# swesterfeld/audiowmark

Measured on AMD Instinct MI355X. Metric: audio seconds watermarked+decoded per wall-second (xRT), 44.1 kHz stereo, higher is better.
Workload: dtype f32; 1 GPU; 60 min stereo 44.1 kHz white noise per GPU resident in HBM, add+get incl. payload decode, payload 0123456789abcdef0011223344556677, strength 10; parallelism=1 GPU, patterns=108, payload_matches=104, ranks_seen=1

## Files before the change

audiowmark_amd/binding.py:

```python
import ctypes as C
import os

import numpy as np

_HERE = os.path.dirname(os.path.abspath(__file__))
N_BANDS = 81
BLOCK_FRAMES = 2226
SOFT_BITS = 858


class AwmError(RuntimeError):
    pass


def library_path():
    return os.path.join(_HERE, "libawm_hip.so")




def _load_hip_runtime():
    candidates = []
    try:
        import torch
# ... 105 lines not shown
lib.awm_add_watermark_segments_rate_s16_d.argtypes = [_vp, _vp, C.c_size_t, _vp, _vp, _vp, _vp, _vp, C.c_int, C.c_int]
lib.awm_add_watermark_segments_keys_rate_s16_d.argtypes = [_vp, _vp, C.c_size_t, _vp, _vp, _vp, _vp, _vp, C.c_int, C.c_int]
lib.awm_add_watermark_segments_rates_d.argtypes = [_vp, _vp, C.c_size_t, _vp, _vp, _vp, _vp, _vp, C.c_int, _vp]
lib.awm_add_watermark_segments_keys_rates_d.argtypes = [_vp, _vp, C.c_size_t, _vp, _vp, _vp, _vp, _vp, C.c_int, _vp]
lib.awm_add_watermark_segments_rates_s16_d.argtypes = [_vp, _vp, C.c_size_t, _vp, _vp, _vp, _vp, _vp, C.c_int, _vp]
lib.awm_add_watermark_segments_keys_rates_s16_d.argtypes = [_vp, _vp, C.c_size_t, _vp, _vp, _vp, _vp, _vp, C.c_int, _vp]


class SegmentPlan(C.Structure):
    _fields_ = [(n, C.c_uint64) for n in ("mix_first", "frame_first", "frame_last", "slice_first", "slice_last", "down_first", "down_last",
                                          "in_first", "in_last", "limiter_block", "first_block", "n_blocks")] + \
               [(n, C.c_int) for n in ("down_hl", "down_np", "down_step", "up_hl", "up_np", "up_step")]


lib.awm_add_segment_plan.argtypes = [C.c_int, C.c_size_t, C.c_size_t, C.POINTER(SegmentPlan)]


class StreamRatePlan(C.Structure):
    _fields_ = [(n, C.c_uint64) for n in ("limiter_block", "down_ahead", "mix_ahead", "min_tile")] + \
               [(n, C.c_int) for n in ("down_hl", "down_np", "down_step", "up_hl", "up_np", "up_step")]


lib.awm_add_stream_rate_plan.argtypes = [C.c_int, C.POINTER(StreamRatePlan)]
lib.awm_add_stream_create_rate_at.argtypes = [_vp, _vp, C.c_char_p, C.c_int, C.c_int, C.c_size_t, C.c_size_t, C.POINTER(_vp)]
lib.awm_add_stream_create_payloads_rate_at.argtypes = [_vp, _vp, _vp, C.c_size_t, C.c_int, C.c_int, C.c_size_t, C.c_size_t, C.POINTER(_vp)]
lib.awm_add_stream_sample_rate.argtypes = [_vp]
lib.awm_add_stream_sample_rate.restype = C.c_int
lib.awm_debug_resample_span_d.argtypes = [_vp, _vp, C.c_size_t, C.c_uint64, C.c_uint64, C.c_size_t, C.c_int, C.c_int, C.c_int, _vp, C.POINTER(C.c_int)]
lib.awm_debug_add_segments_fused_in_use.argtypes = []
lib.awm_debug_add_segments_fused_in_use.restype = C.c_int
lib.awm_debug_alloc_bytes.argtypes = []
lib.awm_debug_alloc_bytes.restype = C.c_ulonglong
lib.awm_debug_payload_tables_d.argtypes = [_vp, _vp, _vp, C.c_size_t, _vp]
lib.awm_debug_key_templates_d.argtypes = [_vp, _vp, C.c_size_t, _vp]
lib.awm_debug_key_payload_tables_d.argtypes = [_vp, _vp, _vp, C.c_size_t, _vp]
lib.awm_get_watermark_batch_d.argtypes = [_vp, _vp, C.c_size_t, _vp, _vp, C.c_int, C.c_int, C.c_size_t, _vp, _vp]
lib.awm_add_watermark_batch_keys_d.argtypes = [_vp, _vp, C.c_char_p, C.c_size_t, _vp, _vp, _vp, C.c_int]
lib.awm_get_watermark_batch_keys_d.argtypes = [_vp, _vp, C.c_size_t, _vp, _vp, C.c_int, C.c_int, C.c_size_t, _vp, _vp]
lib.awm_get_watermark_rate_d.argtypes = [_vp, _vp, _vp, C.c_size_t, C.c_int, C.c_int, C.c_size_t, _vp]
lib.awm_get_watermark_batch_rate_d.argtypes = [_vp, _vp, C.c_size_t, _vp, _vp, C.c_int, C.c_int, C.c_int, C.c_size_t, _vp, _vp]
lib.awm_get_watermark_batch_keys_rate_d.argtypes = [_vp, _vp, C.c_size_t, _vp, _vp, C.c_int, C.c_int, C.c_int, C.c_size_t, _vp, _vp]
lib.awm_debug_clip_slice_values.argtypes = [C.c_int]
lib.awm_debug_clip_slice_values.restype = C.c_size_t
lib.awm_debug_clip_stage_d.argtypes = [_vp, C.c_size_t, _vp, _vp, C.c_int, C.c_int, _vp, _vp]
lib.awm_get_watermark_batch_rates_d.argtypes = [_vp, _vp, C.c_size_t, _vp, _vp, C.c_int, _vp, C.c_int, C.c_size_t, _vp, _vp]
lib.awm_get_watermark_batch_keys_rates_d.argtypes = [_vp, _vp, C.c_size_t, _vp, _vp, C.c_int, _vp, C.c_int, C.c_size_t, _vp, _vp]
lib.awm_debug_clip_stage_rates_d.argtypes = [_vp, C.c_size_t, _vp, _vp, C.c_int, _vp, _vp, _vp]
lib.awm_get_batch_rates_plan.argtypes = [C.c_size_t, _vp, _vp, _vp, _vp]
lib.awm_get_watermark_batch_rates_s16_d.argtypes = [_vp, _vp, C.c_size_t, _vp, _vp, C.c_int, _vp, C.c_int, C.c_size_t, _vp, _vp]
lib.awm_get_watermark_batch_keys_rates_s16_d.argtypes = [_vp, _vp, C.c_size_t, _vp, _vp, C.c_int, _vp, C.c_int, C.c_size_t, _vp, _vp]
lib.awm_debug_clip_stage_rates_s16_d.argtypes = [_vp, C.c_size_t, _vp, _vp, C.c_int, _vp, _vp, _vp]
lib.awm_debug_clip_form_launches.argtypes = [_vp]
lib.awm_debug_clip_form_launches.restype = None
lib.awm_debug_lane_pcm_bytes.argtypes = [_vp]
lib.awm_debug_lane_pcm_bytes.restype = C.c_size_t
lib.awm_decode_chunk_d.argtypes = [_vp, _vp, _vp, C.c_size_t, C.c_int, C.c_int, C.c_size_t, _vp]
lib.awm_tab_up_down.argtypes = [_vp, C.c_int, C.c_int, _vp, _vp]
lib.awm_tab_bit_pos.argtypes = [_vp, _vp]
lib.awm_tab_mix_entries.argtypes = [_vp, _vp]
lib.awm_tab_bit_order.argtypes = [_vp, C.c_size_t, _vp]
lib.awm_tab_frame_mod.argtypes = [_vp, C.c_char_p, _vp]
lib.awm_tab_frame_mod_template.argtypes = [_vp, _vp]
lib.awm_tab_sync_bits.argtypes = [_vp, C.c_int, _vp]
lib.awm_tab_window.argtypes = [C.c_size_t, _vp]
lib.awm_tab_synth_window.argtypes = [_vp]
lib.awm_conv_encode.argtypes = [C.c_int, _vp, C.c_size_t, _vp]
lib.awm_test_gen_noise.argtypes = [_vp, C.c_size_t, _vp]


class RawFormat(C.Structure):
    _fields_ = [("n_channels", C.c_int), ("sample_rate", C.c_int), ("bit_depth", C.c_int), ("encoding", C.c_int), ("big_endian", C.c_int)]


lib.awm_add_watermark_file.argtypes = [_vp, _vp, C.c_char_p, C.c_char_p, C.c_char_p, C.POINTER(RawFormat), C.POINTER(RawFormat)]
lib.awm_add_stream_watermark_file.argtypes = [_vp, _vp, C.c_char_p, C.c_char_p, C.c_char_p, C.POINTER(RawFormat), C.POINTER(RawFormat), C.c_size_t]
lib.awm_add_stream_create_at.argtypes = [_vp, _vp, C.c_char_p, C.c_int, C.c_size_t, C.c_size_t, C.POINTER(_vp)]
lib.awm_debug_sync_db_sliding_d.argtypes = [_vp, _vp, C.c_size_t, C.c_int, _vp, C.c_size_t, C.c_int, C.c_int, _vp]
lib.awm_debug_sync_db_sliding_rows_d.argtypes = [_vp, _vp, C.c_size_t, C.c_int, _vp, _vp, C.c_size_t, C.c_int, C.c_int, _vp, _vp, C.c_longlong, C.c_longlong,
                                                 _vp, _vp, C.c_int, C.c_int, C.c_int, _vp, _vp, C.c_longlong, _vp, C.c_longlong]
lib.awm_debug_block_plane_ld.argtypes = [_vp]
lib.awm_debug_block_db_d.argtypes = [_vp, _vp, _vp, C.c_size_t, C.c_int, _vp, C.c_size_t, C.c_uint32, _vp, C.c_size_t, C.c_size_t, _vp, C.c_size_t,
                                     _vp, _vp]
lib.awm_debug_soft_bits_planes_d.argtypes = [_vp, _vp, _vp, C.c_size_t, C.c_size_t, C.c_int, _vp, _vp, _vp, C.c_size_t, _vp]
lib.awm_get_watermark_file.argtypes = [_vp, _vp, C.c_char_p, C.POINTER(RawFormat), C.c_size_t, _vp]
lib.awm_add_get_watermark_file.argtypes = [_vp, _vp, C.c_char_p, C.c_char_p, C.c_char_p, C.POINTER(RawFormat), C.POINTER(RawFormat), C.c_size_t, _vp]
lib.awm_add_stream_create.argtypes = [_vp, _vp, C.c_char_p, C.c_int, C.c_size_t, C.POINTER(_vp)]
lib.awm_add_stream_destroy.argtypes = [_vp]
lib.awm_add_stream_destroy.restype = None
lib.awm_add_stream_input.argtypes = [_vp]
lib.awm_add_stream_input.restype = C.c_void_p
lib.awm_add_stream_push.argtypes = [_vp, C.c_size_t, C.c_int, _vp, _vp]
lib.awm_add_mix_payloads_d.argtypes = [_vp, _vp, _vp, C.c_size_t, C.c_size_t, C.c_int, _vp, C.c_double, C.c_size_t, _vp, _vp, _vp,
                                       C.c_size_t, C.c_size_t]
lib.awm_add_stream_create_payloads_at.argtypes = [_vp, _vp, _vp, C.c_size_t, C.c_int, C.c_size_t, C.c_size_t, C.POINTER(_vp)]
lib.awm_add_stream_payloads.argtypes = [_vp]
lib.awm_add_stream_payloads.restype = C.c_size_t
lib.awm_add_stream_push_payloads.argtypes = [_vp, C.c_size_t, C.c_int, _vp, _vp]
lib.awm_add_watermark_payloads_file.argtypes = [_vp, _vp, _vp, C.c_size_t, C.c_char_p, _vp, C.POINTER(RawFormat), C.POINTER(RawFormat)]
lib.awm_add_stream_watermark_payloads_file.argtypes = [_vp, _vp, _vp, C.c_size_t, C.c_char_p, _vp, C.POINTER(RawFormat), C.POINTER(RawFormat),
                                                       C.c_size_t]
lib.awm_debug_set_payloads_file_tile.argtypes = [C.c_int]
lib.awm_debug_set_payloads_file_tile.restype = None


lib.awm_decode_chunks_d.argtypes = [_vp, _vp, _vp, C.c_size_t, C.c_int, C.c_int, _vp, _vp, C.c_int, C.c_size_t, _vp, _vp]
lib.awm_pcm_decode_d.argtypes = [_vp, _vp, C.c_size_t, C.c_int, C.c_int, C.c_int, _vp]
lib.awm_pcm_encode_d.argtypes = [_vp, _vp, C.c_size_t, C.c_int, C.c_int, C.c_int, C.c_int, _vp]
lib.awm_plan_chunks.argtypes = [C.c_size_t, C.c_size_t, _vp, _vp, _vp]
lib.awm_merge_patterns.argtypes = [_vp, _vp, _vp, C.c_int, C.c_size_t, _vp]
lib.awm_prof_name.restype = C.c_char_p
lib.awm_set_speed_params.argtypes = [C.c_int, C.c_int, C.c_double, C.c_double]
lib.awm_set_speed_params.restype = None
lib.awm_resample_ratio_frames.argtypes = [C.c_size_t, C.c_int, C.c_int, C.c_double, C.c_double]
lib.awm_resample_ratio_frames.restype = C.c_size_t
lib.awm_resample_ratio_d.argtypes = [_vp, _vp, C.c_size_t, C.c_int, C.c_int, C.c_double, C.c_double, _vp, C.c_size_t]
lib.awm_detect_speed_d.argtypes = [_vp, _vp, _vp, C.c_size_t, C.c_int, C.c_int, C.c_int, _vp, _vp]
lib.awm_detect_speed_batch_d.argtypes = [_vp, _vp, C.c_int, C.c_size_t, _vp, _vp, C.c_int, C.c_int, C.c_int, _vp, _vp, _vp]
lib.awm_debug_set_speed_batch_bytes.argtypes = [C.c_size_t]
lib.awm_debug_set_speed_batch_bytes.restype = None
lib.awm_debug_speed_batch_bytes.argtypes = []
lib.awm_debug_speed_batch_bytes.restype = C.c_size_t
lib.awm_debug_set_speed_batch.argtypes = [C.c_int]
lib.awm_debug_set_speed_batch.restype = None
lib.awm_speed_batch_plan.argtypes = [C.c_size_t, _vp, C.c_int, C.c_int, C.c_int, C.c_size_t, _vp, _vp]
lib.awm_debug_speed_batch_launches.argtypes = [_vp, _vp, _vp, _vp]
lib.awm_debug_speed_batch_launches.restype = None
lib.awm_debug_speed_scan_batch_d.argtypes = [_vp, _vp, C.c_int, C.c_size_t, _vp, _vp, C.c_int, C.c_int, _vp, C.c_double, C.c_double, C.c_int, C.c_int,
                                             _vp, _vp, C.c_size_t, _vp, _vp, _vp]
lib.awm_speed_clip_location_d.argtypes = [_vp, _vp, _vp, C.c_size_t, C.c_int, C.c_int, C.c_double, C.c_int, _vp]
lib.awm_speed_mags_d.argtypes = [_vp, _vp, _vp, C.c_size_t, C.c_int, C.c_int, C.c_double, C.c_double, C.c_double, C.c_size_t, _vp]
lib.awm_var_resample_table.argtypes = [C.c_double, _vp, C.c_size_t, C.POINTER(C.c_int)]
lib.awm_speed_scan_d.argtypes = [_vp, _vp, _vp, C.c_size_t, C.c_int, C.c_int, C.c_double, C.c_double, C.c_double, C.c_int, C.c_int,
                                 _vp, C.c_int, C.c_size_t, _vp, _vp]


class Params(C.Structure):
    _fields_ = [("struct_size", C.c_size_t), ("water_delta", C.c_double), ("mix", C.c_int), ("hard", C.c_int), ("strict", C.c_int),
                ("snr", C.c_int), ("payload_size", C.c_int), ("frames_per_bit", C.c_int), ("sync_threshold2", C.c_double),
                ("get_n_best", C.c_int), ("get_chunk_size", C.c_double), ("detect_speed", C.c_int), ("detect_speed_patient", C.c_int),
                ("try_speed", C.c_double), ("test_speed", C.c_double), ("test_cut", C.c_int), ("test_no_sync", C.c_int),
                ("test_no_limiter", C.c_int), ("test_truncate", C.c_int)]

    def __init__(self, **kw):
        super().__init__()
        lib.awm_params_init(C.byref(self))
        for k, v in kw.items():
            if k not in dict(self._fields_):
                raise TypeError(f"awm_params has no field {k}")
            setattr(self, k, v)


lib.awm_params_init.argtypes = [C.POINTER(Params)]
lib.awm_params_init.restype = None
lib.awm_set_global_params.argtypes = [C.POINTER(Params)]
lib.awm_ctx_set_params.argtypes = [_vp, C.POINTER(Params)]
lib.awm_ctx_get_params.argtypes = [_vp, C.POINTER(Params)]
lib.awm_ctx_snr_begin.argtypes = [_vp]
lib.awm_ctx_snr_end.argtypes = [_vp, C.POINTER(C.c_double), C.POINTER(C.c_double)]
lib.awm_get_watermark_keys_d.argtypes = [_vp, _vp, C.c_int, _vp, C.c_size_t, C.c_int, C.c_size_t, _vp, _vp]
lib.awm_get_watermark_keys_file.argtypes = [_vp, _vp, C.c_int, C.c_char_p, C.POINTER(RawFormat), C.c_size_t, _vp, _vp]


def set_global_params(**kw):
    p = Params(**kw)
    _check(lib.awm_set_global_params(C.byref(p)), "awm_set_global_params")

# ... 938 lines not shown
    def sync_fft(self, pcm, index, frame_count, want_frames=None, first=0, last=None, out=None):
        import torch
        n, ch = _pcm_shape(pcm)
        if last is None:
            last = n * ch
        if out is None:
            db = torch.zeros((frame_count, N_BANDS), dtype=torch.float32, device=pcm.device)
            have = torch.zeros(frame_count, dtype=torch.int8, device=pcm.device)
        else:
            db = _out_tensor(out[0], (frame_count, N_BANDS), torch.float32, pcm.device, "sync_fft (db)")
            have = _out_tensor(out[1], (frame_count,), torch.int8, pcm.device, "sync_fft (have)")
        want = None
        if want_frames is not None:
            want = np.ascontiguousarray(want_frames, np.int8)
        _check(lib.awm_sync_fft_d(self._h, _dev_ptr(pcm), n, ch, index, frame_count, _np(want) if want is not None else None,
                                  first, last, _dev_ptr(db), _dev_ptr(have)), "awm_sync_fft_d")
        return db, have

    def sync_search(self, key, pcm, clip_mode=False, max_out=4096):
        n, ch = _pcm_shape(pcm)
        while True:
            idx = np.zeros(max_out, np.uint64)
            q = np.zeros(max_out, np.float64)
            bt = np.zeros(max_out, np.int32)
            cnt = _check(lib.awm_sync_search_d(self._h, key_bytes(key), _dev_ptr(pcm), n, ch, int(clip_mode), max_out, _np(idx),
                                               _np(q), _np(bt)), "awm_sync_search_d")
            if cnt <= max_out:
                return idx[:cnt], q[:cnt], bt[:cnt]
            max_out = cnt

    def search_approx(self, key, pcm, clip_mode=False):
        n, ch = _pcm_shape(pcm)
        max_out = 4 * (n // 1024 + 1)
        idx = np.zeros(max_out, np.uint64)
        raw = np.zeros(max_out, np.float64)
        mean = np.zeros(max_out, np.float64)
        cnt = _check(lib.awm_search_approx_d(self._h, key_bytes(key), _dev_ptr(pcm), n, ch, int(clip_mode), max_out, _np(idx),
                                             _np(raw), _np(mean)), "awm_search_approx_d")
        return idx[:cnt], raw[:cnt], mean[:cnt]

    def block_soft_bits(self, key, pcm, indices):
        n, ch = _pcm_shape(pcm)
        idx = np.ascontiguousarray(indices, np.uint64)
        out = np.zeros((len(idx), SOFT_BITS), np.float32)
        ok = np.zeros(len(idx), np.int32)
        _check(lib.awm_block_soft_bits_d(self._h, key_bytes(key), _dev_ptr(pcm), n, ch, _np(idx), len(idx), _np(out), _np(ok)),
               "awm_block_soft_bits_d")
        return out, ok

    def block_plane_ld(self):
        return _check(lib.awm_debug_block_plane_ld(self._h), "awm_debug_block_plane_ld")

    def debug_block_db(self, key, pcm, indices, fill=0x7FC00000, slice_range=None, slice_frames=0, planes=None):
        import torch
        n, ch = _pcm_shape(pcm)
        idx = np.ascontiguousarray(indices, np.uint64)
        if planes is None:
            planes = torch.empty((len(idx), ch, N_BANDS, self.block_plane_ld()), dtype=torch.float32, device=pcm.device)
        assert planes.dtype == torch.float32 and planes.is_cuda and planes.is_contiguous()
        assert slice_range is None or (slice_range.dtype == torch.int64 and slice_range.is_cuda and slice_range.is_contiguous() and slice_range.dim() == 2
                                       and slice_range.shape[1] == 2)
        soft = np.zeros((len(idx), SOFT_BITS), np.float32)
        slot = np.zeros(len(idx), np.int32)
        _check(lib.awm_debug_block_db_d(self._h, key_bytes(key), _dev_ptr(pcm), n, ch, _np(idx), len(idx), fill,
                                        _dev_ptr(slice_range) if slice_range is not None else None,
                                        slice_range.shape[0] if slice_range is not None else 0, slice_frames, _dev_ptr(planes), planes.numel(),
                                        _np(soft), _np(slot)), "awm_debug_block_db_d")
        return planes, soft, slot

    def debug_soft_bits_planes(self, key, planes, n_blocks=None, channels=None, block_base=None, slice_range=None, range_index=None):
        import torch
        assert planes.dtype == torch.float32 and planes.is_cuda and planes.is_contiguous()
        n_blocks = planes.shape[0] if n_blocks is None else n_blocks
        channels = planes.shape[1] if channels is None else channels
        for t, dtype in ((block_base, torch.int64), (slice_range, torch.int64), (range_index, torch.int32)):
            assert t is None or (t.dtype == dtype and t.is_cuda and t.is_contiguous())
        opt = lambda t: _dev_ptr(t) if t is not None else None
        soft = np.zeros((max(n_blocks, 1), SOFT_BITS), np.float32)
        _check(lib.awm_debug_soft_bits_planes_d(self._h, key_bytes(key), _dev_ptr(planes), planes.numel(), n_blocks, channels, opt(block_base),
                                                opt(slice_range), opt(range_index), slice_range.shape[0] if slice_range is not None else 0,
                                                _np(soft)), "awm_debug_soft_bits_planes_d")
        return soft[:n_blocks]

    def viterbi_decode(self, block_type, soft):
        soft = np.ascontiguousarray(soft, np.float32)
        if soft.ndim == 1:
            soft = soft[None, :]
        n, coded_len = soft.shape
        rate = 12 if block_type == 2 else 6
        bits = np.zeros((n, coded_len // rate - 15), np.int32)
        err = np.zeros(n, np.float32)
        _check(lib.awm_viterbi_decode(self._h, block_type, _np(soft), coded_len, n, _np(bits), _np(err)), "awm_viterbi_decode")
        return bits, err

    def _pattern_buffer(self, max_out):
        buf = getattr(self, "_pat_buf", None)
        if buf is None or len(buf) < max_out:
            buf = self._pat_buf = (Pattern * max_out)()
        return buf

    def _patterns(self, fn, what, *args, max_out=4096):
        while True:
            buf = self._pattern_buffer(max_out)
            cnt = _check(fn(*args, max_out, C.cast(buf, C.c_void_p)), what)
            if cnt <= max_out:
                return patterns_to_dicts(buf, cnt)
            max_out = cnt

    def get_watermark(self, key, pcm, sample_rate=44100):
        n, ch = _pcm_shape(pcm)
        if sample_rate != 44100:
            return self._patterns(lib.awm_get_watermark_rate_d, "awm_get_watermark_rate_d", self._h, key_bytes(key), _dev_ptr(pcm), n, ch,
                                  sample_rate)
        return self._patterns(lib.awm_get_watermark_d, "awm_get_watermark_d", self._h, key_bytes(key), _dev_ptr(pcm), n, ch)

    def clip_stage(self, clips, sample_rate, out=None):
        import torch
        rates = _rates_array(sample_rate, len(clips))
        shapes = [_pcm_shape(c) for c in clips]
        ch = shapes[0][1]
        assert all(s[1] == ch for s in shapes)
        values = lib.awm_debug_clip_slice_values(ch)
        if out is None:
            out = torch.zeros((len(clips), values), dtype=torch.float32, device=clips[0].device)
        assert out.dtype == torch.float32 and out.is_contiguous() and out.numel() == len(clips) * values
        ptrs = (C.c_void_p * len(clips))(*[_dev_ptr(c) for c in clips])
        frames = (C.c_size_t * len(clips))(*[s[0] for s in shapes])
        ranges = np.zeros((len(clips), 2), np.int64)
        if rates is not None:
            _check(lib.awm_debug_clip_stage_rates_d(self._h, len(clips), ptrs, frames, ch, rates, _dev_ptr(out), _np(ranges)),
                   "awm_debug_clip_stage_rates_d")
        else:
            _check(lib.awm_debug_clip_stage_d(self._h, len(clips), ptrs, frames, ch, sample_rate, _dev_ptr(out), _np(ranges)),
                   "awm_debug_clip_stage_d")
        return out, ranges

    def add_get_watermark(self, key, payload_hex, pcm, out, sample_rate=44100):
        n, ch = _pcm_shape(pcm)
        assert _pcm_shape(out) == (n, ch) and out.data_ptr() != pcm.data_ptr()
        return self._patterns(lib.awm_add_get_watermark_d, "awm_add_get_watermark_d", self._h, key_bytes(key), payload_hex.encode(),
                              _dev_ptr(pcm), _dev_ptr(out), n, ch, sample_rate)

    def set_params(self, params=None, **kw):
        if params is None and kw:
            params = self.get_params()
            for k, v in kw.items():
                if k not in dict(Params._fields_):
                    raise TypeError(f"awm_params has no field {k}")
                setattr(params, k, v)
        _check(lib.awm_ctx_set_params(self._h, C.byref(params) if params is not None else None), "awm_ctx_set_params")

    def get_params(self):
        p = Params()
        _check(lib.awm_ctx_get_params(self._h, C.byref(p)), "awm_ctx_get_params")
        return p

    def snr_begin(self):
        _check(lib.awm_ctx_snr_begin(self._h), "awm_ctx_snr_begin")

    def snr_end(self):
        import math
        sig, delta = C.c_double(), C.c_double()
        _check(lib.awm_ctx_snr_end(self._h, C.byref(sig), C.byref(delta)), "awm_ctx_snr_end")
        return 10 * math.log10(sig.value / delta.value) if delta.value > 0 else float("inf")

    def _patterns_keys(self, fn, what, keys, *args, max_out=4096):
# ... 131 lines not shown
```

audiowmark_amd/csrc/hip/kernels.hh:

```
#pragma once
#include <hip/hip_runtime.h>
#include <cstddef>
#include <cstdint>

#if defined(__HIP_DEVICE_COMPILE__) && !defined(__gfx950__)
#error "audiowmark_amd's HIP kernels are written for gfx950 (MI355X) only"
#endif

namespace awmk {

struct DevTables
{
  const float2 *tw512;
  const float2 *tw1024;
  const float  *window;
  const float  *synth;
  const double2 *slide;
  const double2 *tw512d;
  const float2 *slide32;
};

hipError_t launch_stft_full (hipStream_t st, const DevTables& t, const float *pcm, int n_channels,
                             long long start_index, long long hop, long long frame_count, float2 *out);

// ... 163 lines not shown
                                             bool stereo_aligned, size_t lds_bytes);
struct RateMixSegment { MixSegment s; int limiter_block; };
hipError_t launch_mix_max_segments_rates (hipStream_t st, const RateMixSegment *segs_dev, int n_segs, long long max_frames, int n_channels,
                                          int min_limiter_block);
hipError_t launch_max_segments_rates_s16 (hipStream_t st, const RateMixSegment *segs_dev, int n_segs, long long max_frames, int n_channels,
                                          int min_limiter_block);
struct RateLimiterClip { LimiterClip c; int limiter_block; };
hipError_t launch_limiter_table_batch_rates (hipStream_t st, const RateLimiterClip *clips_dev, int n_clips, float ceiling, long long max_tab);
hipError_t launch_limiter_batch_rates (hipStream_t st, const RateLimiterClip *clips_dev, int n_clips, long long max_frames, int n_channels,
                                       int min_limiter_block, float ceiling, long long max_tab);
struct RateLimitEncodeSegment { LimitEncodeSegment s; int limiter_block; };
hipError_t launch_limit_encode_segments_rates (hipStream_t st, const RateLimitEncodeSegment *segs_dev, int n_segs, long long max_frames, bool mix,
                                               int min_limiter_block);

hipError_t launch_power_sums (hipStream_t st, const float *orig, const float *mixed, long long n_values, double *acc);

struct SyncDbArgs
{
  const float *pcm;
  long long    n_frames;
  int          n_channels;
  int          per_channel;
  long long    base0, base_stride;
  const long long *stream_base;
  int          count0;
  const int   *stream_count;
  long long    n_streams;
  long long    hop;
  float       *out;
  long long    out_stream_stride;
  long long    ld;
  char        *have;
  long long    have_stream_stride;
  long long    first, last;
  int          tile_frames;
  int          xcd_interleave = 0;
  const int           *row_perm = nullptr;
  const unsigned char *band_pos = nullptr;
  int                  rows_per_plane = 0;
  float               *tail = nullptr;
  long long            tail_stream_stride = 0;
  int                  tables_per_slice = 0;
  int                  streams_per_slice = 0;
  long long            slice_stride = 0;
  const long long     *stream_range = nullptr;
  const int           *range_index = nullptr;
  int                  range_div = 1;
  int                  silent_frames_are_zero = 0;
  int                  skip_unread_silent_tiles = 0;
};
hipError_t launch_sync_db (hipStream_t st, const DevTables& t, const SyncDbArgs& a);
hipError_t launch_sync_db_sliding (hipStream_t st, const DevTables& t, const SyncDbArgs& a);
bool sliding_rows_have_tail (int n_channels);

struct SyncTableDev
{
  const int *packed;
  int        rows_per_bit;
  const unsigned *chains = nullptr;
  long long       chains_slice_stride = 0;
  int             planes_per_slice = 1;
  const int      *row_frames = nullptr;
};
void pack_scan_chains (const int *packed, int rows_per_bit, unsigned *out );
struct SyncScanArgs
{
  const float *db;
  const char  *have;
  int          have_is_run = 0;
  long long    plane_stride;
  long long    have_plane_stride;
  long long    row_stride, band_stride, have_row_stride;
  long long    n_lanes;
  const int   *lane_count;
  long long    n_planes;
  double       min_delta;
  double      *quality;
  long long    q_stride;
  SyncTableDev table;
};
hipError_t launch_sync_scan (hipStream_t st, const SyncScanArgs& a);
hipError_t launch_sync_scan_window (hipStream_t st, const SyncScanArgs& a, int total_frames);

struct GatheredScanArgs
{
  const float *db;
  const char  *have;
  long long    plane_stride, have_plane_stride;
  int          ld;
  int          have_ld = 0;
  const float *tail = nullptr;
  long long    tail_plane_stride = 0;
  int          rows_per_bit;
  int          n_lanes;
  const int   *lane_count;
  long long    n_planes;
  double       min_delta;
  double      *quality;
  long long    q_stride;
  float       *chain_mag;
  int         *chain_n;
  int          regular_waves, tail_first, tail_lanes;
};
constexpr size_t GATHERED_SCRATCH_BYTES_PER_PLANE = 18 * 128 * 4;
hipError_t launch_sync_scan_gathered (hipStream_t st, const GatheredScanArgs& a);

hipError_t launch_local_mean (hipStream_t st, const double *q, long long q_stride, long long n_start_frames,
                              double *raw_sorted, double *local_mean, int n_slices = 1);

struct PeakOut { long long p; double raw, mean; };
hipError_t launch_peak_select (hipStream_t st, const double *raw_sorted, const double *local_mean, long long n, double threshold,
                               unsigned int *count, PeakOut *out, unsigned int cap);
hipError_t launch_peak_select_slices (hipStream_t st, const double *raw_sorted, const double *local_mean, long long n, double threshold,
                                      unsigned int *count, int count_stride, PeakOut *out, unsigned int cap, int n_slices);

hipError_t launch_peak_topk (hipStream_t st, const PeakOut *in, const unsigned int *count, unsigned int cap, PeakOut *out, int k, int n_slices);
hipError_t launch_peak_topk_lists (hipStream_t st, const PeakOut *in, const unsigned int *count, int count_stride, unsigned int cap,
                                   PeakOut *out, int k, int n_slices, int n_lists);

struct SoftBitsArgs
{
  const float   *db;
  long long      block_stride, ld;
  int            n_channels;
  const int16_t *mix_frame;
  const uint8_t *mix_up, *mix_down;
  int            n_data_frames;
  int            frames_per_bit;
  int            block_frames;
  long long      n_blocks;
  float         *out;
  const int     *block_slice = nullptr;
  const long long *block_base = nullptr;
  const long long *stream_range = nullptr;
  const int       *range_index = nullptr;
};
hipError_t launch_soft_bits (hipStream_t st, const SoftBitsArgs& a);
bool soft_bits_skips_silent_items (int n_channels, int frames_per_bit);

struct SoftJobDev
{
  int       mode;
  int       n_src, src_off;
  int       len;
  int       norm0, norm1;
  long long out_off;
  int       order_off;
  int       pad;
};
struct SoftPrepArgs
{
  const float      *raw;
  int               n_bits;
  const int        *inv_order;
  const SoftJobDev *jobs;
  const int2       *src;
  long long         n_jobs;
  int               hard;
  float            *out;
};
hipError_t launch_soft_prep (hipStream_t st, const SoftPrepArgs& a);

hipError_t launch_viterbi (hipStream_t st, const float *const soft[3], const long long n_blocks[3], long long n_steps,
                           unsigned char *const decisions_ws[3], int *const bits_out[3], float *const error_out[3], unsigned int *sync_ws);
size_t viterbi_workspace_bytes (long long coded_len, int rate, long long n_blocks);
bool viterbi_steps_supported (long long n_steps);
size_t viterbi_sync_bytes (long long n_blocks);
double probe_dependent_launch_us (hipStream_t st);
const char *viterbi_form_description();

struct KeyTableArgs
{
  const unsigned char *round_keys;
  const unsigned char *sbox;
  const unsigned char *coded;
  unsigned char       *scratch;
  int                  scratch_slots;
  signed char         *tables;
  long long            n_keys;
};
size_t key_table_scratch_bytes();
size_t key_table_bytes();
hipError_t launch_frame_mod_tables (hipStream_t st, const KeyTableArgs& a);

struct KeyTemplateOut
{
  short    *tmpl;
  long long stride;
};
hipError_t launch_key_templates (hipStream_t st, const KeyTableArgs& a, const KeyTemplateOut& t);

struct PayloadTableArgs
{
  const short         *tmpl;
  const int           *tmpl_of;
  long long            tmpl_stride;
  const unsigned char *coded;
  signed char         *tables;
  long long            table_stride;
  int                  half_entries;
  int                  n_code;
  int                  n_payloads;
};
size_t     payload_table_stride (size_t block_frames);
hipError_t launch_payload_tables (hipStream_t st, const PayloadTableArgs& a);

struct ClipKeyTableOut
{
  unsigned int  *chains;
  int           *row_frames, *want, *perm;
  unsigned char *pos;
  short         *mix_frame;
  unsigned char *mix_up, *mix_down;
  int           *inv_order;
};
constexpr int CLIP_KEY_ROWS = 170, CLIP_KEY_WANT = 1020, CLIP_KEY_MIX = 51480, CLIP_KEY_CODED = 858;
hipError_t launch_clip_key_tables (hipStream_t st, const KeyTableArgs& a, const ClipKeyTableOut& out);

// ... 112 lines not shown
```

audiowmark_amd/csrc/hip/kernels.hip:

```cpp
#include "kernels.hh"
#include "awm_fft.hip.h"
#include <cstdlib>
#include <algorithm>
#include <type_traits>
#include <atomic>

namespace awmk {

constexpr int NB = 81;
constexpr int MIN_BAND = 20;
constexpr int WAVES = 4;

typedef const int __attribute__ ((address_space (4))) *const_int_ptr;

__device__ __forceinline__ void
load_shared_tables (const DevTables& t, float2 *s_tw, float *s_win, float2 *s_twb)
{
  fft512_load_twiddles (t.tw512, s_tw);
  for (int i = threadIdx.x; i < 1024; i += blockDim.x)
    s_win[i] = t.window[i];
  if (s_twb)
    for (int i = threadIdx.x; i < NB; i += blockDim.x)
      s_twb[i] = t.tw1024[MIN_BAND + i];
}
// ... 3376 lines not shown
  int chain, cand;
  if (int (blockIdx.x) < a.regular_waves)
    {
      chain = blockIdx.x % 12;
      cand = (blockIdx.x / 12) * 64 + lane;
    }
  else
    {
      chain = lane / a.tail_lanes;
      cand = a.tail_first + lane % a.tail_lanes;
    }
  const bool active = chain < 12 && cand < count;
  if (!__any (active))
    return;
  if (!active)
    chain = 0, cand = 0;
  const int bit = chain >> 1, down = chain & 1;
  const int R = a.rows_per_bit;
  const int ld = a.ld;
  const bool from_tail = a.tail && cand >= ld;
  const long long step = from_tail ? 1 : ld;
  const float *p = from_tail ? a.tail + plane * a.tail_plane_stride + ((long long) bit * R * 60 + down * 30)
                             : a.db + plane * a.plane_stride + ((long long) bit * R * 60 + down * 30) * ld + cand;
  const int hld = a.have_ld ? a.have_ld : ld;
  const char *hv = HAVE ? a.have + plane * a.have_plane_stride + (long long) bit * R * hld + cand : nullptr;

  float mag = 0.f;
  int n = 0;
  auto issue = [&] (int r, float (&v)[30], bool& present) {
    const float *q = p + (long long) r * 60 * step;
    present = HAVE ? hv[r * hld] != 0 : true;
    if (HAVE && !__any (present))
      return;
#pragma unroll
    for (int i = 0; i < 30; i++)
      v[i] = q[i * step];
  };
  auto accumulate = [&] (const float (&v)[30], bool present) {
    if (present)
      {
#pragma unroll
        for (int i = 0; i < 30; i++)
          mag = __fadd_rn (mag, v[i]);
        n++;
      }
  };
  float v[3][30];
  bool pr[3] = { false, false, false };
  const int last = R - 1;
  int r = 0;
  if (R > 0)
    {
#pragma unroll
      for (int k = 0; k < 2; k++)
        {
          issue (k < last ? k : last, v[k], pr[k]);
          __builtin_amdgcn_sched_barrier (0);
        }
      for (; r + 3 <= R; r += 3)
        {
#pragma unroll
          for (int k = 0; k < 3; k++)
            {
              const int nx = r + k + 2;
              issue (nx < last ? nx : last, v[(k + 2) % 3], pr[(k + 2) % 3]);
              __builtin_amdgcn_sched_barrier (0);
              accumulate (v[k], pr[k]);
              __builtin_amdgcn_sched_barrier (0);
            }
        }
#pragma unroll
      for (int k = 0; k < 2; k++)
        if (r + k < R)
          accumulate (v[k], pr[k]);
    }
  if (active)
    {
      a.chain_mag[(plane * 12 + chain) * 128 + cand] = mag;
      if (!down)
        a.chain_n[(plane * 6 + bit) * 128 + cand] = n;
    }
}

__global__ void __launch_bounds__ (64)
sync_quality_kernel (GatheredScanArgs a)
{
  const long long plane = blockIdx.y;
  const int cand = blockIdx.x * 64 + threadIdx.x;
  if (cand >= a.lane_count[plane])
    return;
  double q = 0;
  int total = 0;
  for (int b = 0; b < 6; b++)
    {
      const float um = a.chain_mag[(plane * 12 + 2 * b) * 128 + cand], dm = a.chain_mag[(plane * 12 + 2 * b + 1) * 128 + cand];
      const int n = a.chain_n[(plane * 6 + b) * 128 + cand];
      float raw;
      if (um == 0 || dm == 0)
        raw = 0;
      else if (um < dm)
        raw = __fsub_rn (1.f, __fdiv_rn (um, dm));
      else
        raw = __fsub_rn (__fdiv_rn (dm, um), 1.f);
      const double rb = (b & 1) ? double (raw) : -double (raw);
      q += rb * n;
      total += n;
    }
  if (total)
    q /= total;
  q = q / a.min_delta / 2.9;
  a.quality[plane * a.q_stride + cand] = q;
}

hipError_t
launch_sync_scan_gathered (hipStream_t st, const GatheredScanArgs& a0)
{
  if (a0.n_lanes <= 0 || a0.n_planes <= 0)
    return hipSuccess;
  if (!a0.lane_count || a0.n_planes > 65535 || a0.n_lanes > 128 || !a0.chain_mag || !a0.chain_n)
    return hipErrorInvalidValue;
  GatheredScanArgs a = a0;
  const int full = a.n_lanes / 64, rem = a.n_lanes % 64;
  const bool tail = rem > 0 && rem * 12 <= 64;
  a.regular_waves = 12 * (tail || rem == 0 ? full : full + 1);
  a.tail_first = 64 * full;
  a.tail_lanes = tail ? rem : 1;
  const dim3 grid (unsigned (a.regular_waves + (tail ? 1 : 0)), unsigned (a.n_planes));
  if (a.have)
    hipLaunchKernelGGL (sync_scan_gathered_kernel<true>, grid, dim3 (64), 0, st, a);
  else
    hipLaunchKernelGGL (sync_scan_gathered_kernel<false>, grid, dim3 (64), 0, st, a);
  hipLaunchKernelGGL (sync_quality_kernel, dim3 (unsigned ((a.n_lanes + 63) / 64), unsigned (a.n_planes)), dim3 (64), 0, st, a);
  return hipGetLastError();
}

__global__ void __launch_bounds__ (256)
local_mean_kernel (const double *q, long long q_stride, long long S, double *raw_sorted, double *local_mean)
{
  const long long p = (long long) blockIdx.x * blockDim.x + threadIdx.x;
  const long long n_scores = 4 * S;
  if (p >= n_scores)
    return;
  q += (long long) blockIdx.y * 4 * q_stride;
  raw_sorted += (long long) blockIdx.y * n_scores;
  local_mean += (long long) blockIdx.y * n_scores;
  double avg = 0;
  int n = 0;
  for (int j = -20; j <= 20; j++)
    {
      if (j > -4 && j < 4)
        continue;
      const long long idx = p + j;
      if (idx >= 0 && idx < n_scores)
        {
          avg += q[(idx & 3) * q_stride + (idx >> 2)];
          n++;
        }
    }
  if (n > 0)
    avg /= n;
  raw_sorted[p] = q[(p & 3) * q_stride + (p >> 2)];
  local_mean[p] = avg;
}

hipError_t
launch_local_mean (hipStream_t st, const double *q, long long q_stride, long long n_start_frames, double *raw_sorted, double *local_mean,
                   int n_slices)
{
  const long long n = 4 * n_start_frames;
  if (n <= 0 || n_slices <= 0)
    return hipSuccess;
  hipLaunchKernelGGL (local_mean_kernel, dim3 (unsigned ((n + 255) / 256), unsigned (n_slices)), dim3 (256), 0, st, q, q_stride, n_start_frames,
                      raw_sorted, local_mean);
  return hipGetLastError();
}

__global__ void __launch_bounds__ (128)
soft_bits_kernel (SoftBitsArgs a)
{
  const long long blk = blockIdx.y;
  const int bit = blockIdx.x * blockDim.x + threadIdx.x;
  const int n_bits = a.n_data_frames / a.frames_per_bit;
  if (bit >= n_bits)
    return;
  const float *db = a.db + blk * a.block_stride;
  const int C = a.n_channels;
  const long long mix0 = a.block_slice ? (long long) a.block_slice[blk] * a.n_data_frames * 30 : 0;
  const int16_t *mix_frame = a.mix_frame + mix0;
  const uint8_t *mix_up = a.mix_up + mix0, *mix_down = a.mix_down + mix0;
  double umag = 0, dmag = 0;
  for (int f = bit * a.frames_per_bit; f < (bit + 1) * a.frames_per_bit; f++)
    for (int ch = 0; ch < C; ch++)
      {
        const float *plane = db + (long long) ch * NB * a.ld;
        for (int j = 0; j < 30; j++)
          {
            const int b = f * 30 + j;
            const int frame = mix_frame[b];
            const int next = frame + 1 < a.block_frames ? frame + 1 : frame - 1;
            const int prev = frame - 1 >= 0 ? frame - 1 : frame + 1;
            const float *pu = plane + (long long) (mix_up[b] - MIN_BAND) * a.ld;
            const float *pd = plane + (long long) (mix_down[b] - MIN_BAND) * a.ld;
            umag += pu[frame];
            umag -= double (__fadd_rn (pu[prev], pu[next])) * 0.5;
            dmag += pd[frame];
            dmag -= double (__fadd_rn (pd[prev], pd[next])) * 0.5;
          }
      }
  a.out[blk * n_bits + bit] = float (umag - dmag);
}

constexpr int SB_WAVES = 4;
constexpr int SB_BPW = 4;
constexpr int SB_MAX_ITEMS = 256;

__global__ void __launch_bounds__ (64 * SB_WAVES)
soft_bits_wave_kernel (SoftBitsArgs a, int groups_per_block)
{
  extern __shared__ __attribute__ ((aligned (16))) float4 s_item_dyn[];
  const int lane = threadIdx.x & 63, wave = threadIdx.x >> 6;
  const long long slot = blockIdx.x >> 3;
  const long long blk = (slot / groups_per_block) * 8 + (blockIdx.x & 7);
  const int group = int (slot % groups_per_block);
  if (blk >= a.n_blocks)
    return;
  const int n_bits = a.n_data_frames / a.frames_per_bit;
  const int bit0 = (group * SB_WAVES + wave) * SB_BPW;
  if (bit0 >= n_bits)
    return;
  const float *db = a.db + blk * a.block_stride;
  const int C = a.n_channels;
  const long long mix0 = a.block_slice ? (long long) a.block_slice[blk] * a.n_data_frames * 30 : 0;
  const int16_t *mix_frame = a.mix_frame + mix0;
  const uint8_t *mix_up = a.mix_up + mix0, *mix_down = a.mix_down + mix0;
  const int n_items = a.frames_per_bit * C * 30;
  float4 *items = s_item_dyn + (size_t) wave * SB_BPW * n_items;
  const int n_here = min (SB_BPW, n_bits - bit0);
  int live_lo = 0, live_hi = 0x7fffffff;
  if (a.stream_range)
    {
      const long long sl = a.range_index[blk];
      const long long first = a.stream_range[2 * sl], last = a.stream_range[2 * sl + 1];
      live_lo = a.block_frames;
      live_hi = -1;
      if (first >= 0)
        {
          const long long base = a.block_base[blk];
          const long long lo_num = (first + C - 1) / C - 1024 - base, hi_num = last / C - base;
          const long long lo = lo_num <= 0 ? 0 : (lo_num + 1023) / 1024, hi = hi_num < 0 ? -1 : hi_num / 1024;
          live_lo = int (lo < a.block_frames ? lo : a.block_frames);
          live_hi = int (hi < a.block_frames ? hi : a.block_frames - 1);
        }
    }
  const float zero_db = db_from_complex (make_float2 (0.f, 0.f));
  for (int i = lane; i < n_items; i += 64)
#pragma unroll
  for (int q = 0; q < SB_BPW; q++)
    {
      const int e = q * n_items + i;
      const int bit = bit0 + min (q, n_here - 1);
      const int fi = i / (C * 30), ch = (i / 30) % C, j = i % 30;
      const int b = (bit * a.frames_per_bit + fi) * 30 + j;
      const int frame = mix_frame[b];
      const int next = frame + 1 < a.block_frames ? frame + 1 : frame - 1;
      const int prev = frame - 1 >= 0 ? frame - 1 : frame + 1;
      if (max (frame, max (prev, next)) < live_lo || min (frame, min (prev, next)) > live_hi)
        {
          items[e] = make_float4 (zero_db, __fadd_rn (zero_db, zero_db), zero_db, __fadd_rn (zero_db, zero_db));
          continue;
        }
      const float *plane = db + (long long) ch * NB * a.ld;
      const float *pu = plane + (long long) (mix_up[b] - MIN_BAND) * a.ld;
      const float *pd = plane + (long long) (mix_down[b] - MIN_BAND) * a.ld;
      items[e] = make_float4 (pu[frame], __fadd_rn (pu[prev], pu[next]), pd[frame], __fadd_rn (pd[prev], pd[next]));
    }
  wave_sync();
  if (lane < n_here)
    {
      const float4 *mine = items + lane * n_items;
      double umag = 0, dmag = 0;
      for (int i = 0; i < n_items; i++)
        {
          const float4 t = mine[i];
          umag = __dadd_rn (umag, double (t.x));
          umag = __dsub_rn (umag, __dmul_rn (double (t.y), 0.5));
          dmag = __dadd_rn (dmag, double (t.z));
          dmag = __dsub_rn (dmag, __dmul_rn (double (t.w), 0.5));
        }
      a.out[blk * n_bits + bit0 + lane] = float (__dsub_rn (umag, dmag));
    }
}

int g_soft_bits_generic = 0;
extern "C" void awm_debug_set_soft_bits_generic (int on) { g_soft_bits_generic = on; }

bool
soft_bits_skips_silent_items (int n_channels, int frames_per_bit)
{
  return !g_soft_bits_generic && frames_per_bit * n_channels * 30 <= SB_MAX_ITEMS;
}

hipError_t
launch_soft_bits (hipStream_t st, const SoftBitsArgs& a)
{
  if (a.n_blocks <= 0)
    return hipSuccess;
  const int n_bits = a.n_data_frames / a.frames_per_bit;
// ... 990 lines not shown
```

audiowmark_amd/csrc/host/capi_kernels.cc:

```cpp
#include "context.hh"
#include "syncfinder.hh"
#include "wmget.hh"
#include "wmdecode.hh"
#include "wmspeed.hh"
#include "utils.hh"
#include "wmfile.hh"
#include "keytab_stage.hh"
#include <sys/stat.h>
#include <atomic>
#include <future>
#include <thread>
#include <tuple>
#include <algorithm>
#include <array>
#include <cmath>
#include <cstdlib>
#include <cstring>
#include <memory>

using namespace awm;
namespace awm { Key capi_key (const uint8_t key[16]); }
namespace awm { extern int g_key_tables_on_device; int clip_key_tables_check (awm_ctx *ctx, const uint8_t *keys, size_t n_keys, long long mismatch_out[9]); }

namespace {
// ... 1660 lines not shown
    bad = "slice_range_d, n_slices and slice_frames go together";
  else if (slice_range_d && (slice_frames > n_frames || n_slices > n_frames / slice_frames))
    bad = "the slices do not fit into the samples";
  if (!bad && slice_range_d)
    for (size_t i = 0; i < n_blocks && !bad; i++)
      if (index[i] <= n_frames && n_frames - index[i] >= block_len && index[i] / slice_frames >= n_slices)
        bad = "a block starts behind the last slice";
  if (!bad && slice_range_d)
    if (int rc = debug_check_ranges (ctx, slice_range_d, n_slices, (long long) (n_frames * n_channels), bad))
      return rc;
  if (bad)
    {
      set_error (std::string ("awm_debug_block_db_d: ") + bad);
      return AWM_ERR_ARG;
    }
  KeyTables *kt = ctx->get_key_tables (capi_key (key));
  if (!kt)
    return AWM_ERR_HIP;
  const size_t n_bits = mark_data_frame_count() / params().frames_per_bit;
  const std::vector<size_t> idx (index, index + n_blocks);
  std::vector<int> slot_of;
  std::vector<char> ok;
  const BlockDbView view { fill, planes_out_d };
  if (int rc = block_soft_bits_dev (ctx, ctx, kt, make_wav (pcm_d, n_frames, n_channels), idx, slot_of, ok, slice_range_d, slice_frames, &view))
    return rc;
  size_t n_slots = 0;
  for (size_t i = 0; i < n_blocks; i++)
    {
      slot_out[i] = slot_of[i];
      n_slots = std::max (n_slots, size_t (slot_of[i] + 1));
    }
  if (n_slots)
    AWM_HIP_CHECK (hipMemcpyAsync (soft_out, ctx->ws_soft.ptr, n_slots * n_bits * sizeof (float), hipMemcpyDeviceToHost, ctx->stream));
  AWM_HIP_CHECK (stream_wait (ctx->stream));
  return 0;
}

int
awm_debug_soft_bits_planes_d (awm_ctx *ctx, const uint8_t key[16], const float *planes_d, size_t planes_values, size_t n_blocks, int n_channels,
                              const long long *block_base_d, const long long *slice_range_d, const int *range_index_d, size_t n_slices,
                              float *soft_out)
{
  AWM_ENTER (ctx);
  const size_t block_values = size_t (std::max (n_channels, 0)) * Params::n_bands * size_t (block_plane_ld());
  const bool ranges = slice_range_d != nullptr;
  const char *bad = nullptr;
  if (!planes_d || !soft_out)
    bad = "null pointer";
  else if (n_channels < 1 || n_channels > 3)
    bad = "1, 2 or 3 channels";
  else if (n_blocks < 1 || n_blocks > DEBUG_BLOCKS_MAX)
    bad = "1 .. 64 blocks";
  else if (planes_values / block_values < n_blocks)
    bad = "planes_d holds fewer than n_blocks blocks";
  else if ((block_base_d != nullptr) != ranges || (range_index_d != nullptr) != ranges || (n_slices != 0) != ranges)
    bad = "block_base_d, slice_range_d, range_index_d and n_slices go together";
  if (!bad && ranges)
    {
      std::vector<long long> base (n_blocks);
      std::vector<int> slice (n_blocks);
      AWM_HIP_CHECK (hipMemcpyAsync (base.data(), block_base_d, n_blocks * sizeof (long long), hipMemcpyDeviceToHost, ctx->stream));
      AWM_HIP_CHECK (hipMemcpyAsync (slice.data(), range_index_d, n_blocks * sizeof (int), hipMemcpyDeviceToHost, ctx->stream));
      if (int rc = debug_check_ranges (ctx, slice_range_d, n_slices, DEBUG_RANGE_MAX * n_channels, bad))
        return rc;
      for (size_t i = 0; i < n_blocks && !bad; i++)
        if (base[i] < 0 || base[i] > DEBUG_RANGE_MAX || slice[i] < 0 || size_t (slice[i]) >= n_slices)
          bad = "a block's base or slice is out of range";
    }
  if (bad)
    {
      set_error (std::string ("awm_debug_soft_bits_planes_d: ") + bad);
      return AWM_ERR_ARG;
    }
  KeyTables *kt = ctx->get_key_tables (capi_key (key));
  if (!kt)
    return AWM_ERR_HIP;
  const size_t n_bits = mark_data_frame_count() / params().frames_per_bit;
  if (int rc = ctx->ws_soft.reserve (n_blocks * n_bits * sizeof (float))) return rc;
  const awmk::SoftBitsArgs sb = block_soft_args (kt, n_channels, planes_d, n_blocks, ctx->ws_soft.as<float>(), block_base_d, range_index_d,
                                                 slice_range_d, ranges);
  AWM_HIP_CHECK (awmk::launch_soft_bits (ctx->stream, sb));
  AWM_HIP_CHECK (hipMemcpyAsync (soft_out, ctx->ws_soft.ptr, n_blocks * n_bits * sizeof (float), hipMemcpyDeviceToHost, ctx->stream));
  AWM_HIP_CHECK (stream_wait (ctx->stream));
  return 0;
}

int
awm_viterbi_decode (awm_ctx *ctx, int block_type, const float *soft, size_t coded_len, size_t n, int *bits_out, float *error_out)
{
  AWM_ENTER (ctx);
  if (block_type < 0 || block_type > 2)
    return AWM_ERR_ARG;
  std::vector<std::vector<float>> in (n);
  for (size_t i = 0; i < n; i++)
    in[i].assign (soft + i * coded_len, soft + (i + 1) * coded_len);
  std::vector<std::vector<int>> bits;
  std::vector<float> errors;
  if (int rc = viterbi_decode (ctx, ConvBlockType (block_type), in, bits, errors))
    return rc;
  for (size_t i = 0; i < n; i++)
    {
      std::copy (bits[i].begin(), bits[i].end(), bits_out + i * bits[i].size());
      error_out[i] = errors[i];
    }
  return 0;
}

int
awm_add_watermark_d (awm_ctx *ctx, const uint8_t key[16], const char *payload_hex, const float *pcm_in_d, float *out_d,
                     size_t n_frames, int n_channels, int sample_rate)
{
  AWM_ENTER (ctx);
  if (n_channels >= 1 && add_buffers_overlap (pcm_in_d, out_d, n_frames * size_t (n_channels)))
    {
      set_error ("awm_add_watermark_d: the output overlaps the input");
      return AWM_ERR_ARG;
    }
  FrameModTable *fm = ctx->get_frame_mod (capi_key (key), payload_hex ? payload_hex : "");
  if (!fm)
    return AWM_ERR_ARG;
  if (sample_rate != Params::mark_sample_rate)
    return add_full_rate (ctx, pcm_in_d, out_d, n_frames, n_channels, fm->dev.as<int8_t>(), params().water_delta, !params().test_no_limiter, sample_rate);
  return add_full (ctx, pcm_in_d, out_d, n_frames, n_channels, fm->dev.as<int8_t>(), params().water_delta, !params().test_no_limiter);
}

extern "C" void awm_debug_set_add_payloads_fused (int on) { g_add_payloads_fused = on; }
extern "C" int  awm_debug_add_payloads_fused_in_use (void) { return g_add_payloads_fused_in_use; }
extern "C" int  awm_debug_add_payloads_tile (void) { return awmk::ADD_MULTI_TILE; }
static int g_add_payloads_rate_fused = 2, g_add_payloads_rate_fused_in_use = 0;
extern "C" void awm_debug_set_add_payloads_rate_fused (int mode) { g_add_payloads_rate_fused = mode < 0 ? 0 : mode > 2 ? 2 : mode; }
extern "C" int  awm_debug_add_payloads_rate_fused_in_use (void) { return g_add_payloads_rate_fused_in_use; }

static int
add_payloads_rate (awm_ctx *ctx, const Key& k, const char *const *payload_hex, size_t n_payloads, const float *pcm_in_d, float *const *out_d,
                   size_t n_frames, int C, double water_delta, int use_limiter, int rate, const RateConverter& down, const RateConverter& up,
                   bool *taken)
{
  hipStream_t st = ctx->stream;
  const size_t last44 = up.window_start (n_frames - 1) + size_t (up.hl()) + 1;
  const size_t F = last44 / Params::frame_size + 1;
  const size_t n44 = (F + 1) * Params::frame_size;
  const size_t n_ws = std::min<size_t> (n_payloads, size_t (awmk::ADD_MULTI_TILE)), ws_values = n44 * size_t (C);
  const int lim_block = int (size_t (rate) * size_t (Params::limiter_block_size_ms) / 1000);
  const size_t n_blocks = n_frames / lim_block + 2;
  const ResampleTable& ut = *up.fixed;
  awmk::ResampleMixArgs ma {};
  ma.orig = pcm_in_d;
  ma.n_in = (long long) (F * Params::frame_size);
  ma.n_channels = C;
  ma.ctab = ut.ctab.as<float>();
  ma.hl = ut.hl;
  ma.np = ut.np;
  ma.step = ut.step;
  ma.n_out = (long long) n_frames;
  ma.n_blocks = (long long) n_blocks;
  ma.limiter_block = lim_block;
  ma.n = 1;
  bool mixed = g_add_payloads_rate_fused == 2;
  for (size_t p = 0; mixed && p < n_payloads; p++)
    {
      ma.o[0].wm44 = pcm_in_d;
      ma.o[0].out = out_d[p];
      mixed = awmk::resample_mix_multi_takes (ma);
    }
  *taken = false;
  if (ctx->ws_rate_a.reserve (ws_values * sizeof (float)) || ctx->ws_rate_b.reserve (n_ws * ws_values * sizeof (float))
// ... 3056 lines not shown
```

audiowmark_amd/csrc/host/context.cc:

```cpp
#include "context.hh"
#include <algorithm>
#include <atomic>
#include <chrono>
#include <cstdlib>
#include "utils.hh"
#include <cmath>
#include <cstring>

namespace awm {

static thread_local std::string g_last_error;
void set_error (const std::string& msg) { g_last_error = msg; }
const std::string& last_error() { return g_last_error; }
std::string hip_error_string (hipError_t e) { return std::string (hipGetErrorName (e)) + " (" + hipGetErrorString (e) + ")"; }

static std::atomic<long>   g_dev_allocs { 0 }, g_pin_allocs { 0 };
static std::atomic<double> g_dev_alloc_ms { 0.0 }, g_pin_alloc_ms { 0.0 };
static std::atomic<unsigned long long> g_dev_alloc_bytes { 0 };
static void
note_alloc (std::atomic<long>& count, std::atomic<double>& ms, std::chrono::steady_clock::time_point t0)
{
  const double dt = std::chrono::duration<double, std::milli> (std::chrono::steady_clock::now() - t0).count();
  count.fetch_add (1, std::memory_order_relaxed);
  double cur = ms.load (std::memory_order_relaxed);
// ... 75 lines not shown
extern "C" void
awm_debug_alloc_stats (long *dev_allocs, double *dev_ms, long *pinned_allocs, double *pinned_ms)
{
  if (dev_allocs) *dev_allocs = awm::g_dev_allocs.load();
  if (dev_ms) *dev_ms = awm::g_dev_alloc_ms.load();
  if (pinned_allocs) *pinned_allocs = awm::g_pin_allocs.load();
  if (pinned_ms) *pinned_ms = awm::g_pin_alloc_ms.load();
}

extern "C" unsigned long long awm_debug_alloc_bytes (void) { return awm::g_dev_alloc_bytes.load(); }

hipEvent_t
awm::ReadyMarks::next_event()
{
  if (used == pool.size())
    {
      hipEvent_t e = nullptr;
      if (hipEventCreateWithFlags (&e, hipEventDisableTiming) != hipSuccess)
        return nullptr;
      pool.push_back (e);
    }
  return pool[used++];
}

void
awm::ReadyMarks::release()
{
  disarm();
  for (hipEvent_t e : pool)
    (void) hipEventDestroy (e);
  pool.clear();
}

bool
awm::FileStaging::ensure_events()
{
  if (have_events)
    return true;
  for (int i = 0; i < RING; i++)
    for (hipEvent_t *e : { &in_copied[i], &in_used[i], &out_encoded[i], &out_copied[i] })
      if (!*e && hipEventCreateWithFlags (e, hipEventDisableTiming) != hipSuccess)
        return false;
  have_events = true;
  return true;
}

void
awm::FileStaging::release()
{
  for (int i = 0; i < RING; i++)
    {
      for (hipEvent_t *e : { &in_copied[i], &in_used[i], &out_encoded[i], &out_copied[i] })
        if (*e)
          {
            (void) hipEventDestroy (*e);
            *e = nullptr;
          }
      in_host[i].release();
      out_host[i].release();
      in_dev[i].release();
      out_dev[i].release();
    }
  pcm.release();
  have_events = false;
}

void
awm::WorkLane::release_lane()
{
  for (DevBuffer *b : { &ws_db, &ws_block_db, &ws_have, &ws_q, &ws_raw, &ws_mean, &ws_misc, &ws_refine, &ws_refine_have, &ws_soft, &ws_viterbi,
                        &ws_viterbi_in, &ws_viterbi_bits, &ws_viterbi_err, &ws_viterbi_sync, &ws_block_max, &ws_clip, &ws_idx, &ws_limit_tab, &ws_jobs, &ws_group, &ws_keytab, &ws_keytab_aux, &ws_keytab_scratch, &ws_rate, &ws_pcm, &ws_shard_edge, &ws_shard_tail, &ws_shard_q })
    b->release();
  for (PinnedBuffer *b : { &pin_refine_in[0], &pin_refine_in[1], &pin_refine_q[0], &pin_refine_q[1], &pin_peaks, &pin_blocks, &pin_jobs, &pin_bits, &pin_small, &pin_group, &pin_shard, &pin_shard_up, &pin_keytab })
    b->release();
  for (hipEvent_t& ev : ev_refine)
    if (ev)
      {
        (void) hipEventDestroy (ev);
        ev = nullptr;
      }
  if (ev_sync)
    (void) hipEventDestroy (ev_sync);
  ev_sync = nullptr;
  awm::speed_scratch_free (this);
}

unsigned int *
awm::WorkLane::viterbi_sync (size_t n_decodes)
{
  const size_t before = ws_viterbi_sync.bytes;
  if (ws_viterbi_sync.reserve (awmk::viterbi_sync_bytes ((long long) n_decodes)))
    return nullptr;
  if (ws_viterbi_sync.bytes != before && hipMemsetAsync (ws_viterbi_sync.ptr, 0, ws_viterbi_sync.bytes, stream) != hipSuccess)
    {
      ws_viterbi_sync.release();
      return nullptr;
    }
  return ws_viterbi_sync.as<unsigned int>();
}

awm::WorkLane *
awm_ctx::lane (int i)
{
  if (i <= 0)
    return this;
  if (i >= awm::MAX_LANES)
    return nullptr;
  auto& l = extra_lanes[i - 1];
  if (!l)
    {
      auto nl = std::make_unique<awm::WorkLane>();
      if (hipStreamCreateWithFlags (&nl->stream, hipStreamNonBlocking) != hipSuccess)
        return nullptr;
      nl->own_stream = true;
      l = std::move (nl);
    }
  return l.get();
}

using namespace awm;

int
awm::upload_sync (DevBuffer& buf, const void *src, size_t bytes, hipStream_t st)
{
  if (int rc = buf.reserve (bytes ? bytes : 1))
    return rc;
  static std::mutex staging_mutex;
  static PinnedBuffer staging;
  std::lock_guard<std::mutex> lock (staging_mutex);
  if (int rc = staging.reserve (bytes ? bytes : 1))
    return rc;
  std::memcpy (staging.ptr, src, bytes);
  AWM_HIP_CHECK (hipMemcpyAsync (buf.ptr, staging.ptr, bytes, hipMemcpyHostToDevice, st));
  AWM_HIP_CHECK (hipStreamSynchronize (st));
  return 0;
}

std::vector<float>
awm::zita_table (double frel, unsigned h, unsigned n)
{
  auto sinc = [] (double x) { x = std::fabs (x); if (x < 1e-6) return 1.0; x *= M_PI; return std::sin (x) / x; };
  auto wind = [] (double x) { x = std::fabs (x); if (x >= 1.0) return 0.0; x *= M_PI; return 0.384 + 0.500 * std::cos (x) + 0.116 * std::cos (2 * x); };
  std::vector<float> ctab (size_t (h) * (n + 1));
  float *p = ctab.data();
  for (unsigned j = 0; j <= n; j++)
    {
      double t = double (j) / double (n);
      for (unsigned i = 0; i < h; i++)
        {
          p[h - i - 1] = float (frel * sinc (t * frel) * wind (t / h));
          t += 1;
        }
      p += h;
    }
  return ctab;
}

static int
upload (DevBuffer& buf, const void *src, size_t bytes, hipStream_t st)
{
  return upload_sync (buf, src, bytes, st);
}

static std::vector<int>
pack_sync_table (const SyncTable& t, const std::vector<int>& want_pos )
{
  const int R = t.rows_per_bit;
  std::vector<int> packed (size_t (6) * R * 64, 0);
  for (int bit = 0; bit < 6; bit++)
    for (int r = 0; r < R; r++)
      {
        int *row = &packed[(size_t (bit) * R + r) * 64];
        const size_t src = size_t (bit) * R + r;
        for (int i = 0; i < 30; i++)
          {
            row[i] = t.up[src * 30 + i];
            row[30 + i] = t.down[src * 30 + i];
          }
        row[60] = want_pos.empty() ? t.frame[src] : want_pos[t.frame[src]];
        row[61] = r + 1 < R ? (want_pos.empty() ? t.frame[src + 1] : want_pos[t.frame[src + 1]]) : 0x7fffffff;
      }
  return packed;
}

namespace awm {
ClipKeyHost
build_clip_key_host (const Key& key)
{
  ClipKeyHost h;
  const SyncTable st = build_sync_table (key, true);
  const int total = mark_block_frame_count() * 2, R = st.rows_per_bit;
  std::vector<int> want_pos (total, -1);
  std::vector<char> want (total, 0);
  for (int f : st.frame)
    want[f] = 1;
  for (int f = 0; f < total; f++)
    if (want[f])
// ... 388 lines not shown

  std::vector<float> blob;
  auto push_c = [&] (double re, double im) { blob.push_back (float (re)); blob.push_back (float (im)); };
  const size_t off_tw512 = blob.size();
  for (int k = 0; k < 512; k++)
    push_c (std::cos (-2 * M_PI * k / 512), std::sin (-2 * M_PI * k / 512));
  const size_t off_tw1024 = blob.size();
  for (int k = 0; k <= 512; k++)
    push_c (std::cos (-2 * M_PI * k / 1024), std::sin (-2 * M_PI * k / 1024));
  while (blob.size() % 4) blob.push_back (0);
  const size_t off_win = blob.size();
  auto win = gen_normalized_window (Params::frame_size);
  blob.insert (blob.end(), win.begin(), win.end());
  const size_t off_synth = blob.size();
  auto synth = gen_synth_window();
  blob.insert (blob.end(), synth.begin(), synth.end());
  std::vector<double> slide;
  for (int k = 19; k <= 102; k++)
    {
      for (int j = 0; j < 8; j++)
        {
          slide.push_back (std::cos (-2 * M_PI * k * j / 1024));
          slide.push_back (std::sin (-2 * M_PI * k * j / 1024));
        }
      slide.push_back (std::cos (2 * M_PI * k * 8 / 1024));
      slide.push_back (std::sin (2 * M_PI * k * 8 / 1024));
    }
  const size_t off_tw512d = slide.size();
  for (int k = 0; k < 512; k++)
    {
      slide.push_back (std::cos (-2 * M_PI * k / 512));
      slide.push_back (std::sin (-2 * M_PI * k / 512));
    }
  const size_t off_slide32 = slide.size();
  {
    std::vector<float> f;
    for (int k = 19; k <= 102; k++)
      for (int j = 0; j < 8; j++)
        {
          f.push_back (float (std::cos (2 * M_PI * k * (8 - j) / 1024)));
          f.push_back (float (std::sin (2 * M_PI * k * (8 - j) / 1024)));
        }
    slide.resize (off_slide32 + f.size() / 2);
    std::memcpy (slide.data() + off_slide32, f.data(), f.size() * sizeof (float));
  }
  if (int rc = upload (ctx->tab_slide, slide.data(), slide.size() * sizeof (double), ctx->stream))
    return rc;
  ctx->tabs.slide = ctx->tab_slide.as<double2>();
  ctx->tabs.tw512d = reinterpret_cast<const double2 *> (ctx->tab_slide.as<double>() + off_tw512d);
  ctx->tabs.slide32 = reinterpret_cast<const float2 *> (ctx->tab_slide.as<double>() + off_slide32);
  if (int rc = upload (ctx->tab_mem, blob.data(), blob.size() * sizeof (float), ctx->stream))
    return rc;
  const float *base = ctx->tab_mem.as<float>();
  ctx->tabs.tw512 = reinterpret_cast<const float2 *> (base + off_tw512);
  ctx->tabs.tw1024 = reinterpret_cast<const float2 *> (base + off_tw1024);
  ctx->tabs.window = base + off_win;
  ctx->tabs.synth = base + off_synth;
  if (awmk::probe_dependent_launch_us (ctx->stream) < 0 && hipStreamSynchronize (ctx->stream) != hipSuccess)
    {
      set_error ("awm_ctx_create: the device does not complete work on the context's stream");
      return AWM_ERR_HIP;
    }
  *ctx_out = ctx.release();
  return 0;
}

int
awm_ctx_set_chunk_lanes (awm_ctx *ctx, int n_lanes)
{
  if (!ctx || n_lanes < 1)
    return AWM_ERR_ARG;
  ctx->chunk_lanes = std::min (n_lanes, awm::CHUNK_LANES);
  return 0;
}

int
awm_ctx_warm_up (awm_ctx *ctx, int detect_speed, int file_level)
{
  if (!ctx)
    return AWM_ERR_ARG;
  AWM_HIP_CHECK (hipSetDevice (ctx->device));
  const int lanes = std::max (1, std::min (ctx->chunk_lanes, awm::CHUNK_LANES)) * (detect_speed ? 2 : 1);
  for (int i = 0; i < lanes && i < awm::MAX_LANES; i++)
    if (!ctx->lane (i))
      {
        awm::set_error ("cannot create a work lane (stream)");
        return AWM_ERR_HIP;
      }
  if (file_level && !ctx->get_copy_stream())
    {
      awm::set_error ("cannot create the copy stream");
      return AWM_ERR_HIP;
    }
  return 0;
}

int
awm_ctx_trim (awm_ctx *ctx)
{
  if (!ctx)
    return AWM_ERR_ARG;
  AWM_HIP_CHECK (hipSetDevice (ctx->device));
  AWM_HIP_CHECK (hipStreamSynchronize (ctx->stream));
  for (auto& l : ctx->extra_lanes)
    if (l)
      {
        if (l->stream)
          AWM_HIP_CHECK (hipStreamSynchronize (l->stream));
        l->release_lane();
      }
  if (ctx->copy_stream)
    AWM_HIP_CHECK (hipStreamSynchronize (ctx->copy_stream));
  ctx->release_lane();
  ctx->file_staging.release();
  awm::speed_workspace_free (ctx);
  ctx->ws_add_batch.release();
  ctx->pin_add_batch.release();
  ctx->ws_seg_in.release();
  ctx->ws_key_tmpl.release();
  ctx->ws_seg_out.release();
  ctx->ws_merge_soft.release();
  ctx->ws_rate_a.release();
  ctx->ws_rate_b.release();
  ctx->ws_rate_c.release();
  for (awm_ctx *h : ctx->helpers)
    if (h && h != ctx)
      if (int rc = awm_ctx_trim (h)) return rc;
  return 0;
}

size_t
awm_debug_lane_pcm_bytes (awm_ctx *ctx)
{
  if (!ctx)
    return 0;
  size_t bytes = ctx->ws_pcm.bytes;
  for (auto& l : ctx->extra_lanes)
    if (l)
      bytes += l->ws_pcm.bytes;
  return bytes;
}

void
awm_ctx_destroy (awm_ctx *ctx)
{
  if (!ctx)
    return;
  (void) hipSetDevice (ctx->device);
  (void) hipStreamSynchronize (ctx->stream);
  for (auto& kt : ctx->key_tables)
    release_key_tables (*kt);
  for (auto& t : ctx->frame_mod_tables)
    t->dev.release();
  for (auto& t : ctx->frame_mod_templates)
    t->dev.release();
  for (auto& t : ctx->resample_tables)
    t->ctab.release();
  awm::speed_workspace_free (ctx);
  ctx->ws_snr.release();
  ctx->ws_seg_in.release();
  ctx->ws_key_tmpl.release();
  ctx->ws_seg_out.release();
  ctx->ws_add_batch.release();
  ctx->pin_add_batch.release();
  if (ctx->ev_add_batch)
    (void) hipEventDestroy (ctx->ev_add_batch);
  ctx->ev_add_batch = nullptr;
  ctx->ws_merge_soft.release();
  for (hipEvent_t e : ctx->merge_events)
    if (e)
      (void) hipEventDestroy (e);
  ctx->merge_events.clear();
  ctx->ws_rate_a.release();
  ctx->ws_rate_b.release();
  ctx->ws_rate_c.release();
  ctx->tab_mem.release();
  ctx->tab_slide.release();
  for (auto& l : ctx->extra_lanes)
    if (l)
      {
        if (l->stream)
          (void) hipStreamSynchronize (l->stream);
        l->release_lane();
        if (l->own_stream && l->stream)
          (void) hipStreamDestroy (l->stream);
      }
  ctx->release_lane();
  if (ctx->copy_stream)
    (void) hipStreamSynchronize (ctx->copy_stream);
  ctx->file_staging.release();
  ctx->ready.release();
  if (ctx->copy_stream)
    (void) hipStreamDestroy (ctx->copy_stream);
  if (ctx->own_stream && ctx->stream)
    (void) hipStreamDestroy (ctx->stream);
  delete ctx;
}

int awm_ctx_device (const awm_ctx *ctx) { return ctx ? ctx->device : -1; }

int
awm_ctx_synchronize (awm_ctx *ctx)
{
  if (!ctx)
    return AWM_ERR_ARG;
  AWM_HIP_CHECK (hipStreamSynchronize (ctx->stream));
  return 0;
}

void *awm_ctx_stream (awm_ctx *ctx) { return ctx ? (void *) ctx->stream : nullptr; }

int
awm_ctx_set_stream (awm_ctx *ctx, void *hip_stream)
{
  if (!ctx)
    return AWM_ERR_ARG;
  AWM_HIP_CHECK (hipStreamSynchronize (ctx->stream));
  if (ctx->own_stream && ctx->stream)
    (void) hipStreamDestroy (ctx->stream);
  ctx->stream = (hipStream_t) hip_stream;
  ctx->own_stream = false;
  return 0;
}

}
```

audiowmark_amd/csrc/host/context.hh:

```
#pragma once
#include <condition_variable>
#include <mutex>
#include <hip/hip_runtime.h>
#include <map>
#include <mutex>
#include <memory>
#include <string>
#include <vector>
#include "../hip/kernels.hh"
#include "wmcommon.hh"

namespace awm { void set_error (const std::string& msg); const std::string& last_error(); std::string hip_error_string (hipError_t e); }

#define AWM_HIP_CHECK(expr) \
  do { hipError_t e__ = (expr); if (e__ != hipSuccess) { awm::set_error (std::string (#expr) + ": " + awm::hip_error_string (e__)); return AWM_ERR_HIP; } } while (0)

namespace awm {

inline void
cpu_relax()
{
  for (int k = 0; k < 48; k++)
    __builtin_ia32_pause();
}
// ... 107 lines not shown

struct SpeedWorkspace;
struct SpeedScratch;
struct WorkLane;
void speed_scratch_free (WorkLane *lane);
} struct awm_ctx; namespace awm {
void speed_workspace_free (awm_ctx *ctx);

struct FileStaging
{
  static constexpr int RING = 4;
  PinnedBuffer in_host[RING], out_host[RING];
  DevBuffer    in_dev[RING], out_dev[RING];
  DevBuffer    pcm;
  bool         keep = false;
  size_t       kept_values = 0;
  int          kept_channels = 0, kept_rate = 0;
  hipEvent_t   in_copied[RING] = {}, in_used[RING] = {}, out_encoded[RING] = {}, out_copied[RING] = {};
  bool         have_events = false;
  bool         ensure_events();
  void         release();
};

struct ReadyMarks
{
  const float *base = nullptr;
  size_t       n_frames = 0;
  bool         armed = false;
  std::vector<std::pair<size_t, hipEvent_t>> marks;
  std::vector<hipEvent_t> pool;
  size_t       used = 0;
  hipEvent_t   next_event();
  bool         live = false, live_done = false;
  std::mutex   mu;
  std::condition_variable cv;
  void         disarm() { armed = false; live = live_done = false; marks.clear(); used = 0; base = nullptr; n_frames = 0; }
  void         release();
};

struct FrameModTable
{
  std::vector<unsigned char> key;
  std::string payload;
  bool        mix = true;
  int         frames_per_bit = 2;
  unsigned long last_use = 0;
  DevBuffer   dev;
};

struct FrameModTemplate
{
  std::vector<unsigned char> key;
  bool        mix = true;
  int         frames_per_bit = 2;
  unsigned long last_use = 0;
  DevBuffer   dev;
};

}

namespace awm {
enum ProfId { PROF_ADD_MIX, PROF_LIMITER, PROF_SYNC_DB, PROF_SYNC_SCAN, PROF_LOCAL_MEAN, PROF_REFINE_DB, PROF_REFINE_SCAN,
              PROF_BLOCK_DB, PROF_SOFT_BITS, PROF_VITERBI, PROF_STFT,
              PROF_RESAMPLE, PROF_RESAMPLE_VAR, PROF_SPEED_MAGS, PROF_SPEED_COMPARE, PROF_KEYTAB, PROF_ADD_MIX_MULTI, PROF_PAYLOAD_TAB,
              PROF_RESAMPLE_MIX, PROF_CLIP_RESAMPLE, PROF_KEY_TEMPLATE, PROF_CLIP_STAGE_MIXED,
              PROF_CLIP_PAD_S16, PROF_CLIP_RESAMPLE_S16, PROF_CLIP_STAGE_MIXED_S16,
              PROF_PCM_DECODE, PROF_PCM_ENCODE, PROF_SEGMENT_GATHER_S16, PROF_LIMIT_ENCODE_S16, PROF_COUNT };
struct ProfPending { int id; hipEvent_t start, stop; };
}

namespace awm {
struct WorkLane
{
  hipStream_t    stream = nullptr;
  bool           own_stream = false;
  DevBuffer ws_db, ws_block_db, ws_have, ws_q, ws_raw, ws_mean, ws_misc, ws_refine, ws_refine_have, ws_soft,
            ws_viterbi, ws_viterbi_in, ws_viterbi_bits, ws_viterbi_err, ws_viterbi_sync, ws_block_max, ws_clip, ws_idx, ws_limit_tab, ws_jobs, ws_group, ws_keytab, ws_keytab_aux, ws_keytab_scratch;
  DevBuffer ws_rate;
  DevBuffer ws_pcm;
  DevBuffer ws_shard_edge, ws_shard_tail, ws_shard_q;
  PinnedBuffer pin_refine_in[2], pin_refine_q[2], pin_peaks, pin_blocks, pin_jobs, pin_bits, pin_small, pin_group, pin_shard, pin_shard_up, pin_keytab;
  hipEvent_t   ev_refine[2] = { nullptr, nullptr };
  hipEvent_t   ev_sync = nullptr;
  SpeedScratch *speed_scratch = nullptr;
  double       prof_live_fraction = 1.0;
  unsigned int *viterbi_sync (size_t n_decodes);
  void release_lane();
};
constexpr int MAX_LANES = 16;
constexpr int CHUNK_LANES = 4;
}

struct awm_ctx : awm::WorkLane
{
  int            device = -1;
  awmk::DevTables tabs {};
  awm::DevBuffer tab_mem, tab_slide;

  std::vector<std::unique_ptr<awm::KeyTables>>     key_tables;
  std::vector<std::unique_ptr<awm::FrameModTable>> frame_mod_tables;
  std::vector<std::unique_ptr<awm::FrameModTemplate>> frame_mod_templates;
  std::vector<std::unique_ptr<awm::ResampleTable>> resample_tables;
  awm::ResampleTable *get_resample_table (int rate_in, int rate_out);
  awm::DevBuffer ws_rate_a, ws_rate_b, ws_rate_c;
  std::unique_ptr<awm::WorkLane> extra_lanes[awm::MAX_LANES - 1];
  awm::WorkLane *lane (int i);
  awm::FileStaging file_staging;
  awm::ReadyMarks ready;
  hipStream_t    copy_stream = nullptr;
  hipStream_t    get_copy_stream();
  std::vector<awm_ctx *> helpers;
  std::unique_ptr<awm::ParamValues> own_params;
  awm::DevBuffer ws_merge_soft;
  std::vector<hipEvent_t> merge_events;
  awm::DevBuffer    ws_add_batch;
  awm::PinnedBuffer pin_add_batch;
  hipEvent_t        ev_add_batch = nullptr;
  awm::DevBuffer ws_seg_in, ws_seg_out;
  awm::DevBuffer ws_key_tmpl;
  awm::DevBuffer ws_snr;
  bool           snr_on = false;
  int            chunk_lanes = awm::CHUNK_LANES;

  awm::SpeedWorkspace *speed = nullptr;
  std::mutex     speed_mutex;

  std::mutex     table_mutex;
  unsigned long  table_clock = 0;
  static constexpr size_t MAX_CACHED_TABLES = 64;
  std::mutex     prof_mutex;
  bool   prof_enabled = false;
  std::vector<awm::ProfPending> prof_pending;
  double prof_ms[awm::PROF_COUNT] = { 0 };
  long   prof_launches[awm::PROF_COUNT] = { 0 };
  double prof_bytes[awm::PROF_COUNT] = { 0 };
  void   prof_collect();

  awm::KeyTables     *get_key_tables (const awm::Key& key);
  awm::FrameModTable *get_frame_mod (const awm::Key& key, const std::string& payload_hex);
  awm::FrameModTemplate *get_frame_mod_template (const awm::Key& key);
};

#include "../../../include/awm_hip.h"

namespace awm {
struct ProfScope
{
  awm_ctx *ctx;
  int      id;
  hipEvent_t start = nullptr;
  hipStream_t st;
  ProfScope (awm_ctx *c, int i, double algorithmic_bytes, hipStream_t stream = nullptr) : ctx (c), id (i), st (stream ? stream : c->stream)
  {
    if (!ctx->prof_enabled)
      return;
    {
      std::lock_guard<std::mutex> lock (ctx->prof_mutex);
      ctx->prof_bytes[id] += algorithmic_bytes;
      ctx->prof_launches[id]++;
    }
    if (hipEventCreate (&start) != hipSuccess) { start = nullptr; return; }
    (void) hipEventRecord (start, st);
  }
  ~ProfScope()
  {
    if (!start)
// ... 10 lines not shown
```

audiowmark_amd/csrc/host/syncfinder.cc:

```cpp
#include "syncfinder.hh"
#include "utils.hh"
#include <algorithm>
#include <cmath>
#include <cstdlib>

namespace awm {

static inline int
total_frames (SyncFinder::Mode mode)
{
  return int (mark_block_frame_count()) * (mode == SyncFinder::Mode::CLIP ? 2 : 1);
}

int
SyncFinder::scan_silence (const DeviceWav& wav)
{
  if (int rc = prepare_launch (wav, Mode::CLIP))
    return rc;
  return prepare_finish();
}

int
SyncFinder::prepare_launch (const DeviceWav& wav, Mode mode, size_t scan_lo, size_t scan_hi)
{
  m_prepare_pending = false;
  if (mode != Mode::CLIP)
    {
      m_first = 0;
      m_last = wav.n_values();
      return 0;
    }
  if (int rc = m_lane->ws_misc.reserve (64)) return rc;
  if (int rc = m_lane->pin_small.reserve (64)) return rc;
  auto *res = m_lane->ws_misc.as<unsigned long long>();
  scan_hi = std::min (scan_hi, wav.n_values());
  scan_lo = std::min (scan_lo, scan_hi);
  AWM_HIP_CHECK (awmk::launch_nonzero_range (m_lane->stream, wav.data + scan_lo, (long long) (scan_hi - scan_lo), res));
  AWM_HIP_CHECK (hipMemcpyAsync (m_lane->pin_small.ptr, res, 2 * sizeof (unsigned long long), hipMemcpyDeviceToHost, m_lane->stream));
  m_prepare_values = wav.n_values();
  m_prepare_lo = scan_lo;
  m_prepare_pending = true;
  return 0;
}

int
SyncFinder::prepare_finish()
{
  if (!m_prepare_pending)
    return 0;
  m_prepare_pending = false;
  AWM_HIP_CHECK (stream_wait (m_lane->stream));
  const auto *h = m_lane->pin_small.as<unsigned long long>();
  const bool none = h[0] == ~0ULL;
  m_first = none ? m_prepare_values : m_prepare_lo + h[0];
  m_last = none ? m_prepare_values : m_prepare_lo + h[1];
  return 0;
}

int
SyncFinder::search_approx (KeyTables *kt, const DeviceWav& wav, Mode mode, std::vector<SearchScore>& out)
{
  out.clear();
  long long n_scores = 0;
  if (int rc = approx_device (kt, wav, mode, n_scores))
    return rc;
  return fetch_scores (n_scores, out);
}

int
SyncFinder::fetch_scores (long long n_scores, std::vector<SearchScore>& out)
{
  out.clear();
  if (n_scores <= 0)
    return 0;
  hipStream_t st = m_lane->stream;
  std::vector<double> raw (n_scores), mean (n_scores);
  AWM_HIP_CHECK (hipMemcpyAsync (raw.data(), m_lane->ws_raw.ptr, raw.size() * sizeof (double), hipMemcpyDeviceToHost, st));
  AWM_HIP_CHECK (hipMemcpyAsync (mean.data(), m_lane->ws_mean.ptr, mean.size() * sizeof (double), hipMemcpyDeviceToHost, st));
  AWM_HIP_CHECK (stream_wait (st));
  out.resize (raw.size());
  for (size_t p = 0; p < raw.size(); p++)
    {
      out[p].index = (p >> 2) * Params::frame_size + (p & 3) * Params::sync_search_step;
      out[p].raw_quality = raw[p];
      out[p].local_mean = mean[p];
// ... 262 lines not shown
      if (q >= q_last && q >= q_next)
        {
          selected.push_back (scores[i]);
          i++;
        }
    }
  scores.swap (selected);
}

void
SyncFinder::mask_avg_false_positives (std::vector<SearchScore>& scores)
{
  constexpr int    mask_distance = local_mean_distance + 3;
  constexpr double mask_factor = 3;
  auto sign = [] (const SearchScore& s) { return s.raw_quality - s.local_mean < 0 ? -1 : 1; };
  std::vector<SearchScore> kept;
  const int n = int (scores.size());
  for (int i = 0; i < n; i++)
    {
      bool mask = false;
      for (int d = -mask_distance; d <= mask_distance; d++)
        {
          const int j = i + d;
          if (j == i || j < 0 || j >= n)
            continue;
          const int distance = std::abs (int (scores[i].index) - int (scores[j].index)) / Params::sync_search_step;
          if (distance <= mask_distance
              && scores[j].abs_quality() > scores[i].abs_quality() * mask_factor
              && sign (scores[j]) != sign (scores[i]))
            mask = true;
        }
      if (!mask)
        kept.push_back (scores[i]);
    }
  scores.swap (kept);
}

void
SyncFinder::select_threshold_and_n_best (std::vector<SearchScore>& scores, double threshold)
{
  std::sort (scores.begin(), scores.end(), [] (const SearchScore& a, const SearchScore& b) { return a.abs_quality() > b.abs_quality(); });
  int i = 0;
  while (i < int (scores.size()) && scores[i].abs_quality() > threshold)
    i++;
  if (i >= params().get_n_best)
    scores.resize (i);
  else if (int (scores.size()) > params().get_n_best)
    scores.resize (params().get_n_best);
}

void
SyncFinder::select_truncate_n (std::vector<SearchScore>& scores, size_t n)
{
  std::sort (scores.begin(), scores.end(), [] (const SearchScore& a, const SearchScore& b) { return a.abs_quality() > b.abs_quality(); });
  if (scores.size() > n)
    scores.resize (n);
}

int
SyncFinder::search_refine (KeyTables *kt, const DeviceWav& wav, Mode mode, std::vector<SearchScore>& scores)
{
  SearchJob job;
  job.candidates = scores;
  if (int rc = refine_launch (kt, wav, mode, job))
    return rc;
  return refine_finish (job, scores);
}

namespace {
constexpr int REFINE_TP = 72;
constexpr int REFINE_TP_LINES = 64;
constexpr int REFINE_QS = 128;
}

int
SyncFinder::refine_launch (KeyTables *kt, const DeviceWav& wav, Mode mode, SearchJob& job)
{
  const int clip = mode == Mode::CLIP;
  const auto& sync = kt->sync[clip];
  const int NW = kt->slices ? kt->want_rows_of_slices() : int (sync.want_list.size());
  const size_t n_cand = job.candidates.size();
  job.refined.clear();
  job.batch_pending = false;
  if (!n_cand)
    return 0;
  const bool gathered = wav.n_channels <= 2;
  const int row_values = gathered ? 2 * int (Params::bands_per_frame) : Params::n_bands;
  const bool tail_layout = gathered && awmk::sliding_rows_have_tail (wav.n_channels);
  const size_t per_cand = size_t (NW) * row_values * (tail_layout ? REFINE_TP_LINES : REFINE_TP);
  const size_t tail_per_cand = tail_layout ? size_t (NW) * row_values : 0;
  size_t batch = std::max<size_t> (1, (size_t (job.slice_frames ? 12 : 3) << 30) / (per_cand * sizeof (float)));
  batch = std::min (batch, n_cand);
  if (int rc = m_lane->ws_refine.reserve (batch * (per_cand + tail_per_cand) * sizeof (float))) return rc;
  if (int rc = m_lane->ws_refine_have.reserve (batch * NW * REFINE_TP)) return rc;
  if (int rc = m_lane->ws_q.reserve (batch * (REFINE_QS * sizeof (double) + awmk::GATHERED_SCRATCH_BYTES_PER_PLANE))) return rc;
  if (int rc = m_lane->ws_idx.reserve (batch * NW * (sizeof (long long) + sizeof (int)) + 2 * batch * sizeof (int))) return rc;
  for (size_t c0 = 0; c0 < n_cand; c0 += batch)
    {
      if (job.batch_pending)
        if (int rc = refine_batch_finish (job))
          return rc;
      if (int rc = refine_batch_launch (kt, wav, mode, job, c0, std::min (batch, n_cand - c0), batch))
        return rc;
    }
  return 0;
}

int
SyncFinder::refine_batch_launch (KeyTables *kt, const DeviceWav& wav, Mode mode, SearchJob& job, size_t c0, size_t nb, size_t batch)
{
  const int clip = mode == Mode::CLIP;
  const auto& sync = kt->sync[clip];
  const int NW = kt->slices ? kt->want_rows_of_slices() : int (sync.want_list.size());
  const long long total = total_frames (mode);
  const int QS = REFINE_QS;
  hipStream_t st = m_lane->stream;
  const bool gathered = wav.n_channels <= 2;
  const int row_values = gathered ? 2 * int (Params::bands_per_frame) : Params::n_bands;
  const bool tail_layout = gathered && awmk::sliding_rows_have_tail (wav.n_channels);
  const int TP = tail_layout ? REFINE_TP_LINES : REFINE_TP;
  const int HP = REFINE_TP;
  const size_t per_cand = size_t (NW) * row_values * TP;
  const size_t tail_per_cand = tail_layout ? size_t (NW) * row_values : 0;
  float *const d_tail = tail_layout ? m_lane->ws_refine.as<float>() + batch * per_cand : nullptr;

  const size_t in_bytes = nb * NW * (sizeof (long long) + sizeof (int)) + 2 * nb * sizeof (int);
  const bool slices = job.slice_frames > 0;
  const long long span_frames = slices ? (long long) job.slice_frames : (long long) wav.n_frames;
  PinnedBuffer& pin_in = m_lane->pin_refine_in[job.slot];
  PinnedBuffer& pin_q = m_lane->pin_refine_q[job.slot];
  if (int rc = pin_in.reserve (in_bytes)) return rc;
  if (int rc = pin_q.reserve (nb * QS * sizeof (double))) return rc;
  auto *stream_base = pin_in.as<long long>();
  int *stream_count = reinterpret_cast<int *> (stream_base + nb * NW);
  int *lanes = stream_count + nb * NW;
  int *slice_of = lanes + nb;
  job.lane_count.assign (nb, 0);
  job.starts.assign (nb, 0);
  job.c0 = c0;
  job.nb = nb;
  int max_count = 0;
  long long n_items = 0;
  double db_bytes = 0;
  for (size_t c = 0; c < nb; c++)
    {
      const SearchScore& s = job.candidates[c0 + c];
      const int start = std::max (int (s.index) - Params::sync_search_step, 0);
      const int end = int (s.index) + Params::sync_search_step;
      const long long limit = span_frames - total * Params::frame_size;
      const long long slice0 = slices ? (long long) job.cand_slice[c0 + c] * span_frames : 0;
      slice_of[c] = slices ? job.cand_slice[c0 + c] : 0;
      int count = 0;
      for (int fine = start; fine <= end; fine += Params::sync_search_fine)
        if (fine <= limit)
          count++;
      job.starts[c] = start;
      job.lane_count[c] = lanes[c] = count;
      max_count = std::max (max_count, count);
      n_items += (long long) count * NW;
      if (count)
        db_bytes += double (NW) * ((1024.0 + 8.0 * (count - 1)) * 4 * wav.n_channels + 4.0 * row_values * count);
      const int *want_list = kt->slices ? kt->want_of_slice (job.cand_slice[c0 + c]) : sync.want_list.data();
      for (int w = 0; w < NW; w++)
        {
          stream_base[c * NW + w] = slice0 + start + (long long) want_list[w] * Params::frame_size;
          stream_count[c * NW + w] = count;
        }
    }
  auto *d_base = m_lane->ws_idx.as<long long>();
  int *d_count = reinterpret_cast<int *> (d_base + nb * NW);
  int *d_lanes = d_count + nb * NW;
  int *d_slice_of = d_lanes + nb;
  AWM_HIP_CHECK (hipMemcpyAsync (d_base, stream_base, in_bytes, hipMemcpyHostToDevice, st));

  double *q = pin_q.as<double>();
  std::fill (q, q + nb * QS, 0.0);
  if (max_count > 0)
    {
      awmk::SyncDbArgs da {};
      da.pcm = wav.data;
      da.n_frames = wav.n_frames;
      da.n_channels = wav.n_channels;
      da.per_channel = 0;
      da.stream_base = d_base;
      da.stream_count = d_count;
      da.count0 = max_count;
      da.n_streams = (long long) nb * NW;
      da.hop = Params::sync_search_fine;
      da.out = m_lane->ws_refine.as<float>();
      da.out_stream_stride = (long long) row_values * TP;
      if (gathered)
        {
          da.row_perm = sync.refine_perm.as<int>();
          da.band_pos = sync.refine_pos.as<unsigned char>();
          da.rows_per_plane = NW;
        }
      da.ld = TP;
      da.tail = d_tail;
      da.tail_stream_stride = row_values;
      da.have = m_lane->ws_refine_have.as<char>();
      da.have_stream_stride = HP;
      da.first = (long long) m_first;
      da.last = (long long) m_last;
      if (slices)
        {
          da.stream_range = job.slice_range;
          da.range_index = d_slice_of;
          da.range_div = NW;
          da.tables_per_slice = kt->slices ? 1 : 0;
        }
      da.tile_frames = TP;
      {
        ProfScope ps (m_ctx, PROF_REFINE_DB, (slices ? m_lane->prof_live_fraction : 1.0) * db_bytes, st);
        if (gathered)
          AWM_HIP_CHECK (awmk::launch_sync_db_sliding (st, m_ctx->tabs, da));
        else
          AWM_HIP_CHECK (awmk::launch_sync_db (st, m_ctx->tabs, da));
      }
      if (gathered)
        {
          awmk::GatheredScanArgs ga {};
          ga.db = m_lane->ws_refine.as<float>();
          ga.have = clip ? m_lane->ws_refine_have.as<char>() : nullptr;
          ga.plane_stride = (long long) per_cand;
          ga.have_plane_stride = (long long) NW * HP;
          ga.ld = TP;
          ga.have_ld = HP;
          ga.tail = d_tail;
          ga.tail_plane_stride = (long long) tail_per_cand;
          ga.rows_per_bit = sync.host.rows_per_bit;
          ga.n_lanes = max_count;
          ga.lane_count = d_lanes;
          ga.n_planes = (long long) nb;
          ga.min_delta = std::min (params().water_delta, 0.080);
          ga.quality = m_lane->ws_q.as<double>();
          ga.q_stride = QS;
          ga.chain_mag = reinterpret_cast<float *> (ga.quality + batch * QS);
          ga.chain_n = reinterpret_cast<int *> (ga.chain_mag + batch * 12 * 128);
          ProfScope ps (m_ctx, PROF_REFINE_SCAN, (slices ? m_lane->prof_live_fraction : 1.0) * double (n_items) * 4.0 * row_values, st);
          AWM_HIP_CHECK (awmk::launch_sync_scan_gathered (st, ga));
        }
      else
        {
          awmk::SyncScanArgs sa {};
          sa.db = m_lane->ws_refine.as<float>();
          sa.have = clip ? m_lane->ws_refine_have.as<char>() : nullptr;
          sa.plane_stride = (long long) per_cand;
          sa.have_plane_stride = (long long) NW * HP;
          sa.row_stride = (long long) Params::n_bands * TP;
          sa.band_stride = TP;
          sa.have_row_stride = HP;
          sa.n_lanes = max_count;
          sa.lane_count = d_lanes;
          sa.n_planes = (long long) nb;
          sa.min_delta = std::min (params().water_delta, 0.080);
          sa.quality = m_lane->ws_q.as<double>();
          sa.q_stride = QS;
          sa.table.packed = sync.packed_refine.as<int>();
          sa.table.rows_per_bit = sync.host.rows_per_bit;
          ProfScope ps (m_ctx, PROF_REFINE_SCAN, double (n_items) * 324.0, st);
          AWM_HIP_CHECK (awmk::launch_sync_scan (st, sa));
        }
      AWM_HIP_CHECK (hipMemcpyAsync (q, m_lane->ws_q.ptr, nb * QS * sizeof (double), hipMemcpyDeviceToHost, st));
    }
  hipEvent_t& ev = m_lane->ev_refine[job.slot];
  if (!ev)
    AWM_HIP_CHECK (hipEventCreateWithFlags (&ev, hipEventDisableTiming));
  AWM_HIP_CHECK (hipEventRecord (ev, st));
  job.batch_pending = true;
  return 0;
}

int
SyncFinder::refine_batch_finish (SearchJob& job)
{
  if (!job.batch_pending)
    return 0;
  AWM_HIP_CHECK (event_wait (m_lane->ev_refine[job.slot]));
  job.batch_pending = false;
  const double *q = m_lane->pin_refine_q[job.slot].as<double>();
  for (size_t c = 0; c < job.nb; c++)
    {
      const SearchScore& s = job.candidates[job.c0 + c];
      double best_quality = s.raw_quality;
      size_t best_index = s.index;
      for (int t = 0; t < job.lane_count[c]; t++)
        {
          const double qt = q[c * REFINE_QS + t];
          if (std::fabs (qt - s.local_mean) > std::fabs (best_quality - s.local_mean))
            {
              best_quality = qt;
              best_index = job.starts[c] + t * Params::sync_search_fine;
            }
        }
      job.refined.push_back ({ best_index, best_quality, s.local_mean });
    }
  return 0;
}

int
SyncFinder::refine_finish (SearchJob& job, std::vector<SearchScore>& scores)
{
  if (int rc = refine_batch_finish (job))
    return rc;
  std::stable_sort (job.refined.begin(), job.refined.end(), [] (const SearchScore& a, const SearchScore& b) { return a.index < b.index; });
  scores.swap (job.refined);
  job.refined.clear();
  return 0;
}

int
SyncFinder::prepare (const DeviceWav& wav, Mode mode)
{
  if (int rc = prepare_launch (wav, mode))
    return rc;
  return prepare_finish();
}

int
SyncFinder::search (const Key& key, const DeviceWav& wav, Mode mode, std::vector<Score>& out, bool db_ready)
{
  SearchJob job;
  if (int rc = search_launch (key, wav, mode, job, db_ready))
    return rc;
  return search_finish (job, out);
}

int
SyncFinder::search_launch (const Key& key, const DeviceWav& wav, Mode mode, SearchJob& job, bool db_ready)
{
  if (int rc = approx_launch (key, wav, mode, job,  db_ready, db_ready))
    return rc;
  return select_refine (job);
}

int
SyncFinder::approx_launch (const Key& key, const DeviceWav& wav, Mode mode, SearchJob& job, bool prepared, bool db_ready)
{
  job.out.clear();
  job.done = true;
  job.batch_pending = false;
  job.select_pending = false;
  KeyTables *kt = m_ctx->get_key_tables (key);
  if (!kt)
    return AWM_ERR_HIP;
  if (params().test_no_sync)
    {
      if (mode == Mode::BLOCK)
        {
          const size_t expect0 = Params::frames_pad_start * Params::frame_size;
          const size_t step = mark_block_frame_count() * Params::frame_size;
          const size_t end = (wav.n_frames / Params::frame_size) * Params::frame_size;
          int ab = 0;
          for (size_t idx = expect0; idx + step < end; idx += step)
            job.out.push_back ({ idx, 1.0, (ab++ & 1) ? ConvBlockType::b : ConvBlockType::a });
        }
      return 0;
    }
  if (!prepared)
    if (int rc = prepare (wav, mode))
      return rc;
  job.kt = kt;
  job.wav = wav;
  job.mode = mode;
  job.n_scores = 0;
  if (int rc = approx_device (kt, wav, mode, job.n_scores, db_ready))
    return rc;
  job.speculate_n_best = mode == Mode::CLIP;
  if (int rc = select_launch (job.n_scores, params().sync_threshold2 * 0.75, job.speculate_n_best))
    return rc;
  job.done = false;
  job.select_pending = true;
  return 0;
}

int
SyncFinder::select_refine (SearchJob& job)
{
  if (job.done || !job.select_pending)
    return 0;
  job.select_pending = false;
  if (int rc = select_finish (job.n_scores, params().sync_threshold2 * 0.75, job.candidates, job.speculate_n_best))
    return rc;
  if (job.mode == Mode::CLIP)
    select_truncate_n (job.candidates, std::max (params().get_n_best, 5));
  return refine_launch (job.kt, job.wav, job.mode, job);
}

int
SyncFinder::search_finish (SearchJob& job, std::vector<Score>& out)
{
  out.clear();
  if (job.done)
    {
      out = job.out;
      return 0;
    }
  std::vector<SearchScore> scores;
  if (int rc = refine_finish (job, scores))
    return rc;
  job.done = true;
  select_threshold_and_n_best (scores, params().sync_threshold2);
  std::sort (scores.begin(), scores.end(), [] (const SearchScore& a, const SearchScore& b) { return a.index < b.index; });
  for (const auto& s : scores)
    {
      const double q = s.raw_quality - s.local_mean;
      out.push_back ({ s.index, std::fabs (q), q > 0 ? ConvBlockType::a : ConvBlockType::b });
    }
  return 0;
}

void
SyncFinder::finish_scores (std::vector<SearchScore> scores, std::vector<Score>& out)
{
  out.clear();
  std::stable_sort (scores.begin(), scores.end(), [] (const SearchScore& a, const SearchScore& b) { return a.index < b.index; });
  select_threshold_and_n_best (scores, params().sync_threshold2);
  std::sort (scores.begin(), scores.end(), [] (const SearchScore& a, const SearchScore& b) { return a.index < b.index; });
  for (const auto& s : scores)
    {
      const double q = s.raw_quality - s.local_mean;
      out.push_back ({ s.index, std::fabs (q), q > 0 ? ConvBlockType::a : ConvBlockType::b });
    }
}


namespace {
constexpr unsigned int GROUP_HEAD = 32;
constexpr int GROUP_TOPK_SLICES = 4;
size_t align256 (size_t n) { return (n + 255) & ~size_t (255); }
struct GroupLayout
{
  size_t off_th, off_top, bytes;
  GroupLayout (int n_slices, int k)
  {
    off_th = align256 (size_t (n_slices) * 2 * sizeof (unsigned int));
    off_top = off_th + size_t (n_slices) * GROUP_HEAD * sizeof (awmk::PeakOut);
    bytes = off_top + size_t (n_slices) * GROUP_TOPK_SLICES * k * sizeof (awmk::PeakOut);
  }
};
}

int
SyncFinder::group_approx_launch (KeyTables *kt, const DeviceWav& group, int n_slices, const long long *d_range, GroupJob& gj, bool db_ready)
{
  gj.n_slices = n_slices;
  gj.kt = kt;
  gj.group = group;
  gj.slice_frames = n_slices > 0 ? group.n_frames / n_slices : 0;
  gj.n_scores = 0;
  gj.fallback.assign (std::max (n_slices, 0), 0);
  gj.refine = SearchJob();
  gj.refine.slice_frames = gj.slice_frames;
  gj.refine.slice_range = d_range;
  const Mode mode = Mode::CLIP;
  const long long frame_count = gj.slice_frames / Params::frame_size;
  const long long n_db = frame_count - 1;
  const long long S = n_db - total_frames (mode);
  const int k = params().get_n_best + 1;
  if (n_slices <= 0 || n_db <= 0 || S <= 0 || params().test_no_sync)
    return 0;
  if (gj.slice_frames % Params::frame_size || k > TOPK_MAX)
    {
      gj.fallback.assign (n_slices, 1);
      return 0;
    }
  hipStream_t st = m_lane->stream;
  const int n_shifts = Params::frame_size / Params::sync_search_step;
  const long long ld = (n_db + 63) & ~63LL;
  const long long plane = ld * Params::n_bands;
  const long long q_stride = (S + 63) & ~63LL;
  const long long n_planes = (long long) n_slices * n_shifts;
  const long long n_scores = (long long) n_shifts * S;
  if (int rc = m_lane->ws_db.reserve (size_t (n_planes) * plane * sizeof (float))) return rc;
  if (int rc = m_lane->ws_have.reserve (size_t (n_planes) * ld)) return rc;
  if (int rc = m_lane->ws_q.reserve (size_t (n_planes) * q_stride * sizeof (double))) return rc;
  if (int rc = m_lane->ws_raw.reserve (size_t (n_slices) * n_scores * sizeof (double))) return rc;
  if (int rc = m_lane->ws_mean.reserve (size_t (n_slices) * n_scores * sizeof (double))) return rc;

  awmk::SyncDbArgs da {};
  da.pcm = group.data;
  da.n_frames = group.n_frames;
  da.n_channels = group.n_channels;
  da.base0 = 0;
  da.base_stride = Params::sync_search_step;
  da.streams_per_slice = n_shifts;
  da.slice_stride = (long long) gj.slice_frames;
  da.stream_range = d_range;
  da.range_div = n_shifts;
  da.count0 = int (n_db);
// ... 137 lines not shown
```

audiowmark_amd/csrc/host/syncfinder.hh:

```
#pragma once
#include "context.hh"

namespace awm {

struct DeviceWav
{
  const float *data = nullptr;
  size_t       n_frames = 0;
  int          n_channels = 0;
  int          sample_rate = 44100;
  const int16_t *pcm16 = nullptr;
  size_t n_values() const { return n_frames * n_channels; }
};

class SyncFinder
{
public:
  enum class Mode { BLOCK, CLIP };
  struct Score
  {
    size_t        index;
    double        quality;
    ConvBlockType block_type;
  };
  struct SearchScore
  {
    size_t index;
    double raw_quality;
    double local_mean;
    double abs_quality() const { return std::fabs (raw_quality - local_mean); }
  };
  static constexpr int local_mean_distance = 20;

  explicit SyncFinder (awm_ctx *ctx, WorkLane *lane = nullptr) : m_ctx (ctx), m_lane (lane ? lane : ctx) {}
  hipEvent_t after_db_event = nullptr;
  hipEvent_t after_scan_event = nullptr;

  int search (const Key& key, const DeviceWav& wav, Mode mode, std::vector<Score>& out, bool db_ready = false);
  int prepare (const DeviceWav& wav, Mode mode);
  int prepare_launch (const DeviceWav& wav, Mode mode, size_t scan_lo = 0, size_t scan_hi = size_t (-1));
  int prepare_finish();
  int search_approx (KeyTables *kt, const DeviceWav& wav, Mode mode, std::vector<SearchScore>& out);
  int approx_device (KeyTables *kt, const DeviceWav& wav, Mode mode, long long& n_scores, bool db_ready = false, bool scores_only = false);
  int scores_loaded (long long n_start_frames);
  int select_candidates (long long n_scores, double threshold, std::vector<SearchScore>& out);
  int select_launch (long long n_scores, double threshold, bool speculate_n_best = false);
  int select_finish (long long n_scores, double threshold, std::vector<SearchScore>& out, bool speculated = false);
  int search_refine (KeyTables *kt, const DeviceWav& wav, Mode mode, std::vector<SearchScore>& scores);

  struct SearchJob
  {
    int    slot = 0;
    bool   done = true;
    std::vector<Score> out;
    std::vector<SearchScore> candidates, refined;
    std::vector<int> lane_count, starts;
    size_t c0 = 0, nb = 0;
    bool   batch_pending = false;
    KeyTables *kt = nullptr;
    DeviceWav  wav;
    Mode       mode = Mode::BLOCK;
    long long  n_scores = 0;
    bool       select_pending = false;
    bool       speculate_n_best = false;
    std::vector<int> cand_slice;
    size_t           slice_frames = 0;
    const long long *slice_range = nullptr;
  };
  int search_launch (const Key& key, const DeviceWav& wav, Mode mode, SearchJob& job, bool db_ready = false);
  int search_finish (SearchJob& job, std::vector<Score>& out);
  int approx_launch (const Key& key, const DeviceWav& wav, Mode mode, SearchJob& job, bool prepared = false, bool db_ready = false);
  int select_refine (SearchJob& job);


  struct GroupJob
  {
    int        n_slices = 0;
    size_t     slice_frames = 0;
    long long  n_scores = 0;
    KeyTables *kt = nullptr;
    DeviceWav  group;
    SearchJob  refine;
    std::vector<char> fallback;
  };
  int group_approx_launch (KeyTables *kt, const DeviceWav& group, int n_slices, const long long *d_range, GroupJob& gj, bool db_ready = false);
  int group_select_refine (GroupJob& gj);
  int group_finish (GroupJob& gj, std::vector<std::vector<Score>>& out);

  int refine_launch (KeyTables *kt, const DeviceWav& wav, Mode mode, SearchJob& job);
  int refine_collect (SearchJob& job) { return refine_batch_finish (job); }
  static void finish_scores (std::vector<SearchScore> refined, std::vector<Score>& out);

  static void select_local_maxima (std::vector<SearchScore>& scores);
  static void mask_avg_false_positives (std::vector<SearchScore>& scores);
  static void select_threshold_and_n_best (std::vector<SearchScore>& scores, double threshold);
  static void select_truncate_n (std::vector<SearchScore>& scores, size_t n);
private:
  awm_ctx  *m_ctx;
  WorkLane *m_lane;
  size_t   m_first = 0, m_last = 0;
  size_t   m_prepare_values = 0, m_prepare_lo = 0;
  bool     m_prepare_pending = false;
  int scan_silence (const DeviceWav& wav);
  int fetch_scores (long long n_scores, std::vector<SearchScore>& out);
  int refine_batch_launch (KeyTables *kt, const DeviceWav& wav, Mode mode, SearchJob& job, size_t c0, size_t nb, size_t batch);
  int refine_batch_finish (SearchJob& job);
  int refine_finish (SearchJob& job, std::vector<SearchScore>& scores);
};

}
```

audiowmark_amd/csrc/host/wmdecode.hh:

```
#pragma once
#include "wmget.hh"

namespace awm {

struct PatternRawBits
{
  size_t        index;
  double        quality;
  int           slot;
  ConvBlockType block_type;
};

struct PendingDecode
{
  ConvBlockType      code_type;
  int                mode;
  std::vector<std::pair<int, int>> src;
  int                norm0, norm1;
  double             time;
  SyncFinder::Score  score;
  ResultSet::Type    type;
  size_t             chunk = 0;
  int                order_off = 0;
};

struct DecodeJob
{
  std::vector<PendingDecode> pending;
  std::vector<size_t> which[3];
  size_t nb[3] = { 0, 0, 0 }, bits_off[3] = { 0, 0, 0 }, err_off[3] = { 0, 0, 0 };
  size_t bits_total = 0, err_total = 0, n_out = 0;
  bool   launched = false;
};

struct BlockDbView { unsigned int fill; float *planes_out; };
int block_soft_bits_dev (awm_ctx *ctx, WorkLane *lane, KeyTables *kt, const DeviceWav& wav, const std::vector<size_t>& index,
                         std::vector<int>& slot_of, std::vector<char>& ok, const long long *slice_range = nullptr, size_t slice_frames = 0,
                         const BlockDbView *view = nullptr);
long long block_plane_ld();
awmk::SyncDbArgs block_db_args (const DeviceWav& wav, const long long *d_bases, const int *d_slice_of, size_t nb, float *planes,
                                const long long *slice_range, size_t slice_frames);
awmk::SoftBitsArgs block_soft_args (KeyTables *kt, int n_channels, const float *planes, size_t nb, float *out, const long long *d_bases,
                                    const int *d_slice_of, const long long *slice_range, bool slices);
int decode_launch (awm_ctx *ctx, WorkLane *lane, KeyTables *kt, DecodeJob& job, const float *raw = nullptr);
struct DecodedPattern { size_t pending_index; std::vector<int> bits; float error; };
int decode_finish (WorkLane *lane, const Key& key, DecodeJob& job, const std::vector<ResultSet *>& result_sets, double speed,
                   std::vector<DecodedPattern> *patterns_out = nullptr);
void combine_blocks (const std::vector<PatternRawBits>& pattern_raw_vec, const DeviceWav& wav, size_t chunk, std::vector<PendingDecode>& pending);

int decode_chunks_blocks_only (awm_ctx *ctx, const std::vector<Key>& key_list, const DeviceWav& wav, const std::vector<ChunkRange>& chunks,
                               std::vector<ResultSet>& chunk_sets, std::string *debug_sync_first, int lane_base = 0);

int decode_speed_chunk (awm_ctx *ctx, WorkLane *lane, ResultSet& result_set, const std::vector<Key>& key_list, const DeviceWav& chunk_wav,
                        bool first_chunk, std::string *report);

}
```

audiowmark_amd/csrc/host/wmget.cc:

```cpp
#include "wmget.hh"
#include "wmdecode.hh"
#include "wmspeed.hh"
#include "keytab_stage.hh"
#include <atomic>
#include <functional>
#include <future>
#include <chrono>
#include <memory>
#include <thread>
#include "utils.hh"
#include <algorithm>
#include <cmath>
#include <map>
#include <optional>

namespace awm {
int g_key_tables_on_device = 1;


std::vector<float>
normalize_soft_bits (const std::vector<float>& soft_bits)
{
  std::vector<float> norm;
  norm.reserve (soft_bits.size());
// ... 59 lines not shown
  sb.db = planes;
  sb.block_stride = (long long) n_channels * Params::n_bands * ld;
  sb.ld = ld;
  sb.n_channels = n_channels;
  sb.mix_frame = kt->mix_frame.as<int16_t>();
  sb.mix_up = kt->mix_up.as<uint8_t>();
  sb.mix_down = kt->mix_down.as<uint8_t>();
  sb.n_data_frames = mark_data_frame_count();
  sb.frames_per_bit = params().frames_per_bit;
  sb.block_frames = int (mark_block_frame_count());
  sb.n_blocks = (long long) nb;
  sb.out = out;
  if (kt->slices && slices)
    sb.block_slice = d_slice_of;
  if (slice_range && slices)
    {
      sb.block_base = d_bases;
      sb.stream_range = slice_range;
      sb.range_index = d_slice_of;
    }
  return sb;
}

int
block_soft_bits_dev (awm_ctx *ctx, WorkLane *lane, KeyTables *kt, const DeviceWav& wav, const std::vector<size_t>& index,
                     std::vector<int>& slot_of, std::vector<char>& ok, const long long *slice_range, size_t slice_frames,
                     const BlockDbView *view)
{
  const size_t count = mark_block_frame_count();
  const int n_bits = mark_data_frame_count() / params().frames_per_bit;
  const int C = wav.n_channels;
  slot_of.assign (index.size(), -1);
  ok.assign (index.size(), 0);
  std::vector<long long> bases;
  for (size_t i = 0; i < index.size(); i++)
    if (wav.n_values() >= (index[i] + count * Params::frame_size) * C)
      {
        ok[i] = 1;
        slot_of[i] = int (bases.size());
        bases.push_back ((long long) index[i]);
      }
  if (bases.empty())
    return 0;
  hipStream_t st = lane->stream;
  const long long block_stride = (long long) C * Params::n_bands * block_plane_ld();
  const size_t max_batch = std::max<size_t> (1, (size_t (2) << 30) / (block_stride * sizeof (float)));
  if (int rc = lane->ws_soft.reserve (bases.size() * n_bits * sizeof (float))) return rc;
  const size_t idx_bytes = bases.size() * (sizeof (long long) + sizeof (int));
  if (int rc = lane->ws_idx.reserve (idx_bytes)) return rc;
  if (int rc = lane->pin_blocks.reserve (idx_bytes)) return rc;
  std::copy (bases.begin(), bases.end(), lane->pin_blocks.as<long long>());
  int *slice_of = reinterpret_cast<int *> (lane->pin_blocks.as<long long>() + bases.size());
  for (size_t i = 0; i < bases.size(); i++)
    slice_of[i] = slice_frames ? int (size_t (bases[i]) / slice_frames) : 0;
  AWM_HIP_CHECK (hipMemcpyAsync (lane->ws_idx.ptr, lane->pin_blocks.ptr, idx_bytes, hipMemcpyHostToDevice, st));
  const long long *d_bases = lane->ws_idx.as<long long>();
  const int *d_slice_of = reinterpret_cast<const int *> (d_bases + bases.size());
  const bool padded = slice_range && slice_frames;
  for (size_t b0 = 0; b0 < bases.size(); b0 += max_batch)
    {
      const size_t nb = std::min (max_batch, bases.size() - b0);
      if (int rc = lane->ws_block_db.reserve (nb * block_stride * sizeof (float))) return rc;
      float *planes = lane->ws_block_db.as<float>();
      if (view)
        AWM_HIP_CHECK (awmk::launch_fill_u32 (st, reinterpret_cast<unsigned int *> (planes), view->fill, nb * block_stride));
      const awmk::SyncDbArgs da = block_db_args (wav, d_bases + b0, d_slice_of + b0, nb, planes, slice_range, slice_frames);
      {
        ProfScope ps (ctx, PROF_BLOCK_DB, (padded ? lane->prof_live_fraction : 1.0) * double (nb) * count * C * (4096.0 + 324.0), st);
        AWM_HIP_CHECK (awmk::launch_sync_db (st, ctx->tabs, da));
      }
      const awmk::SoftBitsArgs sb = block_soft_args (kt, C, planes, nb, lane->ws_soft.as<float>() + b0 * n_bits, d_bases + b0, d_slice_of + b0,
                                                     slice_range, slice_frames != 0);
      {
        ProfScope ps (ctx, PROF_SOFT_BITS, (padded ? lane->prof_live_fraction : 1.0) * double (nb) * count * C * 324.0, st);
        AWM_HIP_CHECK (awmk::launch_soft_bits (st, sb));
      }
      if (view)
        AWM_HIP_CHECK (hipMemcpyAsync (view->planes_out + b0 * block_stride, planes, nb * block_stride * sizeof (float), hipMemcpyDeviceToDevice, st));
    }
  return 0;
}

int
block_soft_bits (awm_ctx *ctx, KeyTables *kt, const DeviceWav& wav, const std::vector<size_t>& index,
                 std::vector<std::vector<float>>& raw_bits, std::vector<char>& ok)
{
  const int n_bits = mark_data_frame_count() / params().frames_per_bit;
  std::vector<int> slot_of;
  raw_bits.assign (index.size(), {});
  if (int rc = block_soft_bits_dev (ctx, ctx, kt, wav, index, slot_of, ok))
    return rc;
  size_t n_slots = 0;
  for (int sl : slot_of)
    n_slots = std::max (n_slots, size_t (sl + 1));
  if (!n_slots)
    return 0;
  std::vector<float> host (n_slots * n_bits);
  AWM_HIP_CHECK (hipMemcpyAsync (host.data(), ctx->ws_soft.ptr, host.size() * sizeof (float), hipMemcpyDeviceToHost, ctx->stream));
  AWM_HIP_CHECK (stream_wait (ctx->stream));
  for (size_t i = 0; i < index.size(); i++)
    if (slot_of[i] >= 0)
      raw_bits[i].assign (host.begin() + size_t (slot_of[i]) * n_bits, host.begin() + size_t (slot_of[i] + 1) * n_bits);
  return 0;
}

int
viterbi_check_errors (WorkLane *lane, const float *errors, size_t n)
{
  for (size_t i = 0; i < n; i++)
    if (errors[i] <= -1.5f)
      {
        if (lane->ws_viterbi_sync.ptr)
          (void) hipMemsetAsync (lane->ws_viterbi_sync.ptr, 0, lane->ws_viterbi_sync.bytes, lane->stream);
        set_error (std::string ("viterbi: a device-side wait between the workgroups of a decode timed out; ") + awmk::viterbi_form_description()
                   + " -- awm_debug_set_viterbi_persistent (0) selects the launch chain");
        return AWM_ERR_HIP;
      }
  return 0;
}

int
viterbi_decode_all (awm_ctx *ctx, const std::vector<std::vector<float>> soft[3], std::vector<std::vector<int>> bits[3],
                    std::vector<float> errors[3])
{
  size_t n_steps = 0;
  bool have_steps = false;
  for (int t = 0; t < 3; t++)
    {
      bits[t].assign (soft[t].size(), {});
      errors[t].assign (soft[t].size(), 0.f);
      const size_t rate = t == 2 ? 12 : 6;
      for (const auto& v : soft[t])
        {
          if (v.size() % rate || (have_steps && v.size() / rate != n_steps))
            {
              set_error ("viterbi_decode: ragged batch (a coded length that is no multiple of the rate, or blocks of different lengths)");
              return AWM_ERR_ARG;
            }
          n_steps = v.size() / rate;
          have_steps = true;
        }
    }
  if (soft[0].empty() && soft[1].empty() && soft[2].empty())
    return 0;
  if (!awmk::viterbi_steps_supported ((long long) std::min<size_t> (n_steps, 1u << 20)))
    {
      set_error ("viterbi_decode: " + std::to_string (n_steps) + " trellis steps per block; the decoder takes 15 (the termination alone) up to 256 (64 rounds of 4)");
      return AWM_ERR_ARG;
    }
  hipStream_t st = ctx->stream;
  const size_t n_out = n_steps - conv_order;
  const size_t max_batch = 512;
  size_t done[3] = { 0, 0, 0 };
  while (done[0] < soft[0].size() || done[1] < soft[1].size() || done[2] < soft[2].size())
    {
      size_t nb[3], in_off[3], ws_off[3], bits_off[3], err_off[3];
      size_t in_total = 0, ws_total = 0, bits_total = 0, err_total = 0;
      for (int t = 0; t < 3; t++)
        {
          const size_t rate = t == 2 ? 12 : 6;
          nb[t] = std::min (max_batch, soft[t].size() - done[t]);
          in_off[t] = in_total;    in_total += nb[t] * n_steps * rate;
          ws_off[t] = ws_total;    ws_total += awmk::viterbi_workspace_bytes (n_steps * rate, rate, nb[t]);
          bits_off[t] = bits_total; bits_total += nb[t] * n_out;
          err_off[t] = err_total;  err_total += nb[t];
        }
// ... 242 lines not shown

  static ConvBlockType other (ConvBlockType t) { return t == ConvBlockType::a ? ConvBlockType::b : ConvBlockType::a; }

  std::vector<size_t>
  chain_from (size_t start) const
  {
    const long long half_frame = Params::frame_size / 2;
    const long long last_gap = lrint (blocks.back().index / double (block_len) + 0.5);
    std::vector<size_t> chain { start };
    for (long long gap = 1; gap <= last_gap; )
      {
        const PatternRawBits& tail = blocks[chain.back()];
        const ConvBlockType type = (gap & 1) ? other (tail.block_type) : tail.block_type;
        const size_t next = nearest (chain.back(), blocks.size(), type, (long long) tail.index + gap * block_len, gap * half_frame);
        if (next == NO_BLOCK)
          gap++;
        else
          {
            chain.push_back (next);
            gap = 1;
          }
      }
    return chain;
  }

  float
  quality_sum (const std::vector<size_t>& chain) const
  {
    float sum = 0;
    for (size_t pos : chain)
      sum += blocks[pos].quality;
    return sum;
  }
};

}

void
combine_blocks (const std::vector<PatternRawBits>& raw_blocks, const DeviceWav& wav, size_t chunk, std::vector<PendingDecode>& pending)
{
  const BlockList list { raw_blocks, (long long) (mark_block_frame_count() * Params::frame_size) };
  for (size_t pos = 0; pos < raw_blocks.size(); pos++)
    {
      const PatternRawBits& b = raw_blocks[pos];
      if (b.block_type != ConvBlockType::b)
        continue;
      const size_t partner = list.nearest (0, pos, ConvBlockType::a, (long long) b.index - list.block_len, Params::frame_size / 2);
      if (partner == NO_BLOCK)
        continue;
      const PatternRawBits& a = raw_blocks[partner];
      const SyncFinder::Score score { b.index, (a.quality + b.quality) / 2, ConvBlockType::ab };
      pending.push_back ({ ConvBlockType::ab, 1, { { a.slot, 0 }, { b.slot, 1 } }, 0, 0, double (b.index) / wav.sample_rate, score,
                           ResultSet::Type::BLOCK, chunk });
    }
  std::vector<size_t> best;
  float best_sum = 0;
  for (size_t start = 0; start < raw_blocks.size(); start++)
    {
      std::vector<size_t> chain = list.chain_from (start);
      const float sum = list.quality_sum (chain);
      if (sum > best_sum)
        {
          best = std::move (chain);
          best_sum = sum;
        }
    }
  if (best.size() < 2)
    return;
  PendingDecode all { ConvBlockType::ab, 2, {}, 0, 0, 0.0, { 0, 0, ConvBlockType::a }, ResultSet::Type::ALL, chunk };
  for (size_t pos : best)
    {
      const PatternRawBits& blk = raw_blocks[pos];
      const int ab = blk.block_type == ConvBlockType::b;
      all.src.push_back ({ blk.slot, ab });
      (ab ? all.norm1 : all.norm0)++;
      all.score.quality += blk.quality;
    }
  all.score.quality /= all.norm0 + all.norm1;
  pending.push_back (std::move (all));
}

int g_merge_decodes = 0;
extern "C" void awm_debug_set_merge_decodes (int on) { g_merge_decodes = on; }
int g_chunk_stagger = -1;
extern "C" void awm_debug_set_chunk_stagger (int on) { g_chunk_stagger = on; }
int g_speed_overlap = 1;
extern "C" void awm_debug_set_speed_overlap (int on) { g_speed_overlap = on; }
namespace {

int
block_decoder_run (awm_ctx *ctx, WorkLane *home, bool spread, const std::vector<Key>& key_list, const DeviceWav& stream,
                   const std::vector<ChunkRange>& chunks, const std::vector<ResultSet *>& result_sets, double speed,
                   std::string *debug_sync_first_chunk, int lane_base = 0)
{
  const size_t count = mark_block_frame_count();
  std::vector<SyncFinder::Score> first_scores;
  const int n_lanes = !spread ? 1 : int (std::min<size_t> (chunks.size(), size_t (std::max (1, std::min (ctx->chunk_lanes, CHUNK_LANES)))));
  std::vector<WorkLane *> lanes;
  if (!spread)
    lanes.push_back (home);
  else
    for (int i = 0; i < std::max (n_lanes, 1); i++)
      {
        WorkLane *l = ctx->lane (lane_base + i);
        if (!l)
          {
            set_error ("cannot create a work lane (stream)");
            return AWM_ERR_HIP;
          }
        lanes.push_back (l);
      }
  ReadyMarks *marks = (spread && lane_base == 0 && lanes.size() > 1 && ctx->ready.armed && ctx->ready.base == stream.data
                       && ctx->ready.n_frames == stream.n_frames && (ctx->ready.live || !ctx->ready.marks.empty())) ? &ctx->ready : nullptr;
  if (marks && !marks->live)
    std::rotate (lanes.begin(), lanes.begin() + 1, lanes.end());
  else if (lanes.size() > 1 && lane_base == 0)
    {
      if (!ctx->ev_sync)
        AWM_HIP_CHECK (hipEventCreateWithFlags (&ctx->ev_sync, hipEventDisableTiming));
      AWM_HIP_CHECK (hipEventRecord (ctx->ev_sync, ctx->stream));
      for (size_t i = 1; i < lanes.size(); i++)
        AWM_HIP_CHECK (hipStreamWaitEvent (lanes[i]->stream, ctx->ev_sync, 0));
    }
  auto wait_for_mark = [&] (WorkLane *lane, size_t last_sample_plus_one) -> int {
    if (!marks)
      return 0;
    if (marks->live)
      {
        std::unique_lock<std::mutex> lock (marks->mu);
        marks->cv.wait (lock, [&] { return marks->live_done || (!marks->marks.empty() && marks->marks.back().first >= last_sample_plus_one); });
        hipEvent_t ev = nullptr;
        for (const auto& m : marks->marks)
          if (m.first >= last_sample_plus_one)
            {
              ev = m.second;
              break;
            }
        if (!ev && !marks->marks.empty())
          ev = marks->marks.back().second;
        lock.unlock();
        if (ev)
          AWM_HIP_CHECK (hipStreamWaitEvent (lane->stream, ev, 0));
        return 0;
      }
    if (lane->stream == ctx->stream)
      return 0;
    for (const auto& m : marks->marks)
      if (m.first >= last_sample_plus_one)
        {
          AWM_HIP_CHECK (hipStreamWaitEvent (lane->stream, m.second, 0));
          return 0;
        }
    AWM_HIP_CHECK (hipStreamWaitEvent (lane->stream, marks->marks.back().second, 0));
    return 0;
  };
  struct LaneDrain
  {
    const std::vector<WorkLane *>& lanes;
    bool ok = false;
    ~LaneDrain()
    {
      if (!ok)
        for (WorkLane *l : lanes)
          (void) hipStreamSynchronize (l->stream);
    }
  } drain { lanes };
  auto chunk_wav = [&] (size_t c) {
    DeviceWav cw = stream;
    cw.data = stream.data + chunks[c].first_frame * stream.n_channels;
    cw.n_frames = chunks[c].n_frames;
    return cw;
  };
  struct ChunkState
  {
    size_t c;
    WorkLane *lane;
    size_t ki = 0;
    int stage = 0;
    std::unique_ptr<SyncFinder> finder;
    SyncFinder::SearchJob job;
    DecodeJob decode;
  };
  std::vector<ChunkState> active;
  std::vector<char> lane_busy (lanes.size(), 0);
  size_t next_chunk = 0;
  const int n_soft_bits = mark_data_frame_count() / params().frames_per_bit;
  struct Deferred
  {
    DecodeJob job;
    std::vector<hipEvent_t> rows_ready;
  };
  std::vector<Deferred> deferred (key_list.size());
  size_t merge_rows = 0, merge_capacity = 0;
  if (g_merge_decodes && chunks.size() > 1 && chunks.size() <= size_t (CHUNK_LANES))
    {
      for (const auto& c : chunks)
        merge_capacity += 2 * (c.n_frames / (count * Params::frame_size) + 4);
      merge_capacity *= key_list.size();
      if (ctx->ws_merge_soft.reserve (merge_capacity * n_soft_bits * sizeof (float)))
        merge_capacity = 0;
    }
  size_t merge_events_used = 0;
  std::vector<hipEvent_t> stagger_events (chunks.size(), nullptr);
  struct EventsFree { std::vector<hipEvent_t>& ev; ~EventsFree() { for (hipEvent_t e : ev) if (e) (void) hipEventDestroy (e); } } stagger_free { stagger_events };
  auto advance = [&] (ChunkState& cs) -> int {
    const Key& key = key_list[cs.ki];
    KeyTables *kt = ctx->get_key_tables (key);
    if (!kt)
      return AWM_ERR_HIP;
    if (!cs.finder)
      cs.finder = std::make_unique<SyncFinder> (ctx, cs.lane);
    SyncFinder& finder = *cs.finder;
    const size_t c = cs.c;
    switch (cs.stage)
      {
      case 0:
        {
          if (cs.ki == 0)
            if (int rc = wait_for_mark (cs.lane, chunks[c].first_frame + chunks[c].n_frames))
              return rc;
          const int stagger = g_chunk_stagger >= 0 ? g_chunk_stagger : (chunks.size() > lanes.size() ? 2 : 1);
          if (stagger && cs.ki == 0 && spread)
            {
              if (c > 0 && stagger_events[c - 1])
                AWM_HIP_CHECK (hipStreamWaitEvent (cs.lane->stream, stagger_events[c - 1], 0));
              if (c + 1 < chunks.size())
                {
                  AWM_HIP_CHECK (hipEventCreateWithFlags (&stagger_events[c], hipEventDisableTiming));
                  (stagger == 2 ? finder.after_scan_event : finder.after_db_event) = stagger_events[c];
                }
            }
          if (int rc = finder.approx_launch (key, chunk_wav (c), SyncFinder::Mode::BLOCK, cs.job,  false,  cs.ki > 0))
            return rc;
          finder.after_db_event = finder.after_scan_event = nullptr;
          cs.stage = 1;
          return 0;
        }
      case 1:
        if (int rc = finder.select_refine (cs.job))
          return rc;
        cs.stage = 2;
        return 0;
      case 2:
        {
          std::vector<SyncFinder::Score> scores;
          if (int rc = finder.search_finish (cs.job, scores))
            return rc;
          if (cs.ki == 0 && c == 0)
            first_scores = scores;
          std::vector<size_t> wanted;
          std::vector<const SyncFinder::Score *> wanted_score;
          for (const auto& sc : scores)
            if (chunks[c].n_frames >= sc.index + count * Params::frame_size)
              {
                wanted.push_back (chunks[c].first_frame + sc.index);
                wanted_score.push_back (&sc);
              }
          std::vector<int> slot_of;
          std::vector<char> ok;
          if (int rc = block_soft_bits_dev (ctx, cs.lane, kt, stream, wanted, slot_of, ok))
            return rc;
          std::vector<PatternRawBits> pattern_raw_vec;
          cs.decode = DecodeJob();
          auto& pending = cs.decode.pending;
          for (size_t w = 0; w < wanted.size(); w++)
            {
              if (!ok[w])
                continue;
              const SyncFinder::Score& sc = *wanted_score[w];
              PatternRawBits rb;
              rb.index = sc.index;
              rb.quality = sc.quality;
              rb.slot = slot_of[w];
              rb.block_type = sc.block_type;
              pending.push_back ({ rb.block_type, 0, { { rb.slot, 0 } }, 0, 0, double (rb.index) / stream.sample_rate,
                                   sc, ResultSet::Type::BLOCK, c });
              pattern_raw_vec.push_back (rb);
            }
          combine_blocks (pattern_raw_vec, stream, c, pending);
          size_t n_rows = 0;
          for (size_t w = 0; w < wanted.size(); w++)
            if (ok[w])
              n_rows = std::max (n_rows, size_t (slot_of[w]) + 1);
          if (merge_rows + n_rows <= merge_capacity && !pending.empty())
            {
              hipStream_t st = cs.lane->stream;
              AWM_HIP_CHECK (hipMemcpyAsync (ctx->ws_merge_soft.as<float>() + merge_rows * n_soft_bits, cs.lane->ws_soft.ptr,
                                             n_rows * n_soft_bits * sizeof (float), hipMemcpyDeviceToDevice, st));
              if (merge_events_used == ctx->merge_events.size())
                {
                  hipEvent_t e = nullptr;
                  AWM_HIP_CHECK (hipEventCreateWithFlags (&e, hipEventDisableTiming));
                  ctx->merge_events.push_back (e);
                }
              hipEvent_t ev = ctx->merge_events[merge_events_used++];
              AWM_HIP_CHECK (hipEventRecord (ev, st));
              Deferred& d = deferred[cs.ki];
              d.rows_ready.push_back (ev);
              for (auto& p : pending)
                {
                  for (auto& sp : p.src)
                    sp.first += int (merge_rows);
                  d.job.pending.push_back (std::move (p));
                }
              merge_rows += n_rows;
              cs.decode = DecodeJob();
              cs.ki++;
              cs.stage = cs.ki < key_list.size() ? 0 : 4;
              return 0;
            }
          if (int rc = decode_launch (ctx, cs.lane, kt, cs.decode))
            return rc;
          cs.stage = 3;
          return 0;
        }
      default:
        if (int rc = decode_finish (cs.lane, key, cs.decode, result_sets, speed))
          return rc;
        cs.ki++;
        cs.stage = cs.ki < key_list.size() ? 0 : 4;
        return 0;
      }
  };
  while (next_chunk < chunks.size() || !active.empty())
    {
      bool progressed = false;
      auto chunk_is_loaded = [&] (size_t c) {
        if (!marks || !marks->live)
          return true;
        std::lock_guard<std::mutex> lock (marks->mu);
        return marks->live_done || (!marks->marks.empty() && marks->marks.back().first >= chunks[c].first_frame + chunks[c].n_frames);
      };
      while (next_chunk < chunks.size() && !lane_busy[next_chunk % lanes.size()] && !key_list.empty() && chunk_is_loaded (next_chunk))
        {
          ChunkState cs;
          cs.c = next_chunk;
          cs.lane = lanes[next_chunk % lanes.size()];
          lane_busy[next_chunk % lanes.size()] = 1;
          active.push_back (std::move (cs));
          if (int rc = advance (active.back()))
            return rc;
          next_chunk++;
          progressed = true;
        }
      if (key_list.empty())
        break;
      for (auto& cs : active)
        {
          if (cs.stage >= 1 && cs.stage <= 3 && (active.size() == 1 || hipStreamQuery (cs.lane->stream) != hipErrorNotReady))
            {
              if (int rc = advance (cs))
                return rc;
              if (cs.stage == 0)
                if (int rc = advance (cs))
                  return rc;
              progressed = true;
            }
        }
      for (size_t i = 0; i < active.size(); )
        if (active[i].stage == 4)
          {
            lane_busy[active[i].c % lanes.size()] = 0;
            active.erase (active.begin() + i);
            progressed = true;
          }
        else
          i++;
      if (!progressed)
        {
          if (marks && marks->live && active.empty() && next_chunk < chunks.size())
            {
              std::unique_lock<std::mutex> lock (marks->mu);
              const size_t need = chunks[next_chunk].first_frame + chunks[next_chunk].n_frames;
              marks->cv.wait_for (lock, std::chrono::milliseconds (2),
                                  [&] { return marks->live_done || (!marks->marks.empty() && marks->marks.back().first >= need); });
            }
          else
            std::this_thread::yield();
        }
    }
  for (size_t ki = 0; ki < key_list.size(); ki++)
    {
      Deferred& d = deferred[ki];
      if (d.job.pending.empty())
        continue;
      KeyTables *kt = ctx->get_key_tables (key_list[ki]);
      if (!kt)
        return AWM_ERR_HIP;
      WorkLane *lane = lanes[0];
      for (hipEvent_t ev : d.rows_ready)
        AWM_HIP_CHECK (hipStreamWaitEvent (lane->stream, ev, 0));
      if (int rc = decode_launch (ctx, lane, kt, d.job, ctx->ws_merge_soft.as<float>()))
        return rc;
      if (int rc = decode_finish (lane, key_list[ki], d.job, result_sets, speed))
        return rc;
    }
  drain.ok = true;
  if (debug_sync_first_chunk)
    {
      debug_sync_first_chunk->clear();
      if (key_list.size() == 1 && !chunks.empty())
        {
          const int expect0 = Params::frames_pad_start * Params::frame_size;
          const int expect_step = count * Params::frame_size;
          const int expect_end = int (chunks[0].n_frames / Params::frame_size) * Params::frame_size;
          int sync_match = 0;
          for (int expect_index = expect0; expect_index + expect_step < expect_end; expect_index += expect_step)
            for (const auto& s : first_scores)
              if (std::abs (int (s.index + params().test_cut) - expect_index) < int (Params::frame_size / 2))
                {
                  sync_match++;
                  break;
                }
          *debug_sync_first_chunk = string_printf ("sync_match %d %zd\n", sync_match, first_scores.size());
        }
    }
  return 0;
}


int
clip_run_padded (awm_ctx *ctx, WorkLane *lane, const std::vector<Key>& key_list, const DeviceWav& wav, ResultSet& result_set,
                 double time_offset_sec, double speed)
{
  SyncFinder sync_finder (ctx, lane);
  const size_t count = mark_block_frame_count();
  for (size_t ki = 0; ki < key_list.size(); ki++)
    {
      const Key& key = key_list[ki];
      KeyTables *kt = ctx->get_key_tables (key);
      if (!kt)
        return AWM_ERR_HIP;
// ... 1303 lines not shown
```

include/awm_hip.h:

```cpp
#ifndef AWM_HIP_H
#define AWM_HIP_H

#include <stddef.h>
#include <stdint.h>

#ifdef __cplusplus
extern "C" {
#endif

#define AWM_ERR_GENERIC    (-1)
#define AWM_ERR_NO_DEVICE  (-2)
#define AWM_ERR_ARG        (-3)
#define AWM_ERR_HIP        (-4)
#define AWM_ERR_IO         (-5)

#define AWM_FRAME_SIZE      1024
#define AWM_N_BANDS         81
#define AWM_BLOCK_FRAMES    2226
#define AWM_SOFT_BITS       858

typedef struct awm_ctx awm_ctx;

const char *awm_last_error (void);
const char *awm_version (void);
// ... 245 lines not shown
int awm_multi_get_d (awm_ctx *const *ctxs, int n_ctx, const uint8_t key[16], const float *const *pcm_d, int n_channels,
                     const uint64_t *span_frames, size_t max_out, awm_pattern *out);

int awm_multi_add_watermark_batch_d (awm_ctx *const *ctxs, int n_ctx, const int *ctx_of_clip, const uint8_t *keys, const uint8_t *one_key,
                                     const char *payload_hex, size_t n_clips, const float *const *pcm_in_d, float *const *out_d,
                                     const size_t *n_frames, int n_channels);
int awm_multi_get_watermark_batch_d (awm_ctx *const *ctxs, int n_ctx, const int *ctx_of_clip, const uint8_t *keys, const uint8_t *one_key,
                                     size_t n_clips, const float *const *pcm_d, const size_t *n_frames, int n_channels,
                                     size_t max_out_per_clip, awm_pattern *out, int *n_out);

int awm_ctx_set_helpers (awm_ctx *ctx, awm_ctx *const *helpers, int n_helpers);

void awm_set_speed_params (int detect_speed, int detect_speed_patient, double try_speed, double test_speed);
size_t awm_resample_ratio_frames (size_t n_frames, int n_channels, int rate, double ratio, double max_in_seconds);
int awm_resample_ratio_d (awm_ctx *ctx, const float *pcm_in_d, size_t n_frames, int n_channels, int rate, double ratio,
                          double max_in_seconds, float *out_d, size_t n_out_frames);
int awm_detect_speed_d (awm_ctx *ctx, const uint8_t key[16], const float *pcm_d, size_t n_frames, int n_channels, int rate,
                        int patient, double *speed_out, double *quality_out);
int awm_speed_clip_location_d (awm_ctx *ctx, const uint8_t key[16], const float *pcm_d, size_t n_frames, int n_channels, int rate,
                               double seconds, int candidates, double *location);
int awm_speed_mags_d (awm_ctx *ctx, const uint8_t key[16], const float *pcm_d, size_t n_frames, int n_channels, int rate,
                      double clip_location, double center, double seconds, size_t max_rows, float *out);
int awm_speed_scan_d (awm_ctx *ctx, const uint8_t key[16], const float *pcm_d, size_t n_frames, int n_channels, int rate,
                      double clip_location, double seconds, double step, int n_steps, int n_center_steps,
                      const double *speeds, int n_speeds, size_t max_out, double *out_speed, double *out_quality);

int  awm_detect_speed_batch_d (awm_ctx *ctx, const uint8_t *keys, int key_per_clip, size_t n_clips, const float *const *pcm_d,
                               const size_t *n_frames, int n_channels, int rate, int patient, double *speed_out, double *quality_out,
                               int *use_out);
void awm_debug_set_speed_batch_bytes (size_t bytes);
size_t awm_debug_speed_batch_bytes (void);
int  awm_speed_batch_plan (size_t n_clips, const size_t *n_frames, int n_channels, int rate, int patient, size_t budget_bytes,
                           int *group_of_clip, size_t *bytes_of_group);
void awm_debug_speed_batch_launches (int *k12, int *k13, int *k14, int *k15);
void awm_debug_set_speed_batch (int mode);
int  awm_debug_speed_scan_batch_d (awm_ctx *ctx, const uint8_t *keys, int key_per_clip, size_t n_clips, const float *const *pcm_d,
                                   const size_t *n_frames, int n_channels, int rate, const double *clip_locations, double seconds,
                                   double step, int n_steps, int n_center_steps, const double *speeds, const int *n_speeds,
                                   size_t max_out_per_clip, double *out_speed, double *out_quality, int *n_out);

int    awm_speed_select_n_best (double *speed, double *quality, int count, int n);
double awm_speed_smooth_best (const double *speed, const double *quality, int count, double step, double distance);
size_t awm_speed_clip_positions (const uint8_t key[16], size_t n_values, size_t max_out, uint64_t *positions);
int    awm_speed_clip_candidates (const uint8_t key[16], const float *hashed_values, size_t n, int candidates, double *locations);
int    awm_var_resample_table (double ratio, float *out, size_t max_floats, int *hl);

void awm_debug_set_viterbi_super (int on);
void awm_debug_set_viterbi_persistent (int on);
double awm_debug_dependent_launch_us (void);
int  awm_debug_viterbi_one_launch_in_use (void);
void awm_debug_set_sliding3 (int on);
void awm_debug_set_refine_form (int form);
int  awm_debug_refine_form (void);
void awm_debug_set_k4s_ablate (int flags);
int  awm_debug_sync_db_sliding_d (awm_ctx *ctx, const float *pcm_d, size_t n_frames, int n_channels, const long long *base_d, size_t n_streams,
                                  int count, int ld, float *out_d);
int  awm_debug_sync_db_sliding_rows_d (awm_ctx *ctx, const float *pcm_d, size_t n_frames, int n_channels, const long long *base_d, const int *count_d,
                                       size_t n_streams, int count0, int rows_per_plane, const int *row_perm_d, const unsigned char *band_pos_d,
                                       long long first, long long last, const long long *stream_range_d, const int *range_index_d, int range_div,
                                       int tables_per_slice, int ld, float *out_d, float *tail_d, long long tail_stream_stride, char *have_d,
                                       long long have_stream_stride);
void awm_debug_set_soft_bits_generic (int on);
int  awm_debug_block_plane_ld (awm_ctx *ctx);
int  awm_debug_block_db_d (awm_ctx *ctx, const uint8_t key[16], const float *pcm_d, size_t n_frames, int n_channels, const uint64_t *index,
                           size_t n_blocks, uint32_t fill, const long long *slice_range_d, size_t n_slices, size_t slice_frames,
                           float *planes_out_d, size_t planes_values, float *soft_out, int *slot_out);
int  awm_debug_soft_bits_planes_d (awm_ctx *ctx, const uint8_t key[16], const float *planes_d, size_t planes_values, size_t n_blocks, int n_channels,
                                   const long long *block_base_d, const long long *slice_range_d, const int *range_index_d, size_t n_slices,
                                   float *soft_out);
void awm_debug_set_scan_generic (int on);
int  awm_debug_scan_generic_launches (void);
void awm_debug_set_chunk_stagger (int mode);
void awm_debug_set_resample_phase (int on);
int  awm_debug_resample_span_d (awm_ctx *ctx, const float *in_d, size_t n_in, uint64_t in0, uint64_t out0, size_t n_out, int n_channels,
                                int rate_in, int rate_out, float *out_d, int *phase_form_used);
void awm_debug_set_get_overlap (int on);
void awm_debug_set_speed_compare_wide (int on);
void awm_debug_set_speed_compare_fold (int on);
void awm_debug_set_resample_var_mode (int mode);
void awm_debug_set_speed_overlap (int on);
int  awm_debug_frame_mod_tables_d (awm_ctx *ctx, const uint8_t *keys, size_t n_keys, const char *payload_hex, int8_t *tables_out);
int  awm_debug_clip_key_tables_check_d (awm_ctx *ctx, const uint8_t *keys, size_t n_keys, long long mismatch_out[9]);
void awm_debug_set_key_tables_on_device (int on);
void awm_debug_set_merge_decodes (int on);
void awm_debug_set_add_batched (int on);
void awm_debug_set_add_slab_mb (int mb);
void awm_debug_set_add_payloads_fused (int on);
int  awm_debug_add_payloads_fused_in_use (void);
void awm_debug_set_add_payloads_rate_fused (int mode);
int  awm_debug_add_payloads_rate_fused_in_use (void);
int  awm_debug_add_segments_fused_in_use (void);
int  awm_debug_payload_tables_d (awm_ctx *ctx, const uint8_t key[16], const char *const *payload_hex, size_t n_payloads, int8_t *tables_out);
int  awm_debug_key_templates_d (awm_ctx *ctx, const uint8_t *keys, size_t n_keys, int16_t *out);
int  awm_debug_key_payload_tables_d (awm_ctx *ctx, const uint8_t *keys, const char *const *payload_hex, size_t n, int8_t *tables_out);
void awm_debug_set_payloads_file_tile (int frames1024);
int  awm_debug_add_payloads_tile (void);
void awm_debug_set_fft_pair (int on);
void awm_debug_set_clip_poison (int on);
size_t awm_debug_clip_slice_values (int n_channels);
int  awm_debug_clip_stage_d (awm_ctx *ctx, size_t n_clips, const float *const *pcm_d, const size_t *n_frames, int n_channels, int sample_rate,
                             float *slices_d, long long *range_out);
int  awm_debug_clip_stage_rates_d (awm_ctx *ctx, size_t n_clips, const float *const *pcm_d, const size_t *n_frames, int n_channels,
                                   const int *sample_rates, float *slices_d, long long *range_out);
int  awm_debug_clip_stage_rates_s16_d (awm_ctx *ctx, size_t n_clips, const int16_t *const *pcm_d, const size_t *n_frames, int n_channels,
                                       const int *sample_rates, float *slices_d, long long *range_out);
void awm_debug_clip_form_launches (long out[3]);
size_t awm_debug_lane_pcm_bytes (awm_ctx *ctx);
void awm_debug_set_clip_pad_margin (int frames);
void awm_debug_set_staged_threads (int n);
void awm_debug_clip_key_timing (double us_out[3]);
double awm_debug_time_group_key_tables (int n_keys, int threads);
void awm_debug_set_group_fallback (int on);
void awm_debug_alloc_stats (long *dev_allocs, double *dev_ms, long *pinned_allocs, double *pinned_ms);
unsigned long long awm_debug_alloc_bytes (void);
void awm_debug_file_timing (double ms_out[8]);
void awm_debug_set_io_flags (int flags);

void awm_set_io_threads (int n);

void awm_set_quiet (int quiet);

void awm_set_params (double water_delta, int mix, int frames_per_bit, int test_no_limiter,
                     double sync_threshold2, int n_best, double chunk_size_min);
typedef struct
{
  size_t struct_size;
  double water_delta;
  int    mix;
  int    hard;
  int    strict;
  int    snr;
  int    payload_size;
  int    frames_per_bit;
  double sync_threshold2;
  int    get_n_best;
  double get_chunk_size;
  int    detect_speed, detect_speed_patient;
  double try_speed, test_speed;
  int    test_cut, test_no_sync, test_no_limiter, test_truncate;
} awm_params;
void awm_params_init (awm_params *p);
int  awm_set_global_params (const awm_params *p);
int  awm_ctx_set_params (awm_ctx *ctx, const awm_params *p);
int  awm_ctx_get_params (const awm_ctx *ctx, awm_params *out);

int  awm_ctx_snr_begin (awm_ctx *ctx);
int  awm_ctx_snr_end (awm_ctx *ctx, double *signal_power, double *delta_power);

#ifdef __cplusplus
}
#endif
#endif
```

Baseline: 726,500 xRT.

## Queue block decode behind sync refine using on-device best-offset selection

Adds a device-side selection step in the sync quality kernel that picks each candidate's best refined offset and writes the block base and a live count. Soft-bit extraction for candidate blocks can then be queued right behind the refine batch, on a second stream and gated by events, instead of waiting for a host round trip to choose offsets. Dead blocks are skipped in the soft-bits kernels. This adds extra streams, events and a fallback path for when host and device selections disagree, and it may do speculative work on candidates that are later rejected.

```diff
diff --git a/audiowmark_amd/binding.py b/audiowmark_amd/binding.py
--- a/audiowmark_amd/binding.py
+++ b/audiowmark_amd/binding.py
@@ -211,6 +211,14 @@
 lib.awm_debug_block_db_d.argtypes = [_vp, _vp, _vp, C.c_size_t, C.c_int, _vp, C.c_size_t, C.c_uint32, _vp, C.c_size_t, C.c_size_t, _vp, C.c_size_t,
                                      _vp, _vp]
 lib.awm_debug_soft_bits_planes_d.argtypes = [_vp, _vp, _vp, C.c_size_t, C.c_size_t, C.c_int, _vp, _vp, _vp, C.c_size_t, _vp]
+lib.awm_debug_decode_behind_d.argtypes = [_vp, _vp, _vp, C.c_size_t, C.c_int, C.c_size_t, _vp, _vp, _vp, _vp, _vp, _vp, C.c_longlong, C.c_longlong,
+                                          C.c_longlong, C.c_uint32, _vp, C.c_size_t, _vp, _vp, _vp]
+lib.awm_debug_set_decode_behind_refine.argtypes = [C.c_int]
+lib.awm_debug_set_decode_behind_refine.restype = None
+lib.awm_debug_set_decode_behind_split.argtypes = [C.c_int]
+lib.awm_debug_set_decode_behind_split.restype = None
+lib.awm_debug_decode_behind_counts.argtypes = [_vp, C.c_int]
+lib.awm_debug_decode_behind_counts.restype = None
 lib.awm_get_watermark_file.argtypes = [_vp, _vp, C.c_char_p, C.POINTER(RawFormat), C.c_size_t, _vp]
 lib.awm_add_get_watermark_file.argtypes = [_vp, _vp, C.c_char_p, C.c_char_p, C.c_char_p, C.POINTER(RawFormat), C.POINTER(RawFormat), C.c_size_t, _vp]
 lib.awm_add_stream_create.argtypes = [_vp, _vp, C.c_char_p, C.c_int, C.c_size_t, C.POINTER(_vp)]
@@ -1315,6 +1323,36 @@
                                                 _np(soft)), "awm_debug_soft_bits_planes_d")
         return soft[:n_blocks]
 
+    def debug_decode_behind(self, quality, n_offsets, raw_quality, local_mean, index, start, chunk_first, chunk_frames, stream_frames,
+                            key=None, pcm=None, fill=0x7FC00000):
+        import torch
+        quality = np.ascontiguousarray(quality, np.float64)
+        n = quality.shape[0]
+        assert quality.shape == (n, 128)
+        n_offsets = np.ascontiguousarray(n_offsets, np.int32)
+        raw_quality, local_mean = np.ascontiguousarray(raw_quality, np.float64), np.ascontiguousarray(local_mean, np.float64)
+        index, start = np.ascontiguousarray(index, np.int64), np.ascontiguousarray(start, np.int64)
+        assert all(len(a) == n for a in (n_offsets, raw_quality, local_mean, index, start))
+        base, count = np.zeros(n, np.int64), np.zeros(n, np.int32)
+        planes = soft = None
+        n_frames = ch = 0
+        if pcm is not None:
+            n_frames, ch = _pcm_shape(pcm)
+            planes = torch.empty((n, ch, N_BANDS, self.block_plane_ld()), dtype=torch.float32, device=pcm.device)
+            soft = np.zeros(2 * n * SOFT_BITS, np.float32)
+        _check(lib.awm_debug_decode_behind_d(self._h, key_bytes(key), _dev_ptr(pcm) if pcm is not None else None, n_frames, ch, n, _np(quality),
+                                             _np(n_offsets), _np(raw_quality), _np(local_mean), _np(index), _np(start), chunk_first, chunk_frames,
+                                             stream_frames, fill, _dev_ptr(planes) if planes is not None else None,
+                                             planes.numel() if planes is not None else 0, _np(soft) if soft is not None else None,
+                                             _np(base), _np(count)), "awm_debug_decode_behind_d")
+        return (base, count) if pcm is None else (base, count, planes, soft[:n * SOFT_BITS].reshape(n, SOFT_BITS))
+
+    @staticmethod
+    def decode_behind_counts(reset=False):
+        out = (C.c_longlong * 4)()
+        lib.awm_debug_decode_behind_counts(out, 1 if reset else 0)
+        return tuple(out)
+
     def viterbi_decode(self, block_type, soft):
         soft = np.ascontiguousarray(soft, np.float32)
         if soft.ndim == 1:
diff --git a/audiowmark_amd/csrc/hip/kernels.hh b/audiowmark_amd/csrc/hip/kernels.hh
--- a/audiowmark_amd/csrc/hip/kernels.hh
+++ b/audiowmark_amd/csrc/hip/kernels.hh
@@ -269,6 +269,12 @@
 hipError_t launch_sync_scan (hipStream_t st, const SyncScanArgs& a);
 hipError_t launch_sync_scan_window (hipStream_t st, const SyncScanArgs& a, int total_frames);
 
+struct RefineSelectIn
+{
+  double    raw_quality, local_mean;
+  long long index;
+  long long start;
+};
 struct GatheredScanArgs
 {
   const float *db;
@@ -288,9 +294,19 @@
   float       *chain_mag;
   int         *chain_n;
   int          regular_waves, tail_first, tail_lanes;
+  const RefineSelectIn *select = nullptr;
+  long long    select_chunk_first = 0;
+  long long    select_chunk_frames = 0;
+  long long    select_stream_frames = 0;
+  long long    select_block_samples = 0;
+  int          select_block_frames = 0;
+  int          select_fine = 8;
+  long long   *select_base = nullptr;
+  int         *select_count = nullptr;
 };
 constexpr size_t GATHERED_SCRATCH_BYTES_PER_PLANE = 18 * 128 * 4;
 hipError_t launch_sync_scan_gathered (hipStream_t st, const GatheredScanArgs& a);
+hipError_t launch_refine_select_only (hipStream_t st, const GatheredScanArgs& a);
 
 hipError_t launch_local_mean (hipStream_t st, const double *q, long long q_stride, long long n_start_frames,
                               double *raw_sorted, double *local_mean, int n_slices = 1);
@@ -321,6 +337,7 @@
   const long long *block_base = nullptr;
   const long long *stream_range = nullptr;
   const int       *range_index = nullptr;
+  const int       *block_live = nullptr;
 };
 hipError_t launch_soft_bits (hipStream_t st, const SoftBitsArgs& a);
 bool soft_bits_skips_silent_items (int n_channels, int frames_per_bit);
diff --git a/audiowmark_amd/csrc/hip/kernels.hip b/audiowmark_amd/csrc/hip/kernels.hip
--- a/audiowmark_amd/csrc/hip/kernels.hip
+++ b/audiowmark_amd/csrc/hip/kernels.hip
@@ -3482,34 +3482,65 @@
     }
 }
 
-__global__ void __launch_bounds__ (64)
+template<bool COMPUTE> __global__ void __launch_bounds__ (128)
 sync_quality_kernel (GatheredScanArgs a)
 {
+  __shared__ double s_q[128];
   const long long plane = blockIdx.y;
-  const int cand = blockIdx.x * 64 + threadIdx.x;
-  if (cand >= a.lane_count[plane])
+  const int cand = threadIdx.x;
+  const int count = min (a.lane_count[plane], 128);
+  if (cand < count)
+    {
+      double q = 0;
+      if (COMPUTE)
+        {
+          int total = 0;
+          for (int b = 0; b < 6; b++)
+            {
+              const float um = a.chain_mag[(plane * 12 + 2 * b) * 128 + cand], dm = a.chain_mag[(plane * 12 + 2 * b + 1) * 128 + cand];
+              const int n = a.chain_n[(plane * 6 + b) * 128 + cand];
+              float raw;
+              if (um == 0 || dm == 0)
+                raw = 0;
+              else if (um < dm)
+                raw = __fsub_rn (1.f, __fdiv_rn (um, dm));
+              else
+                raw = __fsub_rn (__fdiv_rn (dm, um), 1.f);
+              const double rb = (b & 1) ? double (raw) : -double (raw);
+              q += rb * n;
+              total += n;
+            }
+          if (total)
+            q /= total;
+          q = q / a.min_delta / 2.9;
+          a.quality[plane * a.q_stride + cand] = q;
+        }
+      else
+        q = a.quality[plane * a.q_stride + cand];
+      s_q[cand] = q;
+    }
+  if (!a.select)
     return;
-  double q = 0;
-  int total = 0;
-  for (int b = 0; b < 6; b++)
-    {
-      const float um = a.chain_mag[(plane * 12 + 2 * b) * 128 + cand], dm = a.chain_mag[(plane * 12 + 2 * b + 1) * 128 + cand];
-      const int n = a.chain_n[(plane * 6 + b) * 128 + cand];
-      float raw;
-      if (um == 0 || dm == 0)
-        raw = 0;
-      else if (um < dm)
-        raw = __fsub_rn (1.f, __fdiv_rn (um, dm));
-      else
-        raw = __fsub_rn (__fdiv_rn (dm, um), 1.f);
-      const double rb = (b & 1) ? double (raw) : -double (raw);
-      q += rb * n;
-      total += n;
-    }
-  if (total)
-    q /= total;
-  q = q / a.min_delta / 2.9;
-  a.quality[plane * a.q_stride + cand] = q;
+  __syncthreads();
+  if (threadIdx.x == 0)
+    {
+      const RefineSelectIn s = a.select[plane];
+      double best_quality = s.raw_quality;
+      long long best_index = s.index;
+      for (int t = 0; t < count; t++)
+        {
+          const double qt = s_q[t];
+          if (fabs (qt - s.local_mean) > fabs (best_quality - s.local_mean))
+            {
+              best_quality = qt;
+              best_index = s.start + (long long) t * a.select_fine;
+            }
+        }
+      const bool live = a.select_chunk_frames >= best_index + a.select_block_samples
+                        && a.select_stream_frames >= a.select_chunk_first + best_index + a.select_block_samples;
+      a.select_base[plane] = a.select_chunk_first + best_index;
+      a.select_count[plane] = live ? a.select_block_frames : 0;
+    }
 }
 
 hipError_t
@@ -3517,7 +3548,7 @@
 {
   if (a0.n_lanes <= 0 || a0.n_planes <= 0)
     return hipSuccess;
-  if (!a0.lane_count || a0.n_planes > 65535 || a0.n_lanes > 128 || !a0.chain_mag || !a0.chain_n)
+  if (!a0.lane_count || a0.n_planes > 65535 || a0.n_lanes > 128 || !a0.chain_mag || !a0.chain_n || (a0.select && (!a0.select_base || !a0.select_count)))
     return hipErrorInvalidValue;
   GatheredScanArgs a = a0;
   const int full = a.n_lanes / 64, rem = a.n_lanes % 64;
@@ -3530,7 +3561,18 @@
     hipLaunchKernelGGL (sync_scan_gathered_kernel<true>, grid, dim3 (64), 0, st, a);
   else
     hipLaunchKernelGGL (sync_scan_gathered_kernel<false>, grid, dim3 (64), 0, st, a);
-  hipLaunchKernelGGL (sync_quality_kernel, dim3 (unsigned ((a.n_lanes + 63) / 64), unsigned (a.n_planes)), dim3 (64), 0, st, a);
+  hipLaunchKernelGGL (sync_quality_kernel<true>, dim3 (1, unsigned (a.n_planes)), dim3 (128), 0, st, a);
+  return hipGetLastError();
+}
+
+hipError_t
+launch_refine_select_only (hipStream_t st, const GatheredScanArgs& a)
+{
+  if (a.n_planes <= 0)
+    return hipSuccess;
+  if (!a.lane_count || a.n_planes > 65535 || a.n_lanes < 0 || a.n_lanes > 128 || !a.quality || !a.select || !a.select_base || !a.select_count)
+    return hipErrorInvalidValue;
+  hipLaunchKernelGGL (sync_quality_kernel<false>, dim3 (1, unsigned (a.n_planes)), dim3 (128), 0, st, a);
   return hipGetLastError();
 }
 
@@ -3581,7 +3623,7 @@
   const long long blk = blockIdx.y;
   const int bit = blockIdx.x * blockDim.x + threadIdx.x;
   const int n_bits = a.n_data_frames / a.frames_per_bit;
-  if (bit >= n_bits)
+  if (bit >= n_bits || (a.block_live && !a.block_live[blk]))
     return;
   const float *db = a.db + blk * a.block_stride;
   const int C = a.n_channels;
@@ -3622,7 +3664,7 @@
   const long long slot = blockIdx.x >> 3;
   const long long blk = (slot / groups_per_block) * 8 + (blockIdx.x & 7);
   const int group = int (slot % groups_per_block);
-  if (blk >= a.n_blocks)
+  if (blk >= a.n_blocks || (a.block_live && !a.block_live[blk]))
     return;
   const int n_bits = a.n_data_frames / a.frames_per_bit;
   const int bit0 = (group * SB_WAVES + wave) * SB_BPW;
diff --git a/audiowmark_amd/csrc/host/capi_kernels.cc b/audiowmark_amd/csrc/host/capi_kernels.cc
--- a/audiowmark_amd/csrc/host/capi_kernels.cc
+++ b/audiowmark_amd/csrc/host/capi_kernels.cc
@@ -1766,6 +1766,94 @@
   AWM_HIP_CHECK (awmk::launch_soft_bits (ctx->stream, sb));
   AWM_HIP_CHECK (hipMemcpyAsync (soft_out, ctx->ws_soft.ptr, n_blocks * n_bits * sizeof (float), hipMemcpyDeviceToHost, ctx->stream));
   AWM_HIP_CHECK (stream_wait (ctx->stream));
+  return 0;
+}
+
+int
+awm_debug_decode_behind_d (awm_ctx *ctx, const uint8_t key[16], const float *pcm_d, size_t n_frames, int n_channels, size_t n_cand,
+                           const double *quality, const int *n_offsets, const double *raw_quality, const double *local_mean,
+                           const long long *index, const long long *start, long long chunk_first, long long chunk_frames,
+                           long long stream_frames, uint32_t fill, float *planes_out_d, size_t planes_values, float *soft_out,
+                           long long *base_out, int *count_out)
+{
+  AWM_ENTER (ctx);
+  constexpr int QS = 128;
+  const size_t block_values = size_t (std::max (n_channels, 0)) * Params::n_bands * size_t (block_plane_ld());
+  const char *bad = nullptr;
+  if (!quality || !n_offsets || !raw_quality || !local_mean || !index || !start || !base_out || !count_out)
+    bad = "null pointer";
+  else if (n_cand < 1 || n_cand > DEBUG_BLOCKS_MAX)
+    bad = "1 .. 64 candidates";
+  else if (chunk_first < 0 || chunk_frames < 0 || stream_frames < 0 || chunk_first > DEBUG_RANGE_MAX || chunk_frames > DEBUG_RANGE_MAX
+           || stream_frames > DEBUG_RANGE_MAX)
+    bad = "chunk or stream out of range";
+  else if (pcm_d && (n_channels < 1 || n_channels > 2 || !planes_out_d || !soft_out || planes_values / block_values < n_cand))
+    bad = "with samples: 1 or 2 channels, planes_out_d for n_cand blocks and soft_out";
+  else if (pcm_d && size_t (stream_frames) > n_frames)
+    bad = "the stream is longer than the samples";
+  for (size_t i = 0; i < n_cand && !bad; i++)
+    if (n_offsets[i] < 0 || n_offsets[i] > QS || index[i] < 0 || start[i] < 0 || index[i] > DEBUG_RANGE_MAX || start[i] > DEBUG_RANGE_MAX)
+      bad = "a candidate's offsets, index or start is out of range";
+  if (bad)
+    {
+      set_error (std::string ("awm_debug_decode_behind_d: ") + bad);
+      return AWM_ERR_ARG;
+    }
+  hipStream_t st = ctx->stream;
+  const size_t q_bytes = n_cand * QS * sizeof (double), sel_bytes = n_cand * sizeof (awmk::RefineSelectIn);
+  const size_t in_bytes = q_bytes + sel_bytes + n_cand * sizeof (int), out_bytes = n_cand * (sizeof (long long) + sizeof (int));
+  if (int rc = ctx->ws_q.reserve (in_bytes)) return rc;
+  if (int rc = ctx->ws_block_base.reserve (out_bytes)) return rc;
+  if (int rc = ctx->pin_small.reserve (in_bytes + out_bytes)) return rc;
+  char *pin = ctx->pin_small.as<char>();
+  std::memcpy (pin, quality, q_bytes);
+  auto *sel = reinterpret_cast<awmk::RefineSelectIn *> (pin + q_bytes);
+  int max_offsets = 0;
+  for (size_t i = 0; i < n_cand; i++)
+    {
+      sel[i] = { raw_quality[i], local_mean[i], index[i], start[i] };
+      max_offsets = std::max (max_offsets, n_offsets[i]);
+    }
+  std::memcpy (pin + q_bytes + sel_bytes, n_offsets, n_cand * sizeof (int));
+  AWM_HIP_CHECK (hipMemcpyAsync (ctx->ws_q.ptr, pin, in_bytes, hipMemcpyHostToDevice, st));
+  awmk::GatheredScanArgs ga {};
+  ga.quality = ctx->ws_q.as<double>();
+  ga.q_stride = QS;
+  ga.n_lanes = max_offsets;
+  ga.n_planes = (long long) n_cand;
+  ga.select = reinterpret_cast<const awmk::RefineSelectIn *> (ctx->ws_q.as<char>() + q_bytes);
+  ga.lane_count = reinterpret_cast<const int *> (ctx->ws_q.as<char>() + q_bytes + sel_bytes);
+  ga.select_chunk_first = chunk_first;
+  ga.select_chunk_frames = chunk_frames;
+  ga.select_stream_frames = stream_frames;
+  ga.select_block_samples = (long long) (mark_block_frame_count() * Params::frame_size);
+  ga.select_block_frames = int (mark_block_frame_count());
+  ga.select_fine = Params::sync_search_fine;
+  ga.select_base = ctx->ws_block_base.as<long long>();
+  ga.select_count = reinterpret_cast<int *> (ga.select_base + n_cand);
+  AWM_HIP_CHECK (awmk::launch_refine_select_only (st, ga));
+  AWM_HIP_CHECK (hipMemcpyAsync (pin + in_bytes, ctx->ws_block_base.ptr, out_bytes, hipMemcpyDeviceToHost, st));
+  const size_t n_bits = mark_data_frame_count() / params().frames_per_bit;
+  if (pcm_d)
+    {
+      KeyTables *kt = ctx->get_key_tables (capi_key (key));
+      if (!kt)
+        return AWM_ERR_HIP;
+      bool fits = false;
+      if (int rc = block_soft_bits_reserve (ctx, n_channels, n_cand, fits)) return rc;
+      if (!fits)
+        return AWM_ERR_ARG;
+      AWM_HIP_CHECK (awmk::launch_fill_u32 (st, ctx->ws_block_db.as<unsigned int>(), fill, n_cand * block_values));
+      AWM_HIP_CHECK (awmk::launch_fill_u32 (st, ctx->ws_soft.as<unsigned int>(), fill, n_cand * n_bits));
+      if (int rc = block_soft_bits_queued (ctx, ctx, kt, make_wav (pcm_d, size_t (stream_frames), n_channels), ga.select_base, ga.select_count, 0,
+                                           n_cand, st))
+        return rc;
+      AWM_HIP_CHECK (hipMemcpyAsync (planes_out_d, ctx->ws_block_db.ptr, n_cand * block_values * sizeof (float), hipMemcpyDeviceToDevice, st));
+      AWM_HIP_CHECK (hipMemcpyAsync (soft_out, ctx->ws_soft.ptr, n_cand * n_bits * sizeof (float), hipMemcpyDeviceToHost, st));
+    }
+  AWM_HIP_CHECK (stream_wait (st));
+  std::memcpy (base_out, pin + in_bytes, n_cand * sizeof (long long));
+  std::memcpy (count_out, pin + in_bytes + n_cand * sizeof (long long), n_cand * sizeof (int));
   return 0;
 }
 
diff --git a/audiowmark_amd/csrc/host/context.cc b/audiowmark_amd/csrc/host/context.cc
--- a/audiowmark_amd/csrc/host/context.cc
+++ b/audiowmark_amd/csrc/host/context.cc
@@ -181,7 +181,22 @@
   if (ev_sync)
     (void) hipEventDestroy (ev_sync);
   ev_sync = nullptr;
+  ws_block_base.release();
+  for (hipEvent_t& ev : ev_behind)
+    if (ev)
+      {
+        (void) hipEventDestroy (ev);
+        ev = nullptr;
+      }
   awm::speed_scratch_free (this);
+}
+
+hipStream_t
+awm::WorkLane::second_stream()
+{
+  if (!stream2 && hipStreamCreateWithFlags (&stream2, hipStreamNonBlocking) != hipSuccess)
+    stream2 = nullptr;
+  return stream2;
 }
 
 unsigned int *
@@ -212,6 +227,11 @@
       if (hipStreamCreateWithFlags (&nl->stream, hipStreamNonBlocking) != hipSuccess)
         return nullptr;
       nl->own_stream = true;
+      if (!nl->second_stream())
+        {
+          (void) hipStreamDestroy (nl->stream);
+          return nullptr;
+        }
       l = std::move (nl);
     }
   return l.get();
@@ -766,7 +786,7 @@
   AWM_HIP_CHECK (hipSetDevice (ctx->device));
   const int lanes = std::max (1, std::min (ctx->chunk_lanes, awm::CHUNK_LANES)) * (detect_speed ? 2 : 1);
   for (int i = 0; i < lanes && i < awm::MAX_LANES; i++)
-    if (!ctx->lane (i))
+    if (!ctx->lane (i) || !ctx->lane (i)->second_stream())
       {
         awm::set_error ("cannot create a work lane (stream)");
         return AWM_ERR_HIP;
@@ -791,10 +811,14 @@
       {
         if (l->stream)
           AWM_HIP_CHECK (hipStreamSynchronize (l->stream));
+        if (l->stream2)
+          AWM_HIP_CHECK (hipStreamSynchronize (l->stream2));
         l->release_lane();
       }
   if (ctx->copy_stream)
     AWM_HIP_CHECK (hipStreamSynchronize (ctx->copy_stream));
+  if (ctx->stream2)
+    AWM_HIP_CHECK (hipStreamSynchronize (ctx->stream2));
   ctx->release_lane();
   ctx->file_staging.release();
   awm::speed_workspace_free (ctx);
@@ -865,10 +889,21 @@
       {
         if (l->stream)
           (void) hipStreamSynchronize (l->stream);
+        if (l->stream2)
+          {
+            (void) hipStreamSynchronize (l->stream2);
+            (void) hipStreamDestroy (l->stream2);
+          }
         l->release_lane();
         if (l->own_stream && l->stream)
           (void) hipStreamDestroy (l->stream);
       }
+  if (ctx->stream2)
+    {
+      (void) hipStreamSynchronize (ctx->stream2);
+      (void) hipStreamDestroy (ctx->stream2);
+      ctx->stream2 = nullptr;
+    }
   ctx->release_lane();
   if (ctx->copy_stream)
     (void) hipStreamSynchronize (ctx->copy_stream);
diff --git a/audiowmark_amd/csrc/host/context.hh b/audiowmark_amd/csrc/host/context.hh
--- a/audiowmark_amd/csrc/host/context.hh
+++ b/audiowmark_amd/csrc/host/context.hh
@@ -213,6 +213,10 @@
   PinnedBuffer pin_refine_in[2], pin_refine_q[2], pin_peaks, pin_blocks, pin_jobs, pin_bits, pin_small, pin_group, pin_shard, pin_shard_up, pin_keytab;
   hipEvent_t   ev_refine[2] = { nullptr, nullptr };
   hipEvent_t   ev_sync = nullptr;
+  hipStream_t  stream2 = nullptr;
+  hipStream_t  second_stream();
+  hipEvent_t   ev_behind[4] = { nullptr, nullptr, nullptr, nullptr };
+  DevBuffer    ws_block_base;
   SpeedScratch *speed_scratch = nullptr;
   double       prof_live_fraction = 1.0;
   unsigned int *viterbi_sync (size_t n_decodes);
diff --git a/audiowmark_amd/csrc/host/syncfinder.cc b/audiowmark_amd/csrc/host/syncfinder.cc
--- a/audiowmark_amd/csrc/host/syncfinder.cc
+++ b/audiowmark_amd/csrc/host/syncfinder.cc
@@ -1,6 +1,8 @@
 #include "syncfinder.hh"
 #include "utils.hh"
+#include "wmdecode.hh"
 #include <algorithm>
+#include <numeric>
 #include <cmath>
 #include <cstdlib>
 
@@ -429,6 +431,8 @@
   const size_t n_cand = job.candidates.size();
   job.refined.clear();
   job.batch_pending = false;
+  job.behind.queued = job.behind.mismatch = false;
+  job.behind.live.clear();
   if (!n_cand)
     return 0;
   const bool gathered = wav.n_channels <= 2;
@@ -441,20 +445,44 @@
   if (int rc = m_lane->ws_refine.reserve (batch * (per_cand + tail_per_cand) * sizeof (float))) return rc;
   if (int rc = m_lane->ws_refine_have.reserve (batch * NW * REFINE_TP)) return rc;
   if (int rc = m_lane->ws_q.reserve (batch * (REFINE_QS * sizeof (double) + awmk::GATHERED_SCRATCH_BYTES_PER_PLANE))) return rc;
-  if (int rc = m_lane->ws_idx.reserve (batch * NW * (sizeof (long long) + sizeof (int)) + 2 * batch * sizeof (int))) return rc;
+  if (int rc = m_lane->ws_idx.reserve (batch * NW * (sizeof (long long) + sizeof (int)) + 2 * batch * sizeof (int)
+                                       + 8 + batch * sizeof (awmk::RefineSelectIn))) return rc;
+  bool behind = job.behind.want > 0 && mode == Mode::BLOCK && gathered && !job.slice_frames && !kt->slices && batch >= n_cand
+                && job.behind.stream.n_channels == wav.n_channels;
+  if (behind)
+    {
+      if (int rc = block_soft_bits_reserve (m_lane, wav.n_channels, n_cand, behind)) return rc;
+      if (int rc = m_lane->ws_block_base.reserve (n_cand * (sizeof (long long) + sizeof (int)))) return rc;
+      if (!m_lane->second_stream())
+        behind = false;
+    }
   for (size_t c0 = 0; c0 < n_cand; c0 += batch)
     {
       if (job.batch_pending)
         if (int rc = refine_batch_finish (job))
           return rc;
-      if (int rc = refine_batch_launch (kt, wav, mode, job, c0, std::min (batch, n_cand - c0), batch))
+      if (int rc = refine_batch_launch (kt, wav, mode, job, c0, std::min (batch, n_cand - c0), batch, behind))
         return rc;
     }
   return 0;
 }
 
-int
-SyncFinder::refine_batch_launch (KeyTables *kt, const DeviceWav& wav, Mode mode, SearchJob& job, size_t c0, size_t nb, size_t batch)
+std::atomic<int> g_behind_split { 50 };
+extern "C" void awm_debug_set_decode_behind_split (int percent) { g_behind_split = std::max (1, std::min (percent, 99)); }
+std::atomic<long long> g_behind_counts[4];
+extern "C" void awm_debug_decode_behind_counts (long long *out, int reset)
+{
+  for (int i = 0; i < 4; i++)
+    {
+      if (out)
+        out[i] = g_behind_counts[i].load();
+      if (reset)
+        g_behind_counts[i] = 0;
+    }
+}
+
+int
+SyncFinder::refine_batch_launch (KeyTables *kt, const DeviceWav& wav, Mode mode, SearchJob& job, size_t c0, size_t nb, size_t batch, bool behind)
 {
   const int clip = mode == Mode::CLIP;
   const auto& sync = kt->sync[clip];
@@ -471,24 +499,27 @@
   const size_t tail_per_cand = tail_layout ? size_t (NW) * row_values : 0;
   float *const d_tail = tail_layout ? m_lane->ws_refine.as<float>() + batch * per_cand : nullptr;
 
-  const size_t in_bytes = nb * NW * (sizeof (long long) + sizeof (int)) + 2 * nb * sizeof (int);
+  const size_t table_bytes = nb * NW * (sizeof (long long) + sizeof (int)) + 2 * nb * sizeof (int);
+  const size_t select_off = (table_bytes + 7) & ~size_t (7);
+  const size_t in_bytes = behind ? select_off + nb * sizeof (awmk::RefineSelectIn) : table_bytes;
   const bool slices = job.slice_frames > 0;
   const long long span_frames = slices ? (long long) job.slice_frames : (long long) wav.n_frames;
   PinnedBuffer& pin_in = m_lane->pin_refine_in[job.slot];
   PinnedBuffer& pin_q = m_lane->pin_refine_q[job.slot];
   if (int rc = pin_in.reserve (in_bytes)) return rc;
-  if (int rc = pin_q.reserve (nb * QS * sizeof (double))) return rc;
+  if (int rc = pin_q.reserve (nb * QS * sizeof (double) + nb * (sizeof (long long) + sizeof (int)))) return rc;
   auto *stream_base = pin_in.as<long long>();
   int *stream_count = reinterpret_cast<int *> (stream_base + nb * NW);
   int *lanes = stream_count + nb * NW;
   int *slice_of = lanes + nb;
+  auto *select_in = reinterpret_cast<awmk::RefineSelectIn *> (pin_in.as<char>() + select_off);
   job.lane_count.assign (nb, 0);
   job.starts.assign (nb, 0);
   job.c0 = c0;
   job.nb = nb;
   int max_count = 0;
-  long long n_items = 0;
-  double db_bytes = 0;
+  std::vector<long long> cand_items (nb, 0);
+  std::vector<double> cand_db_bytes (nb, 0.0);
   for (size_t c = 0; c < nb; c++)
     {
       const SearchScore& s = job.candidates[c0 + c];
@@ -504,37 +535,51 @@
       job.starts[c] = start;
       job.lane_count[c] = lanes[c] = count;
       max_count = std::max (max_count, count);
-      n_items += (long long) count * NW;
+      cand_items[c] = (long long) count * NW;
       if (count)
-        db_bytes += double (NW) * ((1024.0 + 8.0 * (count - 1)) * 4 * wav.n_channels + 4.0 * row_values * count);
+        cand_db_bytes[c] = double (NW) * ((1024.0 + 8.0 * (count - 1)) * 4 * wav.n_channels + 4.0 * row_values * count);
       const int *want_list = kt->slices ? kt->want_of_slice (job.cand_slice[c0 + c]) : sync.want_list.data();
       for (int w = 0; w < NW; w++)
         {
           stream_base[c * NW + w] = slice0 + start + (long long) want_list[w] * Params::frame_size;
           stream_count[c * NW + w] = count;
         }
+      if (behind)
+        select_in[c] = { s.raw_quality, s.local_mean, (long long) s.index, (long long) start };
     }
   auto *d_base = m_lane->ws_idx.as<long long>();
   int *d_count = reinterpret_cast<int *> (d_base + nb * NW);
   int *d_lanes = d_count + nb * NW;
   int *d_slice_of = d_lanes + nb;
+  const auto *d_select_in = reinterpret_cast<const awmk::RefineSelectIn *> (m_lane->ws_idx.as<char>() + select_off);
   AWM_HIP_CHECK (hipMemcpyAsync (d_base, stream_base, in_bytes, hipMemcpyHostToDevice, st));
 
   double *q = pin_q.as<double>();
   std::fill (q, q + nb * QS, 0.0);
-  if (max_count > 0)
-    {
+  const bool queue = behind && gathered && max_count > 0;
+  job.behind.queued = queue;
+  size_t n_first = nb;
+  if (queue && job.behind.want >= 2 && nb >= 12)
+    {
+      n_first = std::max<size_t> (6, nb * size_t (g_behind_split.load()) / 100 / 6 * 6);
+      if (n_first >= nb)
+        n_first = nb;
+    }
+  long long *d_block_base = m_lane->ws_block_base.as<long long>();
+  int *d_block_count = queue ? reinterpret_cast<int *> (d_block_base + nb) : nullptr;
+  auto event = [&] (hipEvent_t& ev) -> hipError_t { return ev ? hipSuccess : hipEventCreateWithFlags (&ev, hipEventDisableTiming); };
+  auto launch_db = [&] (size_t s0, size_t n, hipStream_t s) -> int {
       awmk::SyncDbArgs da {};
       da.pcm = wav.data;
       da.n_frames = wav.n_frames;
       da.n_channels = wav.n_channels;
       da.per_channel = 0;
-      da.stream_base = d_base;
-      da.stream_count = d_count;
+      da.stream_base = d_base + s0 * NW;
+      da.stream_count = d_count + s0 * NW;
       da.count0 = max_count;
-      da.n_streams = (long long) nb * NW;
+      da.n_streams = (long long) n * NW;
       da.hop = Params::sync_search_fine;
-      da.out = m_lane->ws_refine.as<float>();
+      da.out = m_lane->ws_refine.as<float>() + s0 * per_cand;
       da.out_stream_stride = (long long) row_values * TP;
       if (gathered)
         {
@@ -543,49 +588,64 @@
           da.rows_per_plane = NW;
         }
       da.ld = TP;
-      da.tail = d_tail;
+      da.tail = d_tail ? d_tail + s0 * tail_per_cand : nullptr;
       da.tail_stream_stride = row_values;
-      da.have = m_lane->ws_refine_have.as<char>();
+      da.have = m_lane->ws_refine_have.as<char>() + s0 * NW * HP;
       da.have_stream_stride = HP;
       da.first = (long long) m_first;
       da.last = (long long) m_last;
       if (slices)
         {
           da.stream_range = job.slice_range;
-          da.range_index = d_slice_of;
+          da.range_index = d_slice_of + s0;
           da.range_div = NW;
           da.tables_per_slice = kt->slices ? 1 : 0;
         }
       da.tile_frames = TP;
-      {
-        ProfScope ps (m_ctx, PROF_REFINE_DB, (slices ? m_lane->prof_live_fraction : 1.0) * db_bytes, st);
-        if (gathered)
-          AWM_HIP_CHECK (awmk::launch_sync_db_sliding (st, m_ctx->tabs, da));
-        else
-          AWM_HIP_CHECK (awmk::launch_sync_db (st, m_ctx->tabs, da));
-      }
+      const double db_bytes = std::accumulate (cand_db_bytes.begin() + s0, cand_db_bytes.begin() + s0 + n, 0.0);
+      ProfScope ps (m_ctx, PROF_REFINE_DB, (slices ? m_lane->prof_live_fraction : 1.0) * db_bytes, s);
       if (gathered)
+        AWM_HIP_CHECK (awmk::launch_sync_db_sliding (s, m_ctx->tabs, da));
+      else
+        AWM_HIP_CHECK (awmk::launch_sync_db (s, m_ctx->tabs, da));
+      return 0;
+  };
+  auto launch_scan = [&] (size_t s0, size_t n, hipStream_t s) -> int {
+      const long long n_items = std::accumulate (cand_items.begin() + s0, cand_items.begin() + s0 + n, 0LL);
+      if (gathered)
         {
           awmk::GatheredScanArgs ga {};
-          ga.db = m_lane->ws_refine.as<float>();
-          ga.have = clip ? m_lane->ws_refine_have.as<char>() : nullptr;
+          ga.db = m_lane->ws_refine.as<float>() + s0 * per_cand;
+          ga.have = clip ? m_lane->ws_refine_have.as<char>() + s0 * NW * HP : nullptr;
           ga.plane_stride = (long long) per_cand;
           ga.have_plane_stride = (long long) NW * HP;
           ga.ld = TP;
           ga.have_ld = HP;
-          ga.tail = d_tail;
+          ga.tail = d_tail ? d_tail + s0 * tail_per_cand : nullptr;
           ga.tail_plane_stride = (long long) tail_per_cand;
           ga.rows_per_bit = sync.host.rows_per_bit;
           ga.n_lanes = max_count;
-          ga.lane_count = d_lanes;
-          ga.n_planes = (long long) nb;
+          ga.lane_count = d_lanes + s0;
+          ga.n_planes = (long long) n;
           ga.min_delta = std::min (params().water_delta, 0.080);
-          ga.quality = m_lane->ws_q.as<double>();
+          ga.quality = m_lane->ws_q.as<double>() + s0 * QS;
           ga.q_stride = QS;
-          ga.chain_mag = reinterpret_cast<float *> (ga.quality + batch * QS);
-          ga.chain_n = reinterpret_cast<int *> (ga.chain_mag + batch * 12 * 128);
-          ProfScope ps (m_ctx, PROF_REFINE_SCAN, (slices ? m_lane->prof_live_fraction : 1.0) * double (n_items) * 4.0 * row_values, st);
-          AWM_HIP_CHECK (awmk::launch_sync_scan_gathered (st, ga));
+          ga.chain_mag = reinterpret_cast<float *> (m_lane->ws_q.as<double>() + batch * QS) + s0 * 12 * 128;
+          ga.chain_n = reinterpret_cast<int *> (reinterpret_cast<float *> (m_lane->ws_q.as<double>() + batch * QS) + batch * 12 * 128) + s0 * 6 * 128;
+          if (queue)
+            {
+              ga.select = d_select_in + s0;
+              ga.select_chunk_first = (long long) job.behind.chunk_first;
+              ga.select_chunk_frames = (long long) job.behind.chunk_frames;
+              ga.select_stream_frames = (long long) job.behind.stream.n_frames;
+              ga.select_block_samples = (long long) (mark_block_frame_count() * Params::frame_size);
+              ga.select_block_frames = int (mark_block_frame_count());
+              ga.select_fine = Params::sync_search_fine;
+              ga.select_base = d_block_base + s0;
+              ga.select_count = d_block_count + s0;
+            }
+          ProfScope ps (m_ctx, PROF_REFINE_SCAN, (slices ? m_lane->prof_live_fraction : 1.0) * double (n_items) * 4.0 * row_values, s);
+          AWM_HIP_CHECK (awmk::launch_sync_scan_gathered (s, ga));
         }
       else
         {
@@ -605,15 +665,52 @@
           sa.q_stride = QS;
           sa.table.packed = sync.packed_refine.as<int>();
           sa.table.rows_per_bit = sync.host.rows_per_bit;
-          ProfScope ps (m_ctx, PROF_REFINE_SCAN, double (n_items) * 324.0, st);
-          AWM_HIP_CHECK (awmk::launch_sync_scan (st, sa));
-        }
-      AWM_HIP_CHECK (hipMemcpyAsync (q, m_lane->ws_q.ptr, nb * QS * sizeof (double), hipMemcpyDeviceToHost, st));
-    }
+          ProfScope ps (m_ctx, PROF_REFINE_SCAN, double (n_items) * 324.0, s);
+          AWM_HIP_CHECK (awmk::launch_sync_scan (s, sa));
+        }
+      return 0;
+  };
   hipEvent_t& ev = m_lane->ev_refine[job.slot];
   if (!ev)
     AWM_HIP_CHECK (hipEventCreateWithFlags (&ev, hipEventDisableTiming));
-  AWM_HIP_CHECK (hipEventRecord (ev, st));
+  if (!queue)
+    {
+      if (max_count > 0)
+        {
+          if (int rc = launch_db (0, nb, st)) return rc;
+          if (int rc = launch_scan (0, nb, st)) return rc;
+          AWM_HIP_CHECK (hipMemcpyAsync (q, m_lane->ws_q.ptr, nb * QS * sizeof (double), hipMemcpyDeviceToHost, st));
+        }
+      AWM_HIP_CHECK (hipEventRecord (ev, st));
+      job.batch_pending = true;
+      return 0;
+    }
+  hipStream_t st2 = m_lane->stream2;
+  hipEvent_t *evb = m_lane->ev_behind;
+  for (int i = 0; i < 3; i++)
+    AWM_HIP_CHECK (event (evb[i]));
+  g_behind_counts[0]++;
+  if (n_first < nb)
+    {
+      g_behind_counts[1]++;
+      if (int rc = launch_db (0, n_first, st)) return rc;
+      AWM_HIP_CHECK (hipEventRecord (evb[0], st));
+      AWM_HIP_CHECK (hipStreamWaitEvent (st2, evb[0], 0));
+      if (int rc = launch_scan (0, n_first, st2)) return rc;
+      if (int rc = block_soft_bits_queued (m_ctx, m_lane, kt, job.behind.stream, d_block_base, d_block_count, 0, n_first, st2)) return rc;
+      AWM_HIP_CHECK (hipEventRecord (evb[2], st2));
+    }
+  const size_t s0 = n_first < nb ? n_first : 0;
+  if (int rc = launch_db (s0, nb - s0, st)) return rc;
+  if (int rc = launch_scan (s0, nb - s0, st)) return rc;
+  AWM_HIP_CHECK (hipEventRecord (evb[1], st));
+  if (int rc = block_soft_bits_queued (m_ctx, m_lane, kt, job.behind.stream, d_block_base, d_block_count, s0, nb - s0, st)) return rc;
+  if (n_first < nb)
+    AWM_HIP_CHECK (hipStreamWaitEvent (st, evb[2], 0));
+  AWM_HIP_CHECK (hipStreamWaitEvent (st2, evb[1], 0));
+  AWM_HIP_CHECK (hipMemcpyAsync (q, m_lane->ws_q.ptr, nb * QS * sizeof (double), hipMemcpyDeviceToHost, st2));
+  AWM_HIP_CHECK (hipMemcpyAsync (q + nb * QS, d_block_base, nb * (sizeof (long long) + sizeof (int)), hipMemcpyDeviceToHost, st2));
+  AWM_HIP_CHECK (hipEventRecord (ev, st2));
   job.batch_pending = true;
   return 0;
 }
@@ -640,7 +737,26 @@
               best_index = job.starts[c] + t * Params::sync_search_fine;
             }
         }
-      job.refined.push_back ({ best_index, best_quality, s.local_mean });
+      job.refined.push_back ({ best_index, best_quality, s.local_mean, int (job.c0 + c) });
+    }
+  if (job.behind.queued)
+    {
+      const auto *dev_base = reinterpret_cast<const long long *> (q + job.nb * REFINE_QS);
+      const int *dev_count = reinterpret_cast<const int *> (dev_base + job.nb);
+      const size_t block_samples = mark_block_frame_count() * Params::frame_size;
+      job.behind.live.assign (job.c0 + job.nb, 0);
+      for (size_t c = 0; c < job.nb; c++)
+        {
+          const size_t index = job.refined[job.refined.size() - job.nb + c].index;
+          const bool live = job.behind.chunk_frames >= index + block_samples
+                            && job.behind.stream.n_values() >= (job.behind.chunk_first + index + block_samples) * job.behind.stream.n_channels;
+          job.behind.live[job.c0 + c] = live;
+          if (dev_base[c] != (long long) (job.behind.chunk_first + index) || dev_count[c] != (live ? int (mark_block_frame_count()) : 0))
+            {
+              job.behind.mismatch = true;
+              g_behind_counts[2]++;
+            }
+        }
     }
   return 0;
 }
@@ -688,6 +804,7 @@
   job.done = true;
   job.batch_pending = false;
   job.select_pending = false;
+  job.behind.queued = job.behind.mismatch = false;
   KeyTables *kt = m_ctx->get_key_tables (key);
   if (!kt)
     return AWM_ERR_HIP;
@@ -752,7 +869,7 @@
   for (const auto& s : scores)
     {
       const double q = s.raw_quality - s.local_mean;
-      out.push_back ({ s.index, std::fabs (q), q > 0 ? ConvBlockType::a : ConvBlockType::b });
+      out.push_back ({ s.index, std::fabs (q), q > 0 ? ConvBlockType::a : ConvBlockType::b, s.cand });
     }
   return 0;
 }
diff --git a/audiowmark_amd/csrc/host/syncfinder.hh b/audiowmark_amd/csrc/host/syncfinder.hh
--- a/audiowmark_amd/csrc/host/syncfinder.hh
+++ b/audiowmark_amd/csrc/host/syncfinder.hh
@@ -1,5 +1,6 @@
 #pragma once
 #include "context.hh"
+#include <atomic>
 
 namespace awm {
 
@@ -22,12 +23,14 @@
     size_t        index;
     double        quality;
     ConvBlockType block_type;
+    int           cand = -1;
   };
   struct SearchScore
   {
     size_t index;
     double raw_quality;
     double local_mean;
+    int    cand = -1;
     double abs_quality() const { return std::fabs (raw_quality - local_mean); }
   };
   static constexpr int local_mean_distance = 20;
@@ -66,6 +69,15 @@
     std::vector<int> cand_slice;
     size_t           slice_frames = 0;
     const long long *slice_range = nullptr;
+    struct DecodeBehind
+    {
+      int       want = 0;
+      DeviceWav stream;
+      size_t    chunk_first = 0, chunk_frames = 0;
+      bool      queued = false;
+      bool      mismatch = false;
+      std::vector<char> live;
+    } behind;
   };
   int search_launch (const Key& key, const DeviceWav& wav, Mode mode, SearchJob& job, bool db_ready = false);
   int search_finish (SearchJob& job, std::vector<Score>& out);
@@ -103,9 +115,11 @@
   bool     m_prepare_pending = false;
   int scan_silence (const DeviceWav& wav);
   int fetch_scores (long long n_scores, std::vector<SearchScore>& out);
-  int refine_batch_launch (KeyTables *kt, const DeviceWav& wav, Mode mode, SearchJob& job, size_t c0, size_t nb, size_t batch);
+  int refine_batch_launch (KeyTables *kt, const DeviceWav& wav, Mode mode, SearchJob& job, size_t c0, size_t nb, size_t batch, bool behind = false);
   int refine_batch_finish (SearchJob& job);
   int refine_finish (SearchJob& job, std::vector<SearchScore>& scores);
 };
 
+extern std::atomic<long long> g_behind_counts[4];
+
 }
diff --git a/audiowmark_amd/csrc/host/wmdecode.hh b/audiowmark_amd/csrc/host/wmdecode.hh
--- a/audiowmark_amd/csrc/host/wmdecode.hh
+++ b/audiowmark_amd/csrc/host/wmdecode.hh
@@ -42,6 +42,9 @@
                                 const long long *slice_range, size_t slice_frames);
 awmk::SoftBitsArgs block_soft_args (KeyTables *kt, int n_channels, const float *planes, size_t nb, float *out, const long long *d_bases,
                                     const int *d_slice_of, const long long *slice_range, bool slices);
+int block_soft_bits_reserve (WorkLane *lane, int n_channels, size_t n, bool& fits);
+int block_soft_bits_queued (awm_ctx *ctx, WorkLane *lane, KeyTables *kt, const DeviceWav& wav, const long long *d_bases, const int *d_count,
+                            size_t b0, size_t nb, hipStream_t st);
 int decode_launch (awm_ctx *ctx, WorkLane *lane, KeyTables *kt, DecodeJob& job, const float *raw = nullptr);
 struct DecodedPattern { size_t pending_index; std::vector<int> bits; float error; };
 int decode_finish (WorkLane *lane, const Key& key, DecodeJob& job, const std::vector<ResultSet *>& result_sets, double speed,
diff --git a/audiowmark_amd/csrc/host/wmget.cc b/audiowmark_amd/csrc/host/wmget.cc
--- a/audiowmark_amd/csrc/host/wmget.cc
+++ b/audiowmark_amd/csrc/host/wmget.cc
@@ -165,6 +165,43 @@
 }
 
 int
+block_soft_bits_reserve (WorkLane *lane, int n_channels, size_t n, bool& fits)
+{
+  const long long block_stride = (long long) n_channels * Params::n_bands * block_plane_ld();
+  const size_t max_batch = std::max<size_t> (1, (size_t (2) << 30) / (block_stride * sizeof (float)));
+  const int n_bits = mark_data_frame_count() / params().frames_per_bit;
+  fits = n <= max_batch;
+  if (!fits)
+    return 0;
+  if (int rc = lane->ws_block_db.reserve (n * block_stride * sizeof (float))) return rc;
+  return lane->ws_soft.reserve (n * n_bits * sizeof (float));
+}
+
+int
+block_soft_bits_queued (awm_ctx *ctx, WorkLane *lane, KeyTables *kt, const DeviceWav& wav, const long long *d_bases, const int *d_count,
+                        size_t b0, size_t nb, hipStream_t st)
+{
+  const size_t count = mark_block_frame_count();
+  const int n_bits = mark_data_frame_count() / params().frames_per_bit;
+  const int C = wav.n_channels;
+  const long long block_stride = (long long) C * Params::n_bands * block_plane_ld();
+  float *planes = lane->ws_block_db.as<float>() + b0 * block_stride;
+  awmk::SyncDbArgs da = block_db_args (wav, d_bases + b0, nullptr, nb, planes, nullptr, 0);
+  da.stream_count = d_count + b0;
+  {
+    ProfScope ps (ctx, PROF_BLOCK_DB, double (nb) * count * C * (4096.0 + 324.0), st);
+    AWM_HIP_CHECK (awmk::launch_sync_db (st, ctx->tabs, da));
+  }
+  awmk::SoftBitsArgs sb = block_soft_args (kt, C, planes, nb, lane->ws_soft.as<float>() + b0 * n_bits, d_bases + b0, nullptr, nullptr, false);
+  sb.block_live = d_count + b0;
+  {
+    ProfScope ps (ctx, PROF_SOFT_BITS, double (nb) * count * C * 324.0, st);
+    AWM_HIP_CHECK (awmk::launch_soft_bits (st, sb));
+  }
+  return 0;
+}
+
+int
 block_soft_bits (awm_ctx *ctx, KeyTables *kt, const DeviceWav& wav, const std::vector<size_t>& index,
                  std::vector<std::vector<float>>& raw_bits, std::vector<char>& ok)
 {
@@ -573,6 +610,8 @@
 
 int g_merge_decodes = 0;
 extern "C" void awm_debug_set_merge_decodes (int on) { g_merge_decodes = on; }
+int g_decode_behind_refine = 1;
+extern "C" void awm_debug_set_decode_behind_refine (int mode) { g_decode_behind_refine = mode < 0 ? 0 : mode > 2 ? 2 : mode; }
 int g_chunk_stagger = -1;
 extern "C" void awm_debug_set_chunk_stagger (int on) { g_chunk_stagger = on; }
 int g_speed_overlap = 1;
@@ -653,7 +692,11 @@
     {
       if (!ok)
         for (WorkLane *l : lanes)
-          (void) hipStreamSynchronize (l->stream);
+          {
+            (void) hipStreamSynchronize (l->stream);
+            if (l->stream2)
+              (void) hipStreamSynchronize (l->stream2);
+          }
     }
   } drain { lanes };
   auto chunk_wav = [&] (size_t c) {
@@ -728,6 +771,10 @@
           return 0;
         }
       case 1:
+        cs.job.behind.want = spread && lane_base == 0 && speed == 1 && !g_merge_decodes && stream.n_channels <= 2 ? g_decode_behind_refine : 0;
+        cs.job.behind.stream = stream;
+        cs.job.behind.chunk_first = chunks[c].first_frame;
+        cs.job.behind.chunk_frames = chunks[c].n_frames;
         if (int rc = finder.select_refine (cs.job))
           return rc;
         cs.stage = 2;
@@ -739,6 +786,32 @@
             return rc;
           if (cs.ki == 0 && c == 0)
             first_scores = scores;
+          if (cs.job.behind.queued && !cs.job.behind.mismatch)
+            {
+              std::vector<PatternRawBits> pattern_raw_vec;
+              cs.decode = DecodeJob();
+              auto& pending = cs.decode.pending;
+              for (const auto& sc : scores)
+                {
+                  if (sc.cand < 0 || size_t (sc.cand) >= cs.job.behind.live.size() || !cs.job.behind.live[sc.cand])
+                    continue;
+                  PatternRawBits rb;
+                  rb.index = sc.index;
+                  rb.quality = sc.quality;
+                  rb.slot = sc.cand;
+                  rb.block_type = sc.block_type;
+                  pending.push_back ({ rb.block_type, 0, { { rb.slot, 0 } }, 0, 0, double (rb.index) / stream.sample_rate,
+                                       sc, ResultSet::Type::BLOCK, c });
+                  pattern_raw_vec.push_back (rb);
+                }
+              combine_blocks (pattern_raw_vec, stream, c, pending);
+              if (int rc = decode_launch (ctx, cs.lane, kt, cs.decode))
+                return rc;
+              cs.stage = 3;
+              return 0;
+            }
+          if (cs.job.behind.queued)
+            g_behind_counts[3]++;
           std::vector<size_t> wanted;
           std::vector<const SyncFinder::Score *> wanted_score;
           for (const auto& sc : scores)
@@ -838,7 +911,9 @@
         break;
       for (auto& cs : active)
         {
-          if (cs.stage >= 1 && cs.stage <= 3 && (active.size() == 1 || hipStreamQuery (cs.lane->stream) != hipErrorNotReady))
+          const bool behind = cs.stage == 2 && cs.job.behind.queued && cs.job.batch_pending && cs.lane->ev_refine[cs.job.slot];
+          if (cs.stage >= 1 && cs.stage <= 3
+              && (active.size() == 1 || (behind ? hipEventQuery (cs.lane->ev_refine[cs.job.slot]) : hipStreamQuery (cs.lane->stream)) != hipErrorNotReady))
             {
               if (int rc = advance (cs))
                 return rc;
diff --git a/include/awm_hip.h b/include/awm_hip.h
--- a/include/awm_hip.h
+++ b/include/awm_hip.h
@@ -351,6 +351,14 @@
 int  awm_debug_frame_mod_tables_d (awm_ctx *ctx, const uint8_t *keys, size_t n_keys, const char *payload_hex, int8_t *tables_out);
 int  awm_debug_clip_key_tables_check_d (awm_ctx *ctx, const uint8_t *keys, size_t n_keys, long long mismatch_out[9]);
 void awm_debug_set_key_tables_on_device (int on);
+void awm_debug_set_decode_behind_refine (int mode);
+void awm_debug_set_decode_behind_split (int percent);
+void awm_debug_decode_behind_counts (long long out[4], int reset);
+int  awm_debug_decode_behind_d (awm_ctx *ctx, const uint8_t key[16], const float *pcm_d, size_t n_frames, int n_channels, size_t n_cand,
+                                const double *quality, const int *n_offsets, const double *raw_quality, const double *local_mean,
+                                const long long *index, const long long *start, long long chunk_first, long long chunk_frames,
+                                long long stream_frames, uint32_t fill, float *planes_out_d, size_t planes_values, float *soft_out,
+                                long long *base_out, int *count_out);
 void awm_debug_set_merge_decodes (int on);
 void awm_debug_set_add_batched (int on);
 void awm_debug_set_add_slab_mb (int mb);
```

Result: no change. 723,200 xRT (-0.5%).
